# tychedelia/josefine

Hardware: AMD Instinct MI355X
Metric: Raft quorum decisions/sec over N partitions; achieved HBM GB/s vs roofline (higher is better)
Workload: dtype u64

## Files before the change

josefine_amd/csrc/jg_api_drains.h:

```cpp
#pragma once
namespace {
int node_keep_handover(jg_engine* e);
inline void seg_add(std::vector<JgSeg>& v, uint32_t seq, size_t n) {
  if (!n) return;
  if (!v.empty() && v.back().seq == seq) v.back().n += n;
  else v.push_back(JgSeg{seq, n});
}

int drain_scan(jg_engine* e, const std::vector<StepRec>& recs, hipStream_t st) {
  const size_t nrec = recs.size();
  if (!nrec) return JG_OK;
  if (e->scan_cap < 2 * nrec) {
    if (e->h_jobs) HIPCHK(hipHostFree(e->h_jobs));
    if (e->h_totals) HIPCHK(hipHostFree(e->h_totals));
    e->h_jobs = nullptr, e->h_totals = nullptr;
    e->scan_cap = std::max<size_t>(4 * nrec, 64);
    HIPCHK(hipHostMalloc((void**)&e->h_jobs, e->scan_cap * sizeof(JgScanJob), hipHostMallocDefault));
    HIPCHK(hipHostMalloc((void**)&e->h_totals, e->scan_cap * sizeof(uint64_t), hipHostMallocDefault));
  }
  for (size_t k = 0; k < nrec; k++) {
    const StepRec& r = recs[k];
    const uint32_t nb = (r.n + JG_SCAN_TILE - 1) / JG_SCAN_TILE;
    e->h_jobs[2 * k] = JgScanJob{r.d_bsum_m, r.d_bsum_m ? nb : 0u, 0};
    e->h_jobs[2 * k + 1] = JgScanJob{r.d_bsum_f, nb, 0};
// ... 460 lines not shown
    std::fill(count.begin(), count.end(), 0u);
    for (size_t i = 0; i < n; i++) count[(group[order[i]] >> shift) & (BUCKETS - 1)]++;
    uint32_t sum = 0;
    for (uint32_t b = 0; b < BUCKETS; b++) {
      uint32_t c = count[b];
      count[b] = sum;
      sum += c;
    }
    for (size_t i = 0; i < n; i++) tmp[count[(group[order[i]] >> shift) & (BUCKETS - 1)]++] = order[i];
    order.swap(tmp);
  }
}

int prepare_rows(jg_engine* e, uint32_t n, const uint32_t* group, const uint8_t* kind, const uint32_t* from,
                 const uint64_t* term, const uint64_t* id, const uint64_t* aux, const uint8_t* flag,
                 const uint64_t* blk_id, const uint64_t* blk_next, uint64_t n_blocks, uint64_t now_ms, JgRowsArgs* out,
                 uint32_t msg_per_row = 0) {
  StepRec rec;
  rec.n = n;
  rec.msg_per_row = msg_per_row ? msg_per_row : msg_bound(e->cfg.n_replicas);
  rec.fsm_per_row = fsm_bound();
  if ((uint64_t)n * rec.msg_per_row > 0xffffffffull) return fail(JG_EINVAL, "batch too large: split it");
  HIPCHK(e->arenas[e->cur_arena].alloc((size_t)n * 4, (void**)&rec.d_msg_cnt));
  HIPCHK(e->arenas[e->cur_arena].alloc((size_t)n * 4, (void**)&rec.d_fsm_cnt));
  HIPCHK(e->arenas[e->cur_arena].alloc((size_t)n * rec.msg_per_row * sizeof(jg_msg_row), (void**)&rec.d_msg));
  HIPCHK(e->arenas[e->cur_arena].alloc((size_t)n * rec.fsm_per_row * sizeof(jg_fsm_row), (void**)&rec.d_fsm));
  const uint32_t n_tiles = (n + JG_SCAN_TILE - 1) / JG_SCAN_TILE;
  HIPCHK(e->arenas[e->cur_arena].alloc((size_t)n_tiles * 8, (void**)&rec.d_bsum_m));
  HIPCHK(e->arenas[e->cur_arena].alloc((size_t)n_tiles * 8, (void**)&rec.d_bsum_f));
  JgRowsArgs a;
  a.n = n;
  a.group = group;
  a.kind = kind;
  a.from = from;
  a.term = term;
  a.id = id;
  a.aux = aux;
  a.flag = flag;
  a.blk_id = blk_id;
  a.blk_next = blk_next;
  a.n_blocks = n_blocks;
  a.msg_per_row = rec.msg_per_row;
  a.fsm_per_row = rec.fsm_per_row;
  a.msg_out = rec.d_msg;
  a.fsm_out = rec.d_fsm;
  a.msg_cnt = rec.d_msg_cnt;
  a.fsm_cnt = rec.d_fsm_cnt;
  a.bsum_m = rec.d_bsum_m;
  a.bsum_f = rec.d_bsum_f;
  a.err = e->d_err;
  a.now = now_ms;
  a.seq = e->seq;
  rec.seq = e->seq;
  e->n_launch += 1;
  e->recs.push_back(rec);
  e->n_cmds += n;
  e->maybe_irregular = true;
  e->flag_check_pending = true;
  e->irr_gen++;
  *out = a;
  return JG_OK;
}
int launch_rows(jg_engine* e, uint32_t n, const uint32_t* group, const uint8_t* kind, const uint32_t* from,
                const uint64_t* term, const uint64_t* id, const uint64_t* aux, const uint8_t* flag,
                const uint64_t* blk_id, const uint64_t* blk_next, uint64_t n_blocks, uint64_t now_ms) {
  JgRowsArgs a;
  const int rc = prepare_rows(e, n, group, kind, from, term, id, aux, flag, blk_id, blk_next, n_blocks, now_ms, &a);
  if (rc) return rc;
  static const char* runs_env = std::getenv("JG_APPLY_RUNS");
  static const bool runs = runs_env != nullptr, runs_small = runs_env && std::string(runs_env) == "small";
  if (runs_small)
    hipLaunchKernelGGL(k_apply_runs_small, dim3(std::min<uint32_t>((n + JG_RUN_TILE_SMALL - 1) / JG_RUN_TILE_SMALL, e->count_slots)), dim3(JG_BLOCK), 0,
                       e->stream, e->dev, a);
  else if (runs)
    hipLaunchKernelGGL(k_apply_runs, dim3(std::min<uint32_t>((n + JG_RUN_TILE - 1) / JG_RUN_TILE, e->count_slots)), dim3(JG_BLOCK), 0, e->stream,
                       e->dev, a);
  else
    hipLaunchKernelGGL(k_apply_rows, dim3(grid_for(n, e->count_slots)), dim3(JG_BLOCK), 0, e->stream, e->dev, a);
  HIPCHK(hipGetLastError());
  return JG_OK;
}

template <int R>
void launch_calib(jg_engine* e, const uint64_t* rot, const uint64_t* a8, uint64_t* b8, const uint32_t* c4) {
  hipLaunchKernelGGL(k_stream_calib<R>, dim3(e->dense_grid), dim3(JG_BLOCK), 0, e->stream, rot, a8, b8, c4,
                     e->cfg.n_groups);
}

}
```

josefine_amd/csrc/jg_api_misc.h:

```cpp
#pragma once
int jg_chain_compact(jg_engine* e, size_t n_trees, const uint64_t* off, const uint64_t* ids, const uint64_t* nexts,
                     const uint64_t* commits, uint8_t* removed) {
  if (!e || !off || !commits) return fail(JG_EINVAL, "null argument");
  if (!n_trees) return JG_OK;
  if (e->router) e = e->router->sh[0];
  HIPCHK(hipSetDevice(e->device));
  const size_t n = off[n_trees];
  if (n && (!ids || !nexts || !removed)) return fail(JG_EINVAL, "null argument");
  uint64_t *d_off = nullptr, *d_ids = nullptr, *d_next = nullptr, *d_commit = nullptr;
  uint8_t* d_rem = nullptr;
  HIPCHK(hipMalloc((void**)&d_off, (n_trees + 1) * 8));
  HIPCHK(hipMalloc((void**)&d_ids, std::max<size_t>(n * 8, 16)));
  HIPCHK(hipMalloc((void**)&d_next, std::max<size_t>(n * 8, 16)));
  HIPCHK(hipMalloc((void**)&d_commit, n_trees * 8));
  HIPCHK(hipMalloc((void**)&d_rem, std::max<size_t>(n, 16)));
  HIPCHK(hipMemcpyAsync(d_off, off, (n_trees + 1) * 8, hipMemcpyHostToDevice, e->stream));
  if (n) {
    HIPCHK(hipMemcpyAsync(d_ids, ids, n * 8, hipMemcpyHostToDevice, e->stream));
    HIPCHK(hipMemcpyAsync(d_next, nexts, n * 8, hipMemcpyHostToDevice, e->stream));
  }
  HIPCHK(hipMemcpyAsync(d_commit, commits, n_trees * 8, hipMemcpyHostToDevice, e->stream));
  HIPCHK(hipMemsetAsync(d_rem, 0, std::max<size_t>(n, 16), e->stream));
  hipLaunchKernelGGL(k_chain_compact, dim3(grid_for(n_trees, 2048)), dim3(JG_BLOCK), 0, e->stream, n_trees, d_off,
                     d_ids, d_next, d_commit, d_rem);
// ... 126 lines not shown
    if (!router_all_landed(e)) return JG_OK;
    return e->router->run([&](size_t d) { return drain_prefetch(e->router->sh[d], true); });
  }
  return drain_prefetch(e, false);
}

int jg_drain_wait(jg_engine* e) {
  if (!e) return fail(JG_EINVAL, "null argument");
  auto wait = [](jg_engine* s) {
    if (!s->inflight.phase) return (int)JG_OK;
    jg_engine::DrainThread& t = *s->drain_thread;
    std::unique_lock<std::mutex> lk(t.m);
    t.cv.wait(lk, [&] { return t.state == 2; });
    return (int)JG_OK;
  };
  if (e->router) {
    for (jg_engine* s : e->router->sh) wait(s);
    return JG_OK;
  }
  return wait(e);
}

int jg_drain_flush(jg_engine* e) {
  if (!e) return fail(JG_EINVAL, "null argument");
  auto flush = [](jg_engine* s) {
    int rc = drain_prefetch(s, true);
    if (rc) return rc;
    return inflight_finish(s);
  };
  if (e->router) {
    e->pipelined = true;
    for (jg_engine* s : e->router->sh) s->pipelined = true;
    return e->router->run([&](size_t d) { return flush(e->router->sh[d]); });
  }
  return flush(e);
}

int jg_drain_faults(jg_engine* e, jg_fault_row* out, size_t cap, size_t* n) {
  if (!e || !n) return fail(JG_EINVAL, "null argument");
  if (!e->router && e->pipelined && !inflight_landed(e)) {
    *n = 0;
    return JG_OK;
  }
  int rc = e->router ? router_collect(e, 0) : collect(e, 0);
  if (rc) return rc;
  std::vector<jg_fault_row>& q = e->router ? e->router->faults : e->q_faults;
  *n = q.size();
  if (!out) return JG_OK;
  if (cap < q.size()) return fail(JG_ECAPACITY, "output buffer too small");
  if (!q.empty()) std::memcpy(out, q.data(), q.size() * sizeof(jg_fault_row));
  q.clear();
  e->q_fault_seq.clear();
  return JG_OK;
}

int jg_read_state(jg_engine* e, int field, uint32_t replica, void* out, uint32_t g0, uint32_t n) {
  if (!e || (!out && n)) return fail(JG_EINVAL, "null argument");
  if (e->router) return router_read_state(e, field, replica, out, g0, n);
  if ((uint64_t)g0 + n > e->cfg.n_groups) return fail(JG_EINVAL, "group range out of bounds");
  if (field < 0 || field >= JG_FIELD__COUNT) return fail(JG_EINVAL, "unknown field");
  if (field == JG_FIELD_MATCH && replica >= e->cfg.n_replicas) return fail(JG_EINVAL, "replica out of range");
  if (!n) return JG_OK;
  int rc = sync_and_check(e);
  if (rc) return rc;
  const JgDev& d = e->dev;
  std::vector<uint32_t> fl(n);
  HIPCHK(hipMemcpy(fl.data(), d.flags + g0, (size_t)n * 4, hipMemcpyDeviceToHost));
  auto role = [&](uint32_t i) { return fl[i] & JGF_ROLE_MASK; };
  std::vector<uint64_t> t64;
  std::vector<uint32_t> t32;
  auto get64 = [&](const uint64_t* col) -> int {
    t64.resize(n);
    HIPCHK(hipMemcpy(t64.data(), col + g0, (size_t)n * 8, hipMemcpyDeviceToHost));
    return JG_OK;
  };
  auto cold_field = [&](const uint4* col, size_t offset, size_t width, void* dst) -> int {
    HIPCHK(hipMemcpy2D(dst, width, (const char*)(col + g0) + offset, sizeof(uint4), width, n, hipMemcpyDeviceToHost));
    return JG_OK;
  };
  auto cold32 = [&](size_t offset) -> int {
    t32.resize(n);
    return cold_field(d.cold.v, offset, 4, t32.data());
  };
  auto lag_base = [&](std::vector<uint64_t>& base) -> int {
    std::vector<uint64_t> top(n);
    HIPCHK(hipMemcpy(base.data(), d.head + g0, (size_t)n * 8, hipMemcpyDeviceToHost));
    HIPCHK(hipMemcpy(top.data(), d.run_hi + g0, (size_t)n * 8, hipMemcpyDeviceToHost));
    for (uint32_t i = 0; i < n; i++)
      if (jg_lag_base_is_run_hi(fl[i])) base[i] = top[i];
    return JG_OK;
  };
  auto copy64 = [&](const uint64_t* col) -> int {
    HIPCHK(hipMemcpy(out, col + g0, (size_t)n * 8, hipMemcpyDeviceToHost));
    return JG_OK;
  };
  uint64_t* o64 = (uint64_t*)out;
  uint32_t* o32 = (uint32_t*)out;
  uint8_t* o8 = (uint8_t*)out;
  switch (field) {
    case JG_FIELD_TERM: return copy64(d.term);
    case JG_FIELD_COMMIT: {
      std::vector<uint64_t> head(n), col(n);
      if ((rc = lag_base(head))) return rc;
      HIPCHK(hipMemcpy(col.data(), d.commit + g0, (size_t)n * 8, hipMemcpyDeviceToHost));
      if ((rc = get64(d.mlag))) return rc;
      for (uint32_t i = 0; i < n; i++) {
        const uint64_t f = jg_lag_field(t64[i], d.R, d.R);
        o64[i] = (role(i) != JG_ROLE_LEADER || jg_lag_wide(f, d.R)) ? col[i] : head[i] - f;
      }
      return JG_OK;
    }
    case JG_FIELD_HEAD: return copy64(d.head);
    case JG_FIELD_ELECTION_TIME: return cold_field(d.cold.t, JG_COLD_T_ELECTION_TIME, 8, out);
    case JG_FIELD_ELECTION_TIMEOUT: return cold_field(d.cold.t, JG_COLD_T_ELECTION_TIMEOUT, 4, out);
    case JG_FIELD_QUEUED_REQS: return cold_field(d.cold.v, JG_COLD_V_QUEUED, 4, out);
    case JG_FIELD_ID_GEN: {
      std::vector<uint64_t> head(n);
      HIPCHK(hipMemcpy(head.data(), d.head + g0, (size_t)n * 8, hipMemcpyDeviceToHost));
      if ((rc = get64(d.id_gen))) return rc;
      for (uint32_t i = 0; i < n; i++) o64[i] = (fl[i] & JGF_FAST) ? head[i] + 1 : t64[i];
      return JG_OK;
    }
    case JG_FIELD_MATCH: {
      std::vector<uint64_t> head(n), wide(n);
      if ((rc = lag_base(head))) return rc;
      HIPCHK(hipMemcpy(wide.data(), d.match_wide + (size_t)replica * d.G + g0, (size_t)n * 8, hipMemcpyDeviceToHost));
      if ((rc = get64(d.mlag))) return rc;
      for (uint32_t i = 0; i < n; i++) {
        const uint64_t f = jg_lag_field(t64[i], replica, d.R);
        o64[i] = role(i) != JG_ROLE_LEADER ? 0 : jg_lag_wide(f, d.R) ? wide[i] : head[i] - f;
      }
      return JG_OK;
    }
    case JG_FIELD_HEARTBEAT_TIME:
      if ((rc = get64(d.heartbeat_time))) return rc;
      for (uint32_t i = 0; i < n; i++) o64[i] = role(i) == JG_ROLE_LEADER ? t64[i] : 0;
      return JG_OK;
    case JG_FIELD_VOTED_FOR:
      if ((rc = cold32(JG_COLD_V_VOTED_FOR))) return rc;
      for (uint32_t i = 0; i < n; i++) o32[i] = (fl[i] & JGF_VOTED) ? t32[i] : 0;
      return JG_OK;
    case JG_FIELD_LEADER_ID:
      if ((rc = cold32(JG_COLD_V_LEADER_ID))) return rc;
      for (uint32_t i = 0; i < n; i++)
        o32[i] = (role(i) == JG_ROLE_FOLLOWER && (fl[i] & JGF_HAS_LEADER)) ? t32[i] : 0;
      return JG_OK;
    case JG_FIELD_VOTE_SEEN:
    case JG_FIELD_VOTE_GRANTED:
      if ((rc = cold32(JG_COLD_V_VOTES))) return rc;
      for (uint32_t i = 0; i < n; i++) {
        uint32_t v = field == JG_FIELD_VOTE_SEEN ? (t32[i] & 0xff) : ((t32[i] >> 8) & 0xff);
        o8[i] = role(i) == JG_ROLE_CANDIDATE ? (uint8_t)v : 0;
      }
      return JG_OK;
    case JG_FIELD_HAS_VOTED:
      for (uint32_t i = 0; i < n; i++) o8[i] = (fl[i] & JGF_VOTED) ? 1 : 0;
      return JG_OK;
    case JG_FIELD_ROLE:
      for (uint32_t i = 0; i < n; i++) o8[i] = (uint8_t)role(i);
      return JG_OK;
    case JG_FIELD_REPL_STATE:
      for (uint32_t i = 0; i < n; i++)
        o8[i] = role(i) == JG_ROLE_LEADER ? (uint8_t)((fl[i] & JGF_REPL_MASK) >> JGF_REPL_SHIFT) : 0;
      return JG_OK;
    case JG_FIELD_FAULT:
      for (uint32_t i = 0; i < n; i++) o8[i] = (uint8_t)((fl[i] & JGF_FAULT_MASK) >> JGF_FAULT_SHIFT);
      return JG_OK;
    case JG_FIELD_HAS_LEADER:
      for (uint32_t i = 0; i < n; i++) o8[i] = (role(i) == JG_ROLE_FOLLOWER && (fl[i] & JGF_HAS_LEADER)) ? 1 : 0;
      return JG_OK;
    case JG_FIELD_SELF_SLOT:
      for (uint32_t i = 0; i < n; i++) o8[i] = (uint8_t)((fl[i] & JGF_SELF_MASK) >> JGF_SELF_SHIFT);
      return JG_OK;
    default: return fail(JG_EINVAL, "unknown field");
  }
}

int jg_get_counters(jg_engine* e, uint64_t out[4]) {
  if (!e || !out) return fail(JG_EINVAL, "null argument");
  if (e->router) return router_get_counters(e, out);
  int rc = sync_and_check(e);
  if (rc) return rc;
  std::vector<uint64_t> slots(e->count_slots);
  HIPCHK(hipMemcpy(slots.data(), e->dev.blk_decisions, slots.size() * 8, hipMemcpyDeviceToHost));
  uint64_t dec = 0;
  for (uint64_t v : slots) dec += v;
  out[0] = e->n_cmds;
  out[1] = dec;
  out[2] = e->n_dense;
  out[3] = e->n_launch;
  return JG_OK;
}

int jg_device_alloc(jg_engine* e, size_t bytes, void** dev_ptr) {
  if (!e || !dev_ptr) return fail(JG_EINVAL, "null argument");
  if (e->router) return fail(JG_EINVAL, "device pointers are per shard: call this on a shard handle (jg_get_shard)");
  HIPCHK(hipSetDevice(e->device));
  HIPCHK(hipMalloc(dev_ptr, std::max<size_t>(bytes, 16)));
  HIPCHK(hipMemsetAsync(*dev_ptr, 0, std::max<size_t>(bytes, 16), e->stream));
  return JG_OK;
}
// ... 36 lines not shown
}
int jg_timer_stop(jg_engine* e, float* ms) {
  if (!e || !ms) return fail(JG_EINVAL, "null argument");
  if (e->router) {
    *ms = 0;
    for (jg_engine* s : e->router->sh) {
      float v = 0;
      const int rc = jg_timer_stop(s, &v);
      if (rc) return rc;
      *ms = std::max(*ms, v);
    }
    return JG_OK;
  }
  HIPCHK(hipSetDevice(e->device));
  HIPCHK(hipEventRecord(e->ev1, e->stream));
  {
    const auto t0 = std::chrono::steady_clock::now();
    hipError_t q;
    while ((q = hipEventQuery(e->ev1)) == hipErrorNotReady &&
           std::chrono::steady_clock::now() - t0 < std::chrono::milliseconds(20)) {
    }
    if (q != hipSuccess && q != hipErrorNotReady) return fail(JG_EDEVICE, std::string("hipEventQuery: ") + hipGetErrorString(q));
  }
  HIPCHK(hipEventSynchronize(e->ev1));
  HIPCHK(hipEventElapsedTime(ms, e->ev0, e->ev1));
  return JG_OK;
}

int jg_kernel_timing(jg_engine* e, int enable) {
  if (!e) return fail(JG_EINVAL, "null argument");
  if (e->router) {
    for (jg_engine* s : e->router->sh) {
      const int rc = jg_kernel_timing(s, enable);
      if (rc) return rc;
    }
    return JG_OK;
  }
  HIPCHK(hipSetDevice(e->device));
  if (enable && e->kt_ev.empty()) {
    e->kt_ev.resize(2 * jg_engine::KT_RING);
    for (hipEvent_t& ev : e->kt_ev) HIPCHK(hipEventCreate(&ev));
  }
  e->kt_on = enable != 0;
  e->kt_every = enable > 1 ? (uint32_t)enable : 1u;
  e->kt_n = 0, e->kt_seen = 0;
  return JG_OK;
}

int jg_kernel_timing_read(jg_engine* e, float* avg_us, uint32_t* n_launches) {
  if (!e || !avg_us || !n_launches) return fail(JG_EINVAL, "null argument");
  if (e->router) {
    *avg_us = 0, *n_launches = 0;
    for (jg_engine* s : e->router->sh) {
      float v = 0;
      uint32_t k = 0;
      const int rc = jg_kernel_timing_read(s, &v, &k);
      if (rc) return rc;
      if (v > *avg_us) *avg_us = v, *n_launches = k;
    }
    return JG_OK;
  }
  HIPCHK(hipSetDevice(e->device));
  HIPCHK(hipStreamSynchronize(e->stream));
  const uint64_t n = std::min<uint64_t>(e->kt_n, jg_engine::KT_RING);
  double sum = 0;
  for (uint64_t k = 0; k < n; k++) {
    float ms = 0;
    HIPCHK(hipEventElapsedTime(&ms, e->kt_ev[2 * k], e->kt_ev[2 * k + 1]));
    sum += ms;
  }
  *avg_us = n ? (float)(sum * 1e3 / (double)n) : 0.0f;
  *n_launches = (uint32_t)n;
  return JG_OK;
}

int jg_calibrate_stream(jg_engine* e, uint32_t iters, float* avg_us) {
  if (!e || !avg_us || !iters) return fail(JG_EINVAL, "null argument");
  if (e->router) e = e->router->sh[0];
  HIPCHK(hipSetDevice(e->device));
  const size_t G = e->cfg.n_groups, R = e->cfg.n_replicas;
  const size_t blk = std::max<size_t>(G * R * 8, 16);
  const size_t nbuf = std::min<size_t>(std::max<size_t>(((size_t)640 << 20) / blk + 1, 2), 64);
  char* rot = nullptr;
  uint64_t *a8 = nullptr, *b8 = nullptr;
  uint32_t* c4 = nullptr;
  HIPCHK(hipMalloc((void**)&rot, blk * nbuf));
  HIPCHK(hipMalloc((void**)&a8, std::max<size_t>(G * 8, 16)));
  HIPCHK(hipMalloc((void**)&b8, std::max<size_t>(G * 8, 16)));
  HIPCHK(hipMalloc((void**)&c4, std::max<size_t>(G * 4, 16)));
  HIPCHK(hipMemsetAsync(rot, 0, blk * nbuf, e->stream));
  HIPCHK(hipMemsetAsync(a8, 0, std::max<size_t>(G * 8, 16), e->stream));
  HIPCHK(hipMemsetAsync(b8, 0, std::max<size_t>(G * 8, 16), e->stream));
  HIPCHK(hipMemsetAsync(c4, 0, std::max<size_t>(G * 4, 16), e->stream));
  const uint32_t warm = 5;
  for (uint32_t i = 0; i < warm + iters; i++) {
    if (i == warm) HIPCHK(hipEventRecord(e->ev0, e->stream));
    const uint64_t* r = (const uint64_t*)(rot + (i % nbuf) * blk);
    switch (R) {
      case 1: launch_calib<1>(e, r, a8, b8, c4); break;
      case 2: launch_calib<2>(e, r, a8, b8, c4); break;
      case 3: launch_calib<3>(e, r, a8, b8, c4); break;
      case 4: launch_calib<4>(e, r, a8, b8, c4); break;
      case 5: launch_calib<5>(e, r, a8, b8, c4); break;
      case 6: launch_calib<6>(e, r, a8, b8, c4); break;
      case 7: launch_calib<7>(e, r, a8, b8, c4); break;
      default: launch_calib<8>(e, r, a8, b8, c4); break;
    }
  }
  HIPCHK(hipGetLastError());
  HIPCHK(hipEventRecord(e->ev1, e->stream));
  HIPCHK(hipEventSynchronize(e->ev1));
  float ms = 0;
  HIPCHK(hipEventElapsedTime(&ms, e->ev0, e->ev1));
  *avg_us = ms * 1000.0f / (float)iters;
  HIPCHK(hipFree(rot));
  HIPCHK(hipFree(a8));
  HIPCHK(hipFree(b8));
  HIPCHK(hipFree(c4));
  return JG_OK;
}

int jg_synth_fill_acks_device(jg_engine* e, uint32_t mode, uint64_t tick, uint64_t* sim_dev, uint64_t* acks_dev) {
  if (!e || !sim_dev || !acks_dev) return fail(JG_EINVAL, "null argument");
  if (e->router) return fail(JG_EINVAL, "device pointers are per shard: call this on a shard handle (jg_get_shard)");
  if (mode > 1) return fail(JG_EINVAL, "unknown synth mode");
  HIPCHK(hipSetDevice(e->device));
  hipLaunchKernelGGL(k_synth_acks, dim3(grid_for(e->cfg.n_groups, 4096)), dim3(JG_BLOCK), 0, e->stream, e->dev, mode,
                     tick, sim_dev, acks_dev);
  HIPCHK(hipGetLastError());
  return JG_OK;
}

}
```

josefine_amd/csrc/jg_await.h:

```cpp
#pragma once
#include "jg_device.h"
#include "jg_lookup.h"
#include "jg_read.h"
#include "jg_sparse.h"
#include "jg_compact.h"

#define JG_AWT_TILE JG_BLOCK
#define JG_AWT_PARTS 1024u
#define JG_AWT_WORDS 5u
static_assert(sizeof(jg_await_stats) == (JG_AWT_WORDS + 1) * 8, "jg_await_stats is the stat words in order, then left");
static_assert(sizeof(jg_await_row) == 48, "jg_await_row is three 16-byte pieces");
static_assert(sizeof(jg_done_row) == 48, "jg_done_row is three 16-byte pieces");

struct JgAwaitHead {
  uint32_t n, cur, pad[2];
};
static_assert(sizeof(JgAwaitHead) == 16, "the table's head is one 16-byte record");

struct JgAwaitArgs {
  uint32_t peek;
  uint32_t tiles;
  uint32_t parts;
  uint32_t n_keys;
  uint64_t now;
  uint64_t cap;
  uint64_t mask;
  uint4* buf[2];
  uint8_t* verdict;
  uint64_t* bsum;
  uint64_t* part;
  const uint64_t* total;
  uint4* out;
  const uint64_t* keys;
  uint64_t* mpart;
  uint32_t n;
  uint32_t cur;
  uint32_t add;
  uint64_t* sum;
  uint64_t* marked;
  uint32_t m;
  uint32_t room;
  uint32_t stats;
  JgAwaitHead* head;
  const uint32_t* gate;
  const uint4* rows;
  uint64_t* hdr;
};

__device__ __forceinline__ uint64_t jg_awt_u64(uint32_t lo, uint32_t hi) { return (uint64_t)lo | (uint64_t)hi << 32; }

__device__ __forceinline__ uint32_t jg_await_verdict(uint32_t wflags, uint32_t role, uint32_t fault, uint64_t term_now, uint64_t commit,
                                                     uint64_t block_id, uint64_t term, uint64_t deadline, uint64_t now) {
  if (wflags & JG_AWAIT_WITHDRAWN) return JG_DONE_CANCELLED;
  if (fault == JG_FAULT_VACANT) return JG_DONE_LOST | JG_DONE_VACANT;
  if (fault) return JG_DONE_LOST | JG_DONE_FAULTED;
  const bool leads = role == JG_ROLE_LEADER;
  if (term && (!leads || term_now != term)) return JG_DONE_LOST;
  if (leads ? block_id <= commit : block_id < commit) return JG_DONE_APPLIED;
  if (deadline && now >= deadline) return JG_DONE_EXPIRED;
  return 0u;
}

__device__ __forceinline__ void jg_await_count_tiles(const JgDev& d, const uint4* tab, uint32_t n, uint32_t tiles, uint32_t parts, uint64_t now,
                                                     uint8_t* verdict, uint64_t* bsum, uint64_t* part) {
  const uint32_t live = n / JG_AWT_TILE + (n % JG_AWT_TILE ? 1u : 0u);
  uint32_t bc[JG_AWT_WORDS] = {0u, 0u, 0u, 0u, 0u};
  for (uint32_t tile = blockIdx.x; tile < tiles; tile += parts) {
    uint32_t t = 0;
    if (tile < live) {
      const uint32_t i = tile * JG_AWT_TILE + threadIdx.x;
      const bool in = i < n;
      const size_t at = (size_t)(in ? i : 0u) * 3;
      const uint4 w0 = tab[at], w1 = tab[at + 1], w2 = tab[at + 2];
      const uint32_t g = w0.x < d.G ? w0.x : 0u;
      const uint32_t f = d.flags[g];
      const uint64_t term_now = d.term[g], head = d.head[g], pw = d.mlag[g], col = d.commit[g], run_hi = d.run_hi[g];
      const uint64_t commit = jg_read_commit(d, g, f);
      asm volatile("" ::"v"(f), "v"(term_now), "v"(head), "v"(pw), "v"(col), "v"(run_hi));
      const uint32_t role = f & JGF_ROLE_MASK, fault = (f & JGF_FAULT_MASK) >> JGF_FAULT_SHIFT;
      const uint32_t v = in ? jg_await_verdict(w0.y, role, fault, term_now, commit, jg_awt_u64(w1.x, w1.y), jg_awt_u64(w1.z, w1.w),
                                               jg_awt_u64(w2.x, w2.y), now)
                            : 0u;
      if (in) verdict[i] = (uint8_t)v;
      const uint64_t m = __ballot(in && v);
      bc[0] += __popcll(__ballot(in && !v));
      bc[1] += __popcll(m);
      bc[2] += __popcll(__ballot(in && (v & JG_DONE_APPLIED)));
      bc[3] += __popcll(__ballot(in && (v & JG_DONE_LOST)));
      bc[4] += __popcll(__ballot(in && (v & JG_DONE_EXPIRED)));
      t = jg_tile_count(__popcll(m));
    }
    if (threadIdx.x == 0) bsum[tile] = t;
    __syncthreads();
  }
  const uint64_t vals[JG_AWT_WORDS] = {bc[0], bc[1], bc[2], bc[3], bc[4]};
  jg_block_words<JG_AWT_WORDS>(vals, JgNeverMax(), part);
}

__device__ __forceinline__ void jg_await_write_tile(const JgDev& d, const uint4* tab, uint4* dst, uint32_t n, uint32_t add, uint32_t peek, uint64_t cap,
                                                    const uint64_t* total, const uint8_t* verdict, const uint64_t* bsum, uint4* out) {
  const uint64_t done = *total;
  if ((done < cap ? done : cap) == 0) return;
  if ((uint64_t)blockIdx.x * JG_AWT_TILE >= n) return;
  const uint64_t base = bsum[blockIdx.x];
  if (peek && base >= cap) return;
  const uint32_t i = blockIdx.x * JG_AWT_TILE + threadIdx.x;
  const bool in = i < n;
  const uint32_t v = in ? verdict[i] : 0u;
  const uint64_t rank = base + jg_rank_in_tile(__ballot(in && v));
  if (!in) return;
  const bool deliver = v && rank < cap;
  if (!deliver && peek) return;
  const size_t at = (size_t)i * 3;
  const uint4 w0 = tab[at], w1 = tab[at + 1], w2 = tab[at + 2];
  if (!deliver) {
    const size_t to = ((size_t)i - (size_t)(rank < cap ? rank : cap)) * 3;
    dst[to] = w0, dst[to + 1] = w1, dst[to + 2] = w2;
    return;
  }
  const uint32_t g = w0.x < d.G ? w0.x : 0u;
  const uint32_t f = d.flags[g];
  const uint64_t term_now = d.term[g], head = d.head[g];
  const uint64_t commit = jg_read_commit(d, g, f);
  const uint32_t role = f & JGF_ROLE_MASK, fault = (f & JGF_FAULT_MASK) >> JGF_FAULT_SHIFT, self = (f & JGF_SELF_MASK) >> JGF_SELF_SHIFT;
  auto lo = [](uint64_t x) { return (uint32_t)x; };
  auto hi = [](uint64_t x) { return (uint32_t)(x >> 32); };
  jg_u32x4* row = (jg_u32x4*)out + rank * 3;
  row[0] = jg_u32x4{add + g, v | role << 8 | fault << 16 | self << 24, w0.z, w0.w};
  row[1] = jg_u32x4{w1.x, w1.y, lo(term_now), hi(term_now)};
  row[2] = jg_u32x4{lo(commit), hi(commit), lo(head), hi(head)};
}

__global__ __launch_bounds__(JG_BLOCK) void k_await_count(JgDev d, JgAwaitArgs a) {
  jg_await_count_tiles(d, a.buf[a.cur & 1u], a.n, a.tiles, a.parts, a.now, a.verdict, a.bsum, a.part);
}

__global__ __launch_bounds__(JG_BLOCK) void k_await_stats_sum(JgAwaitArgs a) {
  jg_parts_reduce<JG_AWT_WORDS>(a.part, a.parts, a.sum, JgNeverMax());
}

__global__ __launch_bounds__(JG_BLOCK) void k_await_write(JgDev d, JgAwaitArgs a) {
  const uint32_t cur = a.cur & 1u;
  jg_await_write_tile(d, a.buf[cur], a.buf[cur ^ 1u], a.n, a.add, a.peek, a.cap, a.total, a.verdict, a.bsum, a.out);
}

#define JG_AWT_KEYS_LDS 2048u

__device__ __forceinline__ bool jg_awt_has_key(const uint64_t* keys, uint32_t n, uint64_t key) {
  uint32_t lo = 0, hi = n;
  while (lo < hi) {
    const uint32_t mid = (lo + hi) >> 1;
    if (keys[mid] < key) lo = mid + 1;
    else hi = mid;
  }
  return lo < n && keys[lo] == key;
}

__device__ __forceinline__ void jg_await_mark_tiles(uint4* tab, uint32_t n, uint32_t tiles, uint32_t parts, const uint64_t* keys, uint32_t n_keys,
                                                    uint64_t mask, uint64_t* part) {
  __shared__ uint64_t lds_keys[JG_AWT_KEYS_LDS];
  const bool staged = n_keys <= JG_AWT_KEYS_LDS;
  if (staged) {
    for (uint32_t k = threadIdx.x; k < n_keys; k += JG_BLOCK) lds_keys[k] = keys[k];
    __syncthreads();
  }
  uint32_t marked = 0;
  for (uint32_t tile = blockIdx.x; tile < tiles; tile += parts) {
    if ((uint64_t)tile * JG_AWT_TILE >= n) break;
    const uint32_t i = tile * JG_AWT_TILE + threadIdx.x;
    const bool in = i < n;
    const size_t at = (size_t)(in ? i : 0u) * 3;
    const uint4 w0 = tab[at];
    const uint64_t key = jg_awt_u64(w0.z, w0.w) & mask;
    const bool has = staged ? jg_awt_has_key(lds_keys, n_keys, key) : jg_awt_has_key(keys, n_keys, key);
    const bool hit = in && has && !(w0.y & JG_AWAIT_WITHDRAWN);
    if (hit) ((uint32_t*)(tab + at))[1] = w0.y | JG_AWAIT_WITHDRAWN;
    marked += __popcll(__ballot(hit));
  }
  const uint64_t vals[1] = {marked};
  jg_block_words<1>(vals, JgNeverMax(), part);
}

__global__ __launch_bounds__(JG_BLOCK) void k_await_mark(JgAwaitArgs a) {
  jg_await_mark_tiles(a.buf[a.cur & 1u], a.n, a.tiles, a.parts, a.keys, a.n_keys, a.mask, a.mpart);
}

__global__ __launch_bounds__(JG_BLOCK) void k_await_mark_sum(JgAwaitArgs a) {
  jg_parts_reduce<1>(a.mpart, a.parts, a.marked, JgNeverMax());
}


#define JG_AH_TOTAL 0u
#define JG_AH_GIVEN 1u
#define JG_AH_STATS 2u
#define JG_AH_LEFT (JG_AH_STATS + JG_AWT_WORDS)
#define JG_AH_N (JG_AH_LEFT + 1u)
#define JG_AH_CUR (JG_AH_N + 1u)
#define JG_AH_GATE (JG_AH_CUR + 1u)
#define JG_AH_MARKED (JG_AH_GATE + 1u)
#define JG_AH_WORDS (JG_AH_MARKED + 1u)

__device__ __forceinline__ bool jg_await_gated(const uint32_t* gate) { return gate && *gate; }
__device__ __forceinline__ uint32_t jg_await_n_eff(const JgAwaitArgs& a, uint32_t n) {
  const uint64_t e = (uint64_t)n + a.m;
  return e > a.room ? a.room : (uint32_t)e;
// ... 47 lines not shown
```

josefine_amd/csrc/jg_commits.h:

```cpp
#pragma once
#include "jg_device.h"
#include "jg_lookup.h"
#include "jg_read.h"
#include "jg_sparse.h"
#include "jg_watch.h"

#define JG_CMT_ROWS 4u
#define JG_CMT_TILE (JG_BLOCK * JG_CMT_ROWS)
#define JG_CMT_PARTS 1024u
#define JG_CMT_WORDS 6u
static_assert(sizeof(jg_commit_backlog) == JG_CMT_WORDS * 8, "jg_commit_backlog is the backlog words in order");
static_assert(sizeof(jg_commit_row) == 48, "jg_commit_row is three 16-byte pieces");

struct JgCommitArgs {
  uint32_t g0, n;
  uint32_t add;
  uint32_t peek;
  uint32_t commits_only;
  uint32_t backlog;
  uint32_t tiles;
  uint32_t parts;
  uint4* shadow;
  uint32_t* cnt;
  uint64_t* bsum;
  uint64_t* part;
  uint64_t* sum;
  uint4* out;
  uint64_t cap;
  const uint32_t* gate;
};

__device__ __forceinline__ uint64_t jg_cmt_u64(uint32_t lo, uint32_t hi) { return (uint64_t)lo | (uint64_t)hi << 32; }

__device__ __forceinline__ uint64_t jg_commit_view(const JgDev& d, uint32_t g, uint32_t f, uint64_t w, uint64_t head, uint64_t col) {
  const uint32_t R = d.R;
  const bool leader = (f & JGF_ROLE_MASK) == JG_ROLE_LEADER;
  const uint64_t fc = jg_lag_field(w, R, R);
  uint64_t c = leader ? head - fc : col;
  if (leader && (jg_lag_wide(fc, R) || jg_lag_base_is_run_hi(f))) c = jg_read_commit(d, g, f);
  return c;
}
__device__ __forceinline__ bool jg_commit_differs(const uint4& sh, uint64_t commit, uint64_t head, uint32_t commits_only) {
  return sh.x != (uint32_t)commit || sh.y != (uint32_t)(commit >> 32) ||
         (!commits_only && (sh.z != (uint32_t)head || sh.w != (uint32_t)(head >> 32)));
}
__device__ __forceinline__ void jg_commit_backlog_add(bool on, uint64_t m, const uint4& sh, uint64_t commit, uint64_t head, uint32_t* bc,
                                                      uint64_t& commits, uint64_t& appends) {
  const uint64_t cf = jg_cmt_u64(sh.x, sh.y), hf = jg_cmt_u64(sh.z, sh.w);
  const bool up_c = on && commit > cf, up_h = on && head > hf;
  bc[0] += __popcll(m);
  bc[1] += __popcll(__ballot(up_c));
  bc[2] += __popcll(__ballot(up_h));
  bc[3] += __popcll(__ballot(on && (commit < cf || head < hf)));
  commits += up_c ? commit - cf : 0ull;
  appends += up_h ? head - hf : 0ull;
}

__device__ __forceinline__ void jg_commit_ballots(const JgDev& d, const JgCommitArgs& a, uint32_t tile, uint32_t* f, uint64_t* commit,
                                                  uint64_t* head, uint4* sh, uint64_t* m) {
  const uint32_t t0 = tile * JG_CMT_TILE + threadIdx.x;
  uint64_t w[JG_CMT_ROWS], col[JG_CMT_ROWS];
#pragma unroll
  for (uint32_t k = 0; k < JG_CMT_ROWS; k++) {
    const uint32_t i = t0 + k * JG_BLOCK;
    const bool in = i < a.n;
    const uint32_t g = a.g0 + (in ? i : 0u);
    f[k] = in ? d.flags[g] : 0u;
    head[k] = in ? d.head[g] : 0ull;
    w[k] = in ? d.mlag[g] : 0ull;
    col[k] = in ? d.commit[g] : 0ull;
    sh[k] = in ? a.shadow[g] : make_uint4(0, 0, 0, 0);
  }
#pragma unroll
  for (uint32_t k = 0; k < JG_CMT_ROWS; k++) asm volatile("" ::"v"(f[k]), "v"(head[k]), "v"(w[k]), "v"(col[k]), "v"(sh[k].x), "v"(sh[k].z));
#pragma unroll
  for (uint32_t k = 0; k < JG_CMT_ROWS; k++) {
    const uint32_t i = t0 + k * JG_BLOCK;
    const bool in = i < a.n;
    commit[k] = jg_commit_view(d, a.g0 + (in ? i : 0u), f[k], w[k], head[k], col[k]);
    m[k] = __ballot(in && jg_commit_differs(sh[k], commit[k], head[k], a.commits_only));
  }
}

__global__ __launch_bounds__(JG_BLOCK) void k_commit_count(JgDev d, JgCommitArgs a) {
  const uint32_t lane = threadIdx.x & 63u;
  uint32_t bc[4] = {0u, 0u, 0u, 0u};
  uint64_t commits = 0, appends = 0;
  for (uint32_t tile = blockIdx.x; tile < a.tiles; tile += a.parts) {
    uint32_t f[JG_CMT_ROWS];
    uint64_t commit[JG_CMT_ROWS], head[JG_CMT_ROWS], m[JG_CMT_ROWS];
    uint4 sh[JG_CMT_ROWS];
    jg_commit_ballots(d, a, tile, f, commit, head, sh, m);
    uint32_t c = 0;
#pragma unroll
    for (uint32_t k = 0; k < JG_CMT_ROWS; k++) c += __popcll(m[k]);
    if (a.backlog) {
#pragma unroll
      for (uint32_t k = 0; k < JG_CMT_ROWS; k++)
        jg_commit_backlog_add((m[k] >> lane) & 1ull, m[k], sh[k], commit[k], head[k], bc, commits, appends);
    }
    const uint32_t t = jg_tile_count(c);
    if (threadIdx.x == 0) a.cnt[tile] = t, a.bsum[tile] = t;
    __syncthreads();
  }
  if (!a.backlog) return;
  const uint64_t vals[JG_CMT_WORDS] = {bc[0], bc[1], bc[2], bc[3], jg_wave_sum64(commits), jg_wave_sum64(appends)};
  jg_block_words<JG_CMT_WORDS>(vals, JgNeverMax(), a.part);
}

__global__ __launch_bounds__(JG_BLOCK) void k_commit_write(JgDev d, JgCommitArgs a) {
  const uint64_t base = a.bsum[blockIdx.x];
  if (a.cnt[blockIdx.x] == 0 || base >= a.cap) return;
  uint32_t f[JG_CMT_ROWS];
  uint64_t commit[JG_CMT_ROWS], head[JG_CMT_ROWS], m[JG_CMT_ROWS];
  uint4 sh[JG_CMT_ROWS];
  jg_commit_ballots(d, a, blockIdx.x, f, commit, head, sh, m);
  const uint32_t peek = jg_gated_peek(a.peek, a.gate);
  const uint32_t lane = threadIdx.x & 63u;
  const uint32_t t0 = blockIdx.x * JG_CMT_TILE + threadIdx.x;
  uint64_t term[JG_CMT_ROWS];
#pragma unroll
  for (uint32_t k = 0; k < JG_CMT_ROWS; k++)
    term[k] = ((m[k] >> lane) & 1ull) ? d.term[a.g0 + t0 + k * JG_BLOCK] : 0ull;
  jg_u32x4* out = (jg_u32x4*)a.out;
  auto lo = [](uint64_t x) { return (uint32_t)x; };
  auto hi = [](uint64_t x) { return (uint32_t)(x >> 32); };
  jg_ranked_rows<JG_CMT_ROWS>(m, base, a.cap, [&](uint32_t k, uint64_t pos) {
    const uint32_t g = a.g0 + t0 + k * JG_BLOCK;
    const uint32_t role = f[k] & JGF_ROLE_MASK, fault = (f[k] & JGF_FAULT_MASK) >> JGF_FAULT_SHIFT, self = (f[k] & JGF_SELF_MASK) >> JGF_SELF_SHIFT;
    const uint64_t cf = jg_cmt_u64(sh[k].x, sh[k].y), hf = jg_cmt_u64(sh[k].z, sh[k].w);
    const uint32_t state = (commit[k] > cf ? (uint32_t)JG_CMT_COMMITTED : 0u) | (head[k] > hf ? (uint32_t)JG_CMT_APPENDED : 0u) |
                           (commit[k] < cf || head[k] < hf ? (uint32_t)JG_CMT_REWOUND : 0u) |
                           (role == JG_ROLE_LEADER && fault == 0 ? (uint32_t)JG_CMT_LEADS : 0u) |
                           (fault == JG_FAULT_VACANT ? (uint32_t)JG_CMT_VACANT : fault ? (uint32_t)JG_CMT_FAULTED : 0u);
    out[pos * 3 + 0] = jg_u32x4{a.add + g, role | state << 8 | fault << 16 | self << 24, lo(term[k]), hi(term[k])};
    out[pos * 3 + 1] = jg_u32x4{sh[k].x, sh[k].y, lo(commit[k]), hi(commit[k])};
    out[pos * 3 + 2] = jg_u32x4{sh[k].z, sh[k].w, lo(head[k]), hi(head[k])};
    if (!peek) a.shadow[g] = make_uint4(lo(commit[k]), hi(commit[k]), lo(head[k]), hi(head[k]));
  });
}

__global__ __launch_bounds__(JG_BLOCK) void k_commit_backlog_sum(JgCommitArgs a) {
  jg_parts_reduce<JG_CMT_WORDS>(a.part, a.parts, a.sum, JgNeverMax());
}
```

josefine_amd/csrc/jg_dense.h:

```cpp
#pragma once
#include "jg_device.h"

#ifndef JG_BLOCK
#define JG_BLOCK 256
#endif

struct JgDenseHot {
  uint32_t* flags;
  uint64_t* mlag;
  uint64_t* head;
  uint64_t* blk_decisions;
  uint32_t G;
  uint32_t hb_timeout, cfg_flags;
  uint64_t* term;
  uint64_t* heartbeat_time;
  uint32_t g_begin, g_end;
};
__host__ __device__ __forceinline__ JgDenseHot jg_dense_hot_of(const JgDev& d) {
  return JgDenseHot{d.flags, d.mlag, d.head, d.blk_decisions, d.G, d.hb_timeout, d.cfg_flags, d.term, d.heartbeat_time, 0u, d.G};
}
__host__ __device__ __forceinline__ JgDenseHot jg_dense_hot_range(const JgDev& d, uint32_t begin, uint32_t end, uint32_t slot0) {
  JgDenseHot h = jg_dense_hot_of(d);
  h.blk_decisions += slot0, h.g_begin = begin, h.g_end = end;
  return h;
}


__device__ __forceinline__ void jg_block_count(uint64_t* slots, uint32_t v) {
  __shared__ uint32_t wave_sum[JG_BLOCK / 64];
#pragma unroll
  for (int off = 32; off > 0; off >>= 1) v += __shfl_down(v, off, 64);
  uint32_t lane = threadIdx.x & 63u, wave = threadIdx.x >> 6;
  if (lane == 0) wave_sum[wave] = v;
  __syncthreads();
  if (threadIdx.x == 0) {
    uint32_t s = 0;
#pragma unroll
    for (int w = 0; w < JG_BLOCK / 64; w++) s += wave_sum[w];
    if (s)
      (void)__hip_atomic_fetch_add(&slots[blockIdx.x], (uint64_t)s, __ATOMIC_RELAXED, __HIP_MEMORY_SCOPE_AGENT);
  }
}

struct JgDecCount {
  uint32_t lane = 0;
};
__device__ __forceinline__ void jg_count_add(uint64_t* slots, uint32_t total) {
  (void)__hip_atomic_fetch_add(&slots[blockIdx.x], (uint64_t)total, __ATOMIC_RELAXED, __HIP_MEMORY_SCOPE_AGENT);
}
__device__ __forceinline__ void jg_count_step(uint64_t* slots, JgDecCount& c, bool on, uint32_t n) {
  const uint64_t m = __ballot(on);
  if (!m) return;
  const int first = __ffsll((long long)m) - 1;
  const uint32_t n0 = __builtin_amdgcn_readlane(n, first);
  if (__ballot(on && n != n0) == 0) {
    if ((int)(threadIdx.x & 63u) == first && n0) jg_count_add(slots, n0 * (uint32_t)__popcll(m));
  } else {
    c.lane += on ? n : 0u;
  }
}
__device__ __forceinline__ void jg_wave_count(uint64_t* slots, const JgDecCount& c) {
  uint32_t v = c.lane;
  if (__ballot(v != 0) == 0) return;
#pragma unroll
  for (int off = 32; off > 0; off >>= 1) v += __shfl_down(v, off, 64);
  if ((threadIdx.x & 63u) == 0 && v) jg_count_add(slots, v);
}

template <int R>
__device__ __forceinline__ void jg_dense_load_acks(const uint64_t* __restrict__ acks, uint32_t G, uint32_t g,
                                                   uint64_t (&a)[R]) {
#pragma unroll
  for (int r = 0; r < R; r++) a[r] = __builtin_nontemporal_load(&acks[(size_t)r * G + g]);
}
template <int R, bool MAYBE_NO_ACKS = true>
__device__ __forceinline__ void jg_dense_load(const JgDenseHot& d, const uint64_t* __restrict__ acks, uint32_t g,
                                              uint64_t (&a)[R], uint64_t& mword, uint64_t& head) {
  if (!MAYBE_NO_ACKS || acks) {
    jg_dense_load_acks<R>(acks, d.G, g, a);
  } else {
#pragma unroll
    for (int r = 0; r < R; r++) a[r] = JG_NO_ACK;
  }
  mword = d.mlag[g];
  head = d.head[g];
}
template <int R>
struct JgLagTick {
  uint64_t w1, head1;
  uint32_t nf;
  uint32_t l[R + 1];
  uint32_t adv;
  bool cwide;
};

template <int R>
__device__ __forceinline__ uint32_t jg_kth_lag(const uint32_t (&v)[R + 1]) {
  constexpr int K = R / 2;
  if (R == 3) {
    const uint32_t lo = min(v[0], v[1]), hi = max(v[0], v[1]);
    return max(lo, min(hi, v[2]));
  } else if (R == 5) {
    const uint32_t x = max(min(v[0], v[1]), min(v[2], v[3]));
    const uint32_t y = min(max(v[0], v[1]), max(v[2], v[3]));
    const uint32_t lo = min(x, y), hi = max(x, y);
    return max(lo, min(hi, v[4]));
  } else {
    uint32_t q = 0;
#pragma unroll
    for (int j = 0; j < R; j++) {
      int cnt = 0;
#pragma unroll
      for (int i = 0; i < R; i++) cnt += (v[i] < v[j] || (v[i] == v[j] && i < j)) ? 1 : 0;
      q = (cnt == K) ? v[j] : q;
    }
    return q;
  }
}

template <int R>
__device__ __forceinline__ bool jg_lag_tick(uint32_t s, uint32_t f, uint64_t w0, uint64_t head0, uint64_t n_app,
                                            const uint64_t (&a)[R], JgLagTick<R>& o, uint32_t& dec) {
  constexpr uint32_t B = 64u / (R + 1u);
  if (B > 21) return false;
  constexpr uint32_t ESC = (uint32_t)((1ull << (B > 21 ? 21 : B)) - 1ull);
  constexpr uint32_t BEHIND = ESC - 1u, INF = 0xffffffffu;
  const uint32_t n = (uint32_t)n_app;
  bool bad = n_app >= JG_MAX_DENSE_APPENDS;
  const uint64_t head1 = head0 + n;
  uint32_t incm = 0, somem = 0;
#pragma unroll
  for (int r = 0; r < R; r++) {
    const uint32_t fr = (uint32_t)(w0 >> (r * B)) & ESC;
    const uint64_t ar = a[r];
    const uint64_t dk = head1 - ar;
    const bool self = (uint32_t)r == s;
    const bool some = !self && ar != JG_NO_ACK;
    const bool behind = fr == BEHIND;
    uint32_t dl = (uint32_t)(dk >> 32) ? 0xffffffffu : (uint32_t)dk;
    dl = some ? dl : 0xffffffffu;
    const uint32_t frn = fr + n;
    const bool inc = dl < frn;
    incm |= inc ? (1u << r) : 0u;
    somem |= some ? (1u << r) : 0u;
    uint32_t lo = (self && n) ? 0u : min(frn, dl);
    bad |= fr == ESC;
    bad |= behind ? some : lo >= BEHIND;
    bad |= some && ar > head1;
    lo = (behind && !(self && n)) ? INF : lo;
    o.l[r] = lo;
  }
  const uint32_t fc = (uint32_t)(w0 >> (R * B)) & ESC;
  const uint32_t lc = fc == BEHIND ? INF : fc + n;
  const uint32_t ql = jg_kth_lag<R>(o.l);
  const uint32_t nl = min(lc, ql);
  o.l[R] = nl;
  bad |= fc == ESC;
  bad |= nl >= BEHIND;
  if (bad) return false;
  uint32_t nf = (f & ~(somem << JGF_REPL_SHIFT)) | (incm << JGF_REPL_SHIFT);
  nf |= n ? (1u << (JGF_REPL_SHIFT + s)) : 0u;
  nf |= ql < lc ? JGF_COMMIT_KEY : 0u;
  uint64_t w = 0;
#pragma unroll
  for (int r = 0; r <= R; r++) w |= (uint64_t)min(o.l[r], BEHIND) << (r * B);
  o.w1 = w;
  o.head1 = head1;
  o.nf = nf;
  o.cwide = fc == BEHIND;
  o.adv = lc - nl;
  dec += n + (uint32_t)__popc(somem);
  return true;
}

template <int R>
__device__ __forceinline__ bool jg_lag_pre(uint32_t s, uint64_t w0, uint64_t head0, const uint64_t (&a)[R], uint32_t pre,
                                           uint32_t& adv_pre) {
  constexpr uint32_t B = 64u / (R + 1u);
  constexpr uint32_t ESC = (uint32_t)((1ull << (B > 21 ? 21 : B)) - 1ull);
  constexpr uint32_t BEHIND = ESC - 1u, INF = 0xffffffffu;
  bool bad = false;
  uint32_t l[R + 1];
#pragma unroll
  for (int r = 0; r < R; r++) {
    const uint32_t fr = (uint32_t)(w0 >> (r * B)) & ESC;
    const uint64_t ar = a[r];
    const bool some = (uint32_t)r != s && ((pre >> r) & 1u) && ar != JG_NO_ACK;
    const uint64_t dk = head0 - ar;
    uint32_t dl = (uint32_t)(dk >> 32) ? INF : (uint32_t)dk;
    dl = some ? dl : INF;
    bad |= some && ar > head0;
    l[r] = fr == BEHIND ? INF : min(fr, dl);
  }
  const uint32_t fc = (uint32_t)(w0 >> (R * B)) & ESC;
  const uint32_t lc = fc == BEHIND ? INF : fc;
  const uint32_t ql = jg_kth_lag<R>(l);
  adv_pre = lc - min(lc, ql);
  return !bad;
}

template <int R>
__device__ __forceinline__ bool jg_lag_tick_regs(uint32_t s, uint32_t& nf_io, uint32_t (&l)[R + 1], uint64_t& head_io,
                                                 uint64_t n_app, const uint64_t (&a)[R], uint32_t& dec) {
  const uint64_t head0 = head_io;
  constexpr uint32_t INF = 0xffffffffu;
  const uint32_t n = (uint32_t)n_app;
  bool bad = n_app >= JG_MAX_DENSE_APPENDS;
  const uint64_t head1 = head0 + n;
  uint32_t incm = 0, somem = 0;
  uint32_t nl[R + 1];
#pragma unroll
  for (int r = 0; r < R; r++) {
// ... 127 lines not shown
  if ((f & JGF_ROLE_MASK) != JG_ROLE_LEADER) {
    if (n_app) {
      d.flags[g] = f | (JG_FAULT_ENGINE_DENSE_NONLEADER << JGF_FAULT_SHIFT);
      jg_push_fault(d, g, JG_FAULT_ENGINE_DENSE_NONLEADER, seq);
    }
    return JG_DENSE_SKIP;
  }
  if (n_app >= JG_MAX_DENSE_APPENDS) {
    d.flags[g] = f | (JG_FAULT_ENGINE_DENSE_APPENDS << JGF_FAULT_SHIFT);
    jg_push_fault(d, g, JG_FAULT_ENGINE_DENSE_APPENDS, seq);
    return JG_DENSE_SKIP;
  }
  if (!(f & JGF_FAST)) return JG_DENSE_DEFER;
  return JG_DENSE_RUN;
}

template <int R, bool SKIP_OWN>
__device__ __forceinline__ void jg_dense_outbox_none(uint32_t G, const JgLeaderNode& nd, uint32_t g, uint32_t s) {
  nd.o_beat[g] = jg_leader_beat{0, JG_NO_ACK};
  if (nd.o_aec) {
    nd.o_aec[g] = JG_NO_ACK;
    return;
  }
#pragma unroll
  for (int r = 0; r < R; r++)
    if (!(SKIP_OWN && (uint32_t)r == s)) nd.o_ae[(size_t)r * G + g] = JG_NO_ACK;
}
template <int R, bool SKIP_OWN, class MoOf>
__device__ __forceinline__ uint32_t jg_dense_leader_tick(const JgDenseHot& h, const JgDev* dp, const JgLeaderNode& nd,
                                                         uint32_t g, uint32_t seq, uint32_t s, uint64_t term,
                                                         uint64_t hbt, uint64_t head, uint64_t commit, uint32_t nf,
                                                         MoOf mo_of) {
  const uint32_t G = h.G;
  if (head >= JG_MAILBOX_NONE) {
    jg_dense_outbox_none<R, SKIP_OWN>(G, nd, g, s);
    jg_push_fault(*dp, g, JG_FAULT_ENGINE_MAILBOX_RANGE, seq);
    return nf | (JG_FAULT_ENGINE_MAILBOX_RANGE << JGF_FAULT_SHIFT);
  }
  const bool due = (nd.now - hbt) > (uint64_t)h.hb_timeout;
  const uint64_t hb = due ? commit : JG_NO_ACK;
  const bool key_in_range = (nf & JGF_COMMIT_KEY) && !(h.cfg_flags & JG_CFG_SEPARATE_COMMIT_KEY);
  bool dead = false;
  uint64_t word[R];
#pragma unroll
  for (int r = 0; r < R; r++) {
    uint32_t n = JG_AE_NONE;
    uint64_t from = 0;
    if ((uint32_t)r != s && !dead) {
      const bool repl = (nf >> (JGF_REPL_SHIFT + r)) & 1u;
      const uint32_t want = repl ? JG_MAX_INFLIGHT + 1 : 2;
      from = mo_of(r);
      const uint64_t avail = from <= head ? head - from + 1 : 0;
      const uint32_t cnt = avail >= want ? want : (uint32_t)avail;
      if (cnt < want && key_in_range) {
        dead = true;
        from = 0;
        nf |= JG_FAULT_RANGE_HIT_COMMIT_KEY << JGF_FAULT_SHIFT;
      } else {
        n = cnt ? cnt - 1 : 0;
      }
    }
    word[r] = n == JG_AE_NONE ? JG_NO_ACK : JG_AE(from, n);
  }
  if (dead) jg_push_fault(*dp, g, JG_FAULT_RANGE_HIT_COMMIT_KEY, seq);
  if (due) h.heartbeat_time[g] = nd.now;
  nd.o_beat[g] = jg_leader_beat{term, hb};
  if (nd.o_aec) {
    const uint64_t first = s == 0 ? word[R > 1 ? 1 : 0] : word[0];
    bool same = true;
#pragma unroll
    for (int r = 0; r < R; r++) same = same && ((uint32_t)r == s || word[r] == first);
    nd.o_aec[g] = same ? first : JG_AEC_INDIVIDUAL;
    if (__builtin_expect(same, 1)) return nf;
  }
#pragma unroll
  for (int r = 0; r < R; r++)
    if (!(SKIP_OWN && (uint32_t)r == s)) nd.o_ae[(size_t)r * G + g] = word[r];
  return nf;
}

template <int R>
struct JgDenseIn {
  uint32_t f;
  uint64_t a[R], w, head;
  uint64_t term, hbt;
  uint32_t own;
};
template <int R, bool UNIFORM, bool NODE, bool ANY = false>
__device__ __forceinline__ void jg_dense_issue(const JgDenseHot& h, const JgDev* dp,
                                               const uint64_t* __restrict__ acks, uint32_t us,
                                               const JgLeaderNode& nd, bool emit, uint32_t g, JgDenseIn<R>& in) {
  in.f = h.flags[g];
  in.term = in.hbt = 0;
  if (!NODE) {
    jg_dense_load<R, false>(h, acks, g, in.a, in.w, in.head);
  } else {
#pragma unroll
    for (int r = 0; r < R; r++)
      in.a[r] = (ANY && (uint32_t)r == us) ? nd.offered[g] : __builtin_nontemporal_load(&acks[((size_t)r * h.G + g) * nd.ack_stride]);
    if (ANY) in.own = nd.owner[g];
    in.w = h.mlag[g];
    in.head = h.head[g];
    in.term = h.term[g];
    in.hbt = h.heartbeat_time[g];
  }
  asm volatile("" ::"v"(in.f));
  if (NODE) asm volatile("" ::"v"(in.term), "v"(in.hbt));
  __builtin_amdgcn_sched_barrier(0);
}

template <int R>
__device__ __forceinline__ uint64_t jg_lds_kth(const uint64_t (*sm)[JG_BLOCK]) {
  const uint32_t t = threadIdx.x;
  uint64_t q = 0;
#pragma clang loop unroll(disable)
  for (int j = 0; j < R; j++) {
    const uint64_t vj = sm[j][t];
    int cnt = 0;
#pragma clang loop unroll(disable)
    for (int i = 0; i < R; i++) {
      const uint64_t vi = sm[i][t];
      cnt += (vi > vj || (vi == vj && i < j)) ? 1 : 0;
    }
    q = (cnt == R / 2) ? vj : q;
  }
  return q;
}

template <int R, bool UNIFORM>
__device__ __forceinline__ void jg_dense_cold_lds(const JgDev& d, const uint64_t* __restrict__ acks, uint32_t seq,
                                               uint32_t s, uint32_t f, uint64_t n_app, uint32_t g,
                                               const uint64_t (&a_in)[R], uint64_t w0, uint64_t head0, JgDecCount& dec,
                                               uint64_t (*sm)[JG_BLOCK]) {
  const uint32_t G = d.G, t = threadIdx.x;
  const uint32_t B = jg_lag_bits(R);
  const uint64_t esc = jg_lag_esc(R);
  uint64_t(*sa)[JG_BLOCK] = sm + R;
#pragma unroll
  for (int r = 0; r < R; r++) sa[r][t] = ((uint32_t)r == s || !acks) ? JG_NO_ACK : a_in[r];
  uint64_t hi = 0;
#pragma clang loop unroll(disable)
  for (int r = 0; r < R; r++) {
    const uint64_t fl = (w0 >> (r * B)) & esc;
    const uint64_t v = jg_lag_wide(fl, R) ? d.match_wide[(size_t)r * G + g] : head0 - fl;
    sm[r][t] = v;
    hi = v > hi ? v : hi;
    const uint64_t a = sa[r][t];
    hi = (a != JG_NO_ACK && a > hi) ? a : hi;
  }
  const uint64_t fc = (w0 >> (R * B)) & esc;
  const uint64_t commit0 = jg_lag_wide(fc, R) ? d.commit[g] : head0 - fc;
  uint64_t commit = commit0, head = head0;
  uint32_t nf = f, fault = 0, dc = 0;
  const bool fused = hi <= head0;
  if (fused) {
    head = head0 + n_app;
    if (n_app) {
      const bool inc = sm[s][t] < head;
      if (inc) sm[s][t] = head;
      nf = inc ? (nf | (1u << (JGF_REPL_SHIFT + s))) : (nf & ~(1u << (JGF_REPL_SHIFT + s)));
      dc += (uint32_t)n_app;
    }
  } else {
    for (uint64_t i = 0; i < n_app && !fault; i++) {
      head += 1;
      const bool inc = sm[s][t] < head;
      if (inc) sm[s][t] = head;
      nf = inc ? (nf | (1u << (JGF_REPL_SHIFT + s))) : (nf & ~(1u << (JGF_REPL_SHIFT + s)));
      dc += 1;
      const uint64_t q = jg_lds_kth<R>(sm);
      if (q > commit) {
        if (q <= head) commit = q;
        else fault = JG_FAULT_COMMIT_MISSING_BLOCK;
      }
    }
  }
#pragma clang loop unroll(disable)
  for (int r = 0; r < R; r++) {
    if (fault) continue;
    const uint64_t a = sa[r][t];
    if (a == JG_NO_ACK) continue;
    const bool inc = sm[r][t] < a;
    if (inc) sm[r][t] = a;
    nf = inc ? (nf | (1u << (JGF_REPL_SHIFT + r))) : (nf & ~(1u << (JGF_REPL_SHIFT + r)));
    dc += 1;
    if (!fused) {
      const uint64_t q = jg_lds_kth<R>(sm);
      if (q > commit) {
        if (q <= head) commit = q;
        else fault = JG_FAULT_COMMIT_MISSING_BLOCK;
      }
    }
  }
  if (fused) {
    const uint64_t q = jg_lds_kth<R>(sm);
    commit = q > commit ? q : commit;
  }
  if (fault) {
    nf |= fault << JGF_FAULT_SHIFT;
    jg_push_fault(d, g, fault, seq);
  }
  if (commit != commit0) nf |= JGF_COMMIT_KEY;
  dec.lane += dc;
  uint64_t w = 0;
#pragma clang loop unroll(disable)
  for (int r = 0; r < R; r++) {
    const uint64_t v = sm[r][t];
    const uint64_t fl = jg_lag_encode(v, head, R);
    if (jg_lag_wide(fl, R)) d.match_wide[(size_t)r * G + g] = v;
    w |= fl << (r * B);
  }
  const uint64_t fl = jg_lag_encode(commit, head, R);
  if (jg_lag_wide(fl, R) && (commit != commit0 || !jg_lag_wide(fc, R))) d.commit[g] = commit;
  w |= fl << (R * B);
  if (w != w0) d.mlag[g] = w;
  if (head != head0) d.head[g] = head;
  if (nf != f) d.flags[g] = nf;
}

template <int R, bool UNIFORM, bool NODE, bool DEFER, bool FSM = false, bool ANY = false>
__device__ __forceinline__ void jg_dense_group(const JgDenseHot& h, const JgDev* dp,
                                               const uint64_t* __restrict__ acks, uint32_t seq, uint32_t us, const JgLeaderNode& nd, bool emit, uint32_t g,
                                               const JgDenseIn<R>& in, JgDecCount& dec, uint64_t (*sm)[JG_BLOCK]) {
  const uint32_t f = in.f;
  const uint32_t s = UNIFORM ? us : (f & JGF_SELF_MASK) >> JGF_SELF_SHIFT;
  const uint64_t mword0 = in.w, head0 = in.head, term = in.term, hbt = in.hbt;
  bool hbr_trigger = false;
  uint64_t a[R];
#pragma unroll
  for (int r = 0; r < R; r++) {
    a[r] = NODE ? jg_answer_ack(in.a[r]) : in.a[r];
    if (NODE) hbr_trigger |= (uint32_t)r != s && jg_answer_hb(in.a[r]) == 0;
  }
  uint64_t n_app = a[0];
#pragma unroll
  for (int r = 1; r < R; r++) n_app = (uint32_t)r == s ? a[r] : n_app;
  if (NODE && !nd.ack_stride) n_app = 0;
  const bool mine = !ANY || in.own == s;
  if (ANY && !mine) {
#pragma unroll
    for (int r = 0; r < R; r++) a[r] = JG_NO_ACK;
    n_app = 0;
    hbr_trigger = false;
  }
  uint32_t pre = 0;
  if (FSM) {
    pre = (uint32_t)(n_app >> JG_NODE_PRE_SHIFT) & 0xffu;
    n_app &= (1ull << JG_NODE_PRE_SHIFT) - 1ull;
  }
  JgLagTick<R> lt;
  lt.cwide = false, lt.adv = 0;
  uint32_t dl = 0;
  bool hot = (f & (JGF_FAULT_MASK | JGF_ROLE_MASK | JGF_FAST)) == (JG_ROLE_LEADER | JGF_FAST);
  uint64_t base0 = head0;
  if (NODE) {
    const bool runx = (f & (JGF_FAULT_MASK | JGF_ROLE_MASK | JGF_FAST | JGF_WIN_MASK | JGF_NO_GENESIS)) == JG_ROLE_LEADER && n_app == 0;
    if (__builtin_expect(runx, 0)) {
      if (!(f & JGF_RUN)) base0 = dp->run_hi[g];
      hot = true;
    }
  }
  if (NODE) hot = hot && !hbr_trigger;
  if (ANY) hot = hot && mine;
  hot = jg_lag_tick<R>(s, f, mword0, base0, n_app, a, lt, dl) && hot;
  if (FSM) hot = hot && n_app <= 1 && !lt.cwide;
  uint32_t adv_pre = 0;
  if (FSM && __builtin_expect(pre != 0, 0)) hot = jg_lag_pre<R>(s, mword0, base0, a, pre, adv_pre) && hot;
  if (!NODE) jg_count_step(h.blk_decisions, dec, hot, dl);
  if (__builtin_expect(hot, 1)) {
    if (emit)
      lt.nf = jg_dense_leader_tick<R, UNIFORM>(h, dp, nd, g, seq, s, term, hbt, lt.head1, lt.head1 - lt.l[R], lt.nf, [&](int r) {
        return lt.l[r] == 0xffffffffu ? dp->match_wide[(size_t)r * h.G + g] : lt.head1 - lt.l[r];
      });
    if (lt.w1 != mword0) h.mlag[g] = lt.w1;
    if (lt.head1 != base0) h.head[g] = lt.head1;
    if (lt.nf != f) h.flags[g] = lt.nf;
    if (FSM) {
      uint32_t w = (n_app ? JG_FSM_APPENDED_BIT : 0u) | lt.adv | (adv_pre << JG_FSM_PRE_SHIFT);
      if (__builtin_expect(lt.adv > JG_FSM_ADV_MASK, 0)) {
        const uint64_t commit0 = lt.head1 - lt.l[R] - lt.adv;
        nd.fsm_prev[g] = commit0;
        nd.fsm_mid[g] = commit0 + adv_pre;
        w = (n_app ? JG_FSM_APPENDED_BIT : 0u) | JG_FSM_WIDE_BIT;
      }
      if (w) nd.fsm_delta[g] = w;
    }
    if (NODE) jg_count_step(h.blk_decisions, dec, true, dl);
    return;
  }
  const JgDev& d = *dp;
  if (NODE && !ANY && nd.mask_offers && (f & JGF_ROLE_MASK) != JG_ROLE_LEADER) {
    if (emit) jg_dense_outbox_none<R, UNIFORM>(h.G, nd, g, s);
    return;
  }
  int cls = jg_dense_classify(d, g, f, n_app, seq);
  if ((NODE || DEFER) && cls == JG_DENSE_RUN) cls = JG_DENSE_DEFER;
  jg_defer_mark(d, g, cls == JG_DENSE_DEFER);
  if (NODE) {
    if (emit && mine) jg_dense_outbox_none<R, UNIFORM>(h.G, nd, g, s);
    return;
  }
  if (DEFER || cls != JG_DENSE_RUN) return;
  *d.cold_seen = 1;
  jg_dense_cold_lds<R, UNIFORM>(d, acks, seq, s, f, n_app, g, a, mword0, head0, dec, sm);
}

template <int R, bool UNIFORM, bool NODE, bool DEFER, bool FSM = false, bool ANY = false>
__device__ __forceinline__ JgDecCount jg_dense_tick_body(const JgDenseHot& h, const JgDev* dp,
                                                       const uint64_t* __restrict__ acks, uint32_t seq, uint32_t us,
                                                       const JgLeaderNode& nd, uint64_t (*sm)[JG_BLOCK]) {
  const uint32_t end = h.g_end, stride = gridDim.x * JG_BLOCK;
  const bool emit = NODE && nd.o_beat != nullptr;
  JgDecCount dec;
  uint32_t g = h.g_begin + blockIdx.x * JG_BLOCK + threadIdx.x;
  for (; g < end; g += stride) {
    if (FSM && nd.sparse_bits && jg_sparse_skip(nd.sparse_bits, nd.sparse_mode, g)) continue;
    if (ANY) {
      const uint32_t f0 = h.flags[g];
      if (__ballot((f0 & (JGF_ROLE_MASK | JGF_FAULT_MASK)) == JG_ROLE_LEADER) == 0) continue;
    }
    JgDenseIn<R> in;
    jg_dense_issue<R, UNIFORM, NODE, ANY>(h, dp, acks, us, nd, emit, g, in);
    jg_dense_group<R, UNIFORM, NODE, DEFER, FSM, ANY>(h, dp, acks, seq, us, nd, emit, g, in, dec, sm);
  }
  return dec;
}

template <int R, bool DEFER>
__global__ __launch_bounds__(JG_BLOCK) void k_leader_tick_dense(JgDenseHot h, const JgDev* __restrict__ dp,
                                                                               const uint64_t* __restrict__ acks,
                                                                               uint32_t seq, int us) {
  __shared__ uint64_t sm[DEFER ? 1 : 2 * R][JG_BLOCK];
  JgDecCount dec;
  JgLeaderNode nd{};
  if (us >= 0) dec = jg_dense_tick_body<R, true, false, DEFER>(h, dp, acks, seq, (uint32_t)us, nd, sm);
  else dec = jg_dense_tick_body<R, false, false, DEFER>(h, dp, acks, seq, 0, nd, sm);
  jg_wave_count(h.blk_decisions, dec);
}

#ifdef JG_LEADER_WAVES
#define JG_LEADER_OCC __attribute__((amdgpu_waves_per_eu(JG_LEADER_WAVES, JG_LEADER_WAVES)))
#else
#define JG_LEADER_OCC
#endif
#ifdef JG_FOLLOWER_WAVES
#define JG_FOLLOWER_OCC __attribute__((amdgpu_waves_per_eu(JG_FOLLOWER_WAVES, JG_FOLLOWER_WAVES)))
#else
#define JG_FOLLOWER_OCC
#endif
template <int R, bool FSM>
__global__ __launch_bounds__(JG_BLOCK) JG_LEADER_OCC void k_leader_node_tick(JgDenseHot h, const JgDev* __restrict__ dp,
                                                                const uint64_t* __restrict__ acks, uint32_t seq, int us,
                                                                JgLeaderNode nd) {
  if (nd.clock) {
    const uint32_t a = nd.clock->idx_lead & 1u;
    nd.now = nd.clock->v[a].now, seq = nd.clock->v[a].seq[nd.clock_slot];
    if (blockIdx.x == 0 && threadIdx.x == 0) nd.clock->idx_rest = a;
  }
  JgDecCount dec;
  if (us >= 0) dec = jg_dense_tick_body<R, true, true, true, FSM>(h, dp, acks, seq, (uint32_t)us, nd, nullptr);
  else dec = jg_dense_tick_body<R, false, true, true, FSM>(h, dp, acks, seq, 0, nd, nullptr);
  jg_wave_count(h.blk_decisions, dec);
}

struct JgLeaderJob {
  JgDenseHot h;
  const JgDev* dp;
  const uint64_t* acks;
  uint32_t seq;
  int us;
  JgLeaderNode nd;
};
template <int R>
__global__ __launch_bounds__(JG_BLOCK) void k_leader_node_tick_any(const JgLeaderJob* __restrict__ jobs) {
  const JgLeaderJob& j = jobs[blockIdx.y];
  JgLeaderNode nd = j.nd;
  uint32_t seq = j.seq;
  if (nd.clock) {
    const uint32_t a = nd.clock->idx_lead & 1u;
    nd.now = nd.clock->v[a].now, seq = nd.clock->v[a].seq[nd.clock_slot];
    if (blockIdx.x == 0 && blockIdx.y == 0 && threadIdx.x == 0) nd.clock->idx_rest = a;
  }
  const JgDecCount dec = jg_dense_tick_body<R, true, true, true, false, true>(j.h, j.dp, j.acks, seq, (uint32_t)j.us, nd, nullptr);
  jg_wave_count(j.h.blk_decisions, dec);
}

struct JgClaimArgs {
  const uint32_t* flags[JG_MAX_REPLICAS];
  uint32_t R, G;
  uint8_t* owner;
  uint64_t* answers;
};
__global__ __launch_bounds__(JG_BLOCK) void k_cluster_claim(JgClaimArgs a) {
  const uint32_t n4 = (a.G + 3u) / 4u;
  constexpr uint32_t M = JGF_ROLE_MASK | JGF_FAULT_MASK;
  for (uint32_t q = blockIdx.x * JG_BLOCK + threadIdx.x; q < n4; q += gridDim.x * JG_BLOCK) {
    uint32_t o[4] = {JG_OWNER_NONE, JG_OWNER_NONE, JG_OWNER_NONE, JG_OWNER_NONE};
    if (q * 4u + 3u < a.G) {
      for (uint32_t r = a.R; r-- > 0;) {
        const uint4 f = ((const uint4*)a.flags[r])[q];
        o[0] = (f.x & M) == JG_ROLE_LEADER ? r : o[0];
        o[1] = (f.y & M) == JG_ROLE_LEADER ? r : o[1];
        o[2] = (f.z & M) == JG_ROLE_LEADER ? r : o[2];
        o[3] = (f.w & M) == JG_ROLE_LEADER ? r : o[3];
      }
    } else {
      for (uint32_t k = 0; k < 4; k++)
        for (uint32_t r = a.R; q * 4u + k < a.G && r-- > 0;) o[k] = (a.flags[r][q * 4u + k] & M) == JG_ROLE_LEADER ? r : o[k];
    }
    const uint32_t now = o[0] | o[1] << 8 | o[2] << 16 | o[3] << 24, was = ((const uint32_t*)a.owner)[q];
    if (now == was) continue;
    for (uint32_t k = 0; k < 4; k++) {
      const uint32_t p = (was >> (8 * k)) & 0xffu;
      if (p != JG_OWNER_NONE && p != o[k] && o[k] != JG_OWNER_NONE && q * 4u + k < a.G) a.answers[(size_t)p * a.G + q * 4u + k] = JG_NO_ACK;
    }
    ((uint32_t*)a.owner)[q] = now;
  }
}

template <int R, bool UNIFORM>
__device__ __forceinline__ uint32_t jg_dense_ticks_body(const JgDev& d, const uint64_t* __restrict__ acks,
                                                        uint32_t n_ticks, size_t tick_stride, uint32_t seq0,
                                                        uint32_t us) {
  const uint32_t G = d.G;
  uint32_t dec = 0;
  for (uint32_t g = blockIdx.x * JG_BLOCK + threadIdx.x; g < G; g += gridDim.x * JG_BLOCK) {
    const uint32_t f = d.flags[g];
    const uint32_t s = UNIFORM ? us : (f & JGF_SELF_MASK) >> JGF_SELF_SHIFT;
    uint64_t a[R], mword0, head0;
    jg_dense_load<R, false>(jg_dense_hot_of(d), acks, g, a, mword0, head0);
    asm volatile("" ::"v"(f));
    __builtin_amdgcn_sched_barrier(0);
    const bool leader = (f & JGF_ROLE_MASK) == JG_ROLE_LEADER;
    const bool dead = (f & JGF_FAULT_MASK) != 0;
    const bool defer = !dead && leader && !(f & JGF_FAST);
    jg_defer_mark(d, g, defer);
    if (dead || defer) continue;
    constexpr uint32_t B = 64u / (R + 1u);
    constexpr uint32_t ESC = (uint32_t)((1ull << (B > 31 ? 31 : B)) - 1ull);
    uint64_t head = head0;
    uint32_t nf = f, gdec = 0;
    uint32_t l[R + 1];
    bool fits = B <= 21;
#pragma unroll
    for (int r = 0; r <= R; r++) {
      l[r] = (uint32_t)(mword0 >> (r * B)) & ESC;
      fits = fits && l[r] != ESC;
      l[r] = l[r] == ESC - 1u ? 0xffffffffu : l[r];
    }
    fits = fits || !leader;
    uint64_t a1[R];
    if (n_ticks > 1) {
      jg_dense_load_acks<R>(acks + tick_stride, G, g, a1);
    } else {
#pragma unroll
      for (int r = 0; r < R; r++) a1[r] = JG_NO_ACK;
    }
    for (uint32_t t = 0; fits && t < n_ticks; t++) {
      uint64_t a2[R];
      if (t + 2 < n_ticks) {
        jg_dense_load_acks<R>(acks + (size_t)(t + 2) * tick_stride, G, g, a2);
      } else {
#pragma unroll
        for (int r = 0; r < R; r++) a2[r] = JG_NO_ACK;
      }
      uint64_t n_app = a[0];
#pragma unroll
      for (int r = 1; r < R; r++) n_app = (uint32_t)r == s ? a[r] : n_app;
      if (!leader) {
        if (n_app) {
          nf = f | (JG_FAULT_ENGINE_DENSE_NONLEADER << JGF_FAULT_SHIFT);
          jg_push_fault(d, g, JG_FAULT_ENGINE_DENSE_NONLEADER, seq0 + t);
          break;
        }
      } else if (!jg_lag_tick_regs<R>(s, nf, l, head, n_app, a, gdec)) {
        fits = false;
      }
#pragma unroll
      for (int r = 0; r < R; r++) a[r] = a1[r], a1[r] = a2[r];
    }
    uint64_t w = mword0;
    if (leader && fits) {
      w = 0;
#pragma unroll
      for (int r = 0; r <= R; r++) {
        fits = fits && (l[r] < ESC - 1u || l[r] == 0xffffffffu);
        w |= (uint64_t)min(l[r], ESC - 1u) << (r * B);
      }
    }
    jg_defer_mark(d, g, !fits);
    if (!fits) continue;
    dec += gdec;
    if (w != mword0) d.mlag[g] = w;
    if (head != head0) d.head[g] = head;
    if (nf != f) d.flags[g] = nf;
  }
  return dec;
}

template <int R>
__global__ __launch_bounds__(JG_BLOCK) void k_leader_tick_dense_n(JgDev d, const uint64_t* __restrict__ acks,
                                                                   uint32_t n_ticks, size_t tick_stride,
                                                                   uint32_t seq0, int us) {
  uint32_t dec;
  if (us >= 0) dec = jg_dense_ticks_body<R, true>(d, acks, n_ticks, tick_stride, seq0, (uint32_t)us);
  else dec = jg_dense_ticks_body<R, false>(d, acks, n_ticks, tick_stride, seq0, 0);
  jg_block_count(d.blk_decisions, dec);
}
```

josefine_amd/csrc/jg_device.h:

```cpp
#pragma once
#include <hip/hip_runtime.h>
#include <stdint.h>

#include "../../include/josefine_gpu.h"

#define JGF_ROLE_MASK 0x3u
#define JGF_VOTED (1u << 2)
#define JGF_HAS_LEADER (1u << 3)
#define JGF_FAST (1u << 4)
#define JGF_COMMIT_KEY (1u << 5)
#ifdef JG_GSM_WAVES
#define JG_GSM_OCC __attribute__((amdgpu_waves_per_eu(JG_GSM_WAVES)))
#else
#define JG_GSM_OCC
#endif
#define JGF_NO_GENESIS (1u << 6)
#define JGF_RUN (1u << 7)
#define JGF_REPL_SHIFT 8
#define JGF_REPL_MASK (0xffu << JGF_REPL_SHIFT)
#define JGF_FAULT_SHIFT 16
#define JGF_FAULT_MASK (0xffu << JGF_FAULT_SHIFT)
#define JGF_SELF_SHIFT 24
#define JGF_SELF_MASK (0x7u << JGF_SELF_SHIFT)
#define JGF_WIN_SHIFT 28
#define JGF_WIN_MASK (0xfu << JGF_WIN_SHIFT)

struct JgXqRec {
  jg_msg_row row;
  uint32_t seq;
  uint32_t k;
};

struct JgFaultRec {
  uint32_t group;
  uint32_t code;
  uint32_t seq;
  uint32_t pad;
};

struct JgCold {
  uint64_t election_time;
  uint32_t election_timeout;
  uint32_t rng_draws;
  uint32_t voted_for;
  uint32_t leader_id;
  uint32_t queued;
  uint32_t votes;
};
struct JgColdCols {
  uint4* t;
  uint4* v;
};
#define JG_COLD_T_ELECTION_TIME 0
#define JG_COLD_T_ELECTION_TIMEOUT 8
#define JG_COLD_V_VOTED_FOR 0
#define JG_COLD_V_LEADER_ID 4
#define JG_COLD_V_QUEUED 8
#define JG_COLD_V_VOTES 12
__device__ __forceinline__ JgCold jg_cold_load(const JgColdCols& p, uint32_t g) {
  const uint4 a = p.t[g], b = p.v[g];
  JgCold c;
  c.election_time = (uint64_t)a.x | (uint64_t)a.y << 32;
  c.election_timeout = a.z, c.rng_draws = a.w, c.voted_for = b.x, c.leader_id = b.y, c.queued = b.z, c.votes = b.w;
  return c;
}
__device__ __forceinline__ void jg_cold_store_timer(const JgColdCols& p, uint32_t g, const JgCold& c) {
  p.t[g] = make_uint4((uint32_t)c.election_time, (uint32_t)(c.election_time >> 32), c.election_timeout, c.rng_draws);
}
__device__ __forceinline__ void jg_cold_store_rest(const JgColdCols& p, uint32_t g, const JgCold& c) {
  p.v[g] = make_uint4(c.voted_for, c.leader_id, c.queued, c.votes);
}
__device__ __forceinline__ void jg_cold_store(const JgColdCols& p, uint32_t g, const JgCold& c) {
  jg_cold_store_timer(p, g, c);
  jg_cold_store_rest(p, g, c);
}
__device__ __forceinline__ JgCold jg_cold_of(uint64_t election_time, uint32_t voted_for, uint32_t leader_id, uint32_t election_timeout,
                                             uint32_t rng_draws, uint32_t queued, uint32_t votes) {
  JgCold c;
  c.election_time = election_time, c.election_timeout = election_timeout, c.rng_draws = rng_draws;
  c.voted_for = voted_for, c.leader_id = leader_id, c.queued = queued, c.votes = votes;
  return c;
}

struct JgDev {
  uint32_t G, R;
  uint32_t node_ids[JG_MAX_REPLICAS];
  uint32_t hb_timeout, el_min, el_max, cfg_flags;
  uint64_t seed, group_base;
  uint64_t* term;
  uint64_t* commit;
  uint64_t* head;
  uint64_t* id_gen;
  uint64_t* run_hi;
  uint64_t* mlag;
  uint64_t* match_wide;
  uint64_t* heartbeat_time;
  uint64_t* win_lo;
  uint64_t* win_hi;
  uint64_t* win_next;
  uint32_t* flags;
  JgColdCols cold;
  uint32_t* fvote_id;
  uint64_t* blk_decisions;
  JgFaultRec* fault_q;
  uint32_t* fault_q_n;
  uint32_t fault_q_cap;
// ... 6 lines not shown
  uint32_t* cold_seen;
  JgXqRec* xq;
  uint32_t* xq_n;
  uint32_t xq_cap;
  uint32_t slow_cap;
  uint32_t* err;
};

__device__ __forceinline__ uint64_t jg_mix64(uint64_t z) {
  z += 0x9e3779b97f4a7c15ull;
  z = (z ^ (z >> 30)) * 0xbf58476d1ce4e5b9ull;
  z = (z ^ (z >> 27)) * 0x94d049bb133111ebull;
  return z ^ (z >> 31);
}

__host__ __device__ __forceinline__ uint32_t jg_lag_bits(uint32_t R) { return 64u / (R + 1u); }
__host__ __device__ __forceinline__ uint64_t jg_lag_esc(uint32_t R) { return (1ull << jg_lag_bits(R)) - 1ull; }
__host__ __device__ __forceinline__ uint64_t jg_lag_field(uint64_t w, uint32_t r, uint32_t R) {
  return (w >> (r * jg_lag_bits(R))) & jg_lag_esc(R);
}
__host__ __device__ __forceinline__ uint64_t jg_lag_with(uint64_t w, uint32_t r, uint32_t R, uint64_t field) {
  const uint32_t sh = r * jg_lag_bits(R);
  return (w & ~(jg_lag_esc(R) << sh)) | (field << sh);
}
__host__ __device__ __forceinline__ uint64_t jg_lag_behind(uint32_t R) { return jg_lag_esc(R) - 1ull; }
__host__ __device__ __forceinline__ bool jg_lag_wide(uint64_t field, uint32_t R) { return field >= jg_lag_behind(R); }
__host__ __device__ __forceinline__ uint64_t jg_lag_encode(uint64_t v, uint64_t base, uint32_t R) {
  if (v > base) return jg_lag_esc(R);
  return base - v < jg_lag_behind(R) ? base - v : jg_lag_behind(R);
}

struct JgLane {
  uint32_t g;
  uint64_t term, commit, head, id_gen, run_hi, election_time, heartbeat_time;
  uint64_t mword, mbase;
  uint32_t flags, voted_for, leader_id, election_timeout, rng_draws, queued, votes;
  uint64_t now;
  uint32_t seq;
  uint32_t decisions;
  jg_msg_row* mp;
  jg_msg_row* mend;
  jg_fsm_row* fp;
  jg_fsm_row* fend;
  uint32_t overflow;
  uint32_t xq_on;
  uint32_t xq_k;
  uint64_t cap_ack, cap_hbc;
  uint32_t cap_has;
  uint64_t* cap_ae;
};

__device__ __forceinline__ uint32_t jg_role(const JgLane& L) { return L.flags & JGF_ROLE_MASK; }
__device__ __forceinline__ void jg_set_role(JgLane& L, uint32_t r) { L.flags = (L.flags & ~JGF_ROLE_MASK) | r; }
__device__ __forceinline__ uint32_t jg_fault(const JgLane& L) { return (L.flags & JGF_FAULT_MASK) >> JGF_FAULT_SHIFT; }
__device__ __forceinline__ uint32_t jg_self(const JgLane& L) { return (L.flags & JGF_SELF_MASK) >> JGF_SELF_SHIFT; }
__device__ __forceinline__ uint32_t jg_wcnt(const JgLane& L) { return (L.flags & JGF_WIN_MASK) >> JGF_WIN_SHIFT; }
__device__ __forceinline__ uint32_t jg_self_id(const JgDev& d, const JgLane& L) { return d.node_ids[jg_self(L)]; }

__device__ inline void jg_push_fault(const JgDev& d, uint32_t g, uint32_t code, uint32_t seq) {
  uint32_t i = atomicAdd(d.fault_q_n, 1u);
  if (i < d.fault_q_cap) {
    JgFaultRec r;
    r.group = g;
    r.code = code;
    r.seq = seq;
    r.pad = 0;
    d.fault_q[i] = r;
  }
}
__device__ inline void jg_raise(const JgDev& d, JgLane& L, uint32_t code) {
  if (jg_fault(L)) return;
  L.flags |= code << JGF_FAULT_SHIFT;
  jg_push_fault(d, L.g, code, L.seq);
}

__device__ inline void jg_chain_normalize(const JgDev& d, JgLane& L);

__host__ __device__ __forceinline__ bool jg_lag_base_is_run_hi(uint32_t flags) {
  return (flags & (JGF_WIN_MASK | JGF_NO_GENESIS | JGF_RUN)) == 0;
}
__device__ __forceinline__ uint64_t jg_lane_base(const JgLane& L) {
  return (L.flags & (JGF_WIN_MASK | JGF_NO_GENESIS)) == 0 ? L.run_hi : L.head;
}
__device__ inline uint64_t jg_match_get(const JgDev& d, const JgLane& L, uint32_t r) {
  const uint64_t f = jg_lag_field(L.mword, r, d.R);
  return jg_lag_wide(f, d.R) ? d.match_wide[(size_t)r * d.G + L.g] : L.mbase - f;
}
__device__ inline void jg_match_set(const JgDev& d, JgLane& L, uint32_t r, uint64_t v) {
  const uint64_t f = jg_lag_encode(v, L.mbase, d.R);
  if (jg_lag_wide(f, d.R)) d.match_wide[(size_t)r * d.G + L.g] = v;
  L.mword = jg_lag_with(L.mword, r, d.R, f);
}
__device__ inline void jg_match_rebase(const JgDev& d, JgLane& L, uint64_t base) {
  uint64_t w = 0;
  for (uint32_t r = 0; r < d.R; r++) {
    const uint64_t v = jg_match_get(d, L, r);
    const uint64_t f = jg_lag_encode(v, base, d.R);
    if (jg_lag_wide(f, d.R)) d.match_wide[(size_t)r * d.G + L.g] = v;
    w = jg_lag_with(w, r, d.R, f);
  }
  L.mword = w;
  L.mbase = base;
}

__device__ inline void jg_load(const JgDev& d, JgLane& L, uint32_t g) {
  L.g = g;
  L.flags = d.flags[g];
  L.term = d.term[g];
  L.head = d.head[g];
  L.id_gen = (L.flags & JGF_FAST) ? L.head + 1 : d.id_gen[g];
  L.run_hi = (L.flags & JGF_RUN) ? L.head : d.run_hi[g];
  L.heartbeat_time = d.heartbeat_time[g];
  {
    const JgCold c = jg_cold_load(d.cold, g);
    L.election_time = c.election_time, L.voted_for = c.voted_for, L.leader_id = c.leader_id;
    L.election_timeout = c.election_timeout, L.rng_draws = c.rng_draws, L.queued = c.queued, L.votes = c.votes;
  }
  L.mword = 0;
  L.mbase = jg_lane_base(L);
  if ((L.flags & JGF_ROLE_MASK) == JG_ROLE_LEADER) {
    L.mword = d.mlag[g];
    const uint64_t fc = jg_lag_field(L.mword, d.R, d.R);
    L.commit = jg_lag_wide(fc, d.R) ? d.commit[g] : L.mbase - fc;
  } else {
    L.commit = d.commit[g];
  }
  L.decisions = 0;
  L.overflow = 0;
  L.xq_on = 0;
  L.xq_k = 0;
}
template <bool CHAIN = true>
__device__ inline void jg_store(const JgDev& d, JgLane& L) {
  uint32_t g = L.g;
  if (CHAIN && jg_wcnt(L)) jg_chain_normalize(d, L);
  const bool run = (L.run_hi == L.head) && (jg_wcnt(L) == 0) && !(L.flags & JGF_NO_GENESIS);
  const bool fast = run && (L.id_gen == L.head + 1);
  L.flags = run ? (L.flags | JGF_RUN) : (L.flags & ~JGF_RUN);
  L.flags = fast ? (L.flags | JGF_FAST) : (L.flags & ~JGF_FAST);
  if (!fast && jg_role(L) == JG_ROLE_LEADER && !jg_fault(L)) *d.irregular_seen = 1;
  if (jg_role(L) == JG_ROLE_LEADER) {
    const uint64_t base = jg_lane_base(L);
    if (L.mbase != base) jg_match_rebase(d, L, base);
    const uint64_t fc = jg_lag_encode(L.commit, base, d.R);
    if (jg_lag_wide(fc, d.R)) d.commit[g] = L.commit;
    d.mlag[g] = jg_lag_with(L.mword, d.R, d.R, fc);
  } else {
    d.commit[g] = L.commit;
  }
  d.flags[g] = L.flags;
  d.term[g] = L.term;
  d.head[g] = L.head;
  d.id_gen[g] = L.id_gen;
  d.run_hi[g] = L.run_hi;
  d.heartbeat_time[g] = L.heartbeat_time;
  jg_cold_store(d.cold, g, jg_cold_of(L.election_time, L.voted_for, L.leader_id, L.election_timeout, L.rng_draws, L.queued, L.votes));
}

__device__ inline int jg_slot_of(const JgDev& d, uint32_t node_id);

template <bool CHAIN = true>
__device__ inline void jg_store_dirty(const JgDev& d, JgLane& L, const JgLane& O) {
  if (jg_role(L) != jg_role(O)) {
    jg_store<CHAIN>(d, L);
    return;
  }
  const uint32_t g = L.g;
  if (CHAIN && jg_wcnt(L)) jg_chain_normalize(d, L);
  const bool run = (L.run_hi == L.head) && (jg_wcnt(L) == 0) && !(L.flags & JGF_NO_GENESIS);
  const bool fast = run && (L.id_gen == L.head + 1);
  L.flags = run ? (L.flags | JGF_RUN) : (L.flags & ~JGF_RUN);
  L.flags = fast ? (L.flags | JGF_FAST) : (L.flags & ~JGF_FAST);
  if (!fast && jg_role(L) == JG_ROLE_LEADER && !jg_fault(L)) *d.irregular_seen = 1;
  if (jg_role(L) == JG_ROLE_LEADER) {
    const uint64_t base = jg_lane_base(L);
    if (L.mbase != base) jg_match_rebase(d, L, base);
    const uint64_t fc = jg_lag_encode(L.commit, base, d.R);
    if (jg_lag_wide(fc, d.R)) d.commit[g] = L.commit;
    const uint64_t w = jg_lag_with(L.mword, d.R, d.R, fc);
    if (w != O.mword) d.mlag[g] = w;
  } else if (L.commit != O.commit) {
    d.commit[g] = L.commit;
  }
  if (L.flags != O.flags) d.flags[g] = L.flags;
  if (L.term != O.term) d.term[g] = L.term;
  if (L.head != O.head) d.head[g] = L.head;
  if (!fast && (L.id_gen != O.id_gen || (O.flags & JGF_FAST))) d.id_gen[g] = L.id_gen;
  if (!run && (L.run_hi != O.run_hi || (O.flags & JGF_RUN))) d.run_hi[g] = L.run_hi;
  if (L.heartbeat_time != O.heartbeat_time) d.heartbeat_time[g] = L.heartbeat_time;
  if (L.election_time != O.election_time || L.voted_for != O.voted_for || L.leader_id != O.leader_id ||
      L.election_timeout != O.election_timeout || L.rng_draws != O.rng_draws || L.queued != O.queued || L.votes != O.votes)
    jg_cold_store(d.cold, g, jg_cold_of(L.election_time, L.voted_for, L.leader_id, L.election_timeout, L.rng_draws, L.queued, L.votes));
}

__device__ inline void jg_emit_msg(const JgDev& d, JgLane& L, uint8_t kind, uint8_t to_kind, uint32_t to_id,
                                   uint8_t flag, uint64_t term, uint64_t id, uint64_t aux) {
  if (!L.xq_on && L.mp >= L.mend) {
    L.overflow = 1;
    return;
  }
  if (L.xq_on == 2) {
    if (kind == JG_CMD_APPEND_RESPONSE) {
      L.cap_ack = id;
      return;
    }
    if (kind == JG_CMD_HEARTBEAT_RESPONSE) {
      L.cap_hbc = id;
      L.cap_has = flag;
      return;
    }
  }
  if (L.xq_on == 3) {
    if (kind == JG_CMD_HEARTBEAT) {
      L.cap_hbc = id;
      return;
    }
    if (kind == JG_CMD_APPEND_ENTRIES) {
      const int r = jg_slot_of(d, to_id);
      if (r >= 0) L.cap_ae[(size_t)r * d.G + L.g] = JG_AE(id, aux);
      return;
    }
  }
  if (L.xq_on == 4 && kind == JG_CMD_VOTE_RESPONSE && to_kind == JG_TO_PEER && id == 0 && aux == 0 && L.xq_k < 256u) {
    const int to = jg_slot_of(d, to_id);
    const uint32_t n = (uint32_t)L.cap_hbc & 0xffu;
    if (to >= 0 && !n) {
      L.cap_ack = term;
      L.cap_hbc = 1u | L.xq_k << 8 | (uint32_t)(flag & 1u) << 19 | (uint32_t)to << 21;
      L.xq_k++;
      return;
    }
    if (to >= 0 && (uint32_t)to == (((uint32_t)L.cap_hbc >> 21) & 7u) && term == L.cap_ack && L.xq_k == (((uint32_t)L.cap_hbc >> 8) & 0xffu) + n && n < 255u &&
        (n == 1u || (uint32_t)(flag & 1u) == (((uint32_t)L.cap_hbc >> 20) & 1u))) {
      L.cap_hbc = (((uint32_t)L.cap_hbc & ~(1u << 20)) | (uint32_t)(flag & 1u) << 20) + 1u;
      L.xq_k++;
      return;
    }
  }
  jg_msg_row r;
  r.group = L.g;
  r.kind = kind;
  r.to_kind = to_kind;
  r.flag = flag;
  r.pad = 0;
  r.to_id = to_id;
  r.from = jg_self_id(d, L);
  r.term = term;
  r.id = id;
  r.aux = aux;
  if (L.xq_on) {
    const uint32_t i = atomicAdd(d.xq_n, 1u);
    if (i < d.xq_cap) {
      JgXqRec q;
      q.row = r;
      q.seq = L.seq;
      q.k = L.xq_k++;
      d.xq[i] = q;
    }
    return;
  }
  *L.mp++ = r;
}
__device__ inline void jg_emit_fsm(JgLane& L, uint8_t kind, uint64_t a, uint64_t b) {
  if (L.fp >= L.fend) {
    L.overflow = 1;
    return;
  }
  jg_fsm_row r;
  r.group = L.g;
// ... 535 lines not shown
```

josefine_amd/csrc/jg_follower.h:

```cpp
#pragma once
#include "jg_dense.h"

struct JgFollowerArgs {
  const uint32_t* leader;
  uint32_t leader_id;
  const jg_leader_beat* beat;
  const uint64_t* ae;
  const uint64_t* aec;
  uint64_t* o_answer;
  uint64_t* o_hbc;
  uint64_t now;
  uint32_t seq;
  uint32_t tick;
  const JgClock* clock;
  uint32_t clock_slot, pad_;
  uint32_t* fsm_delta;
  uint64_t* fsm_prev;
  const uint8_t* owner;
  uint32_t self_slot;
  uint32_t seq_off;
  const uint64_t* sparse_bits;
  uint32_t sparse_mode, pad3_;
};
__device__ __forceinline__ uint32_t jg_member_id(const JgDev& d, uint32_t slot) {
  uint32_t id = 0;
#pragma unroll
  for (uint32_t r = 0; r < JG_MAX_REPLICAS; r++) id = r == slot ? d.node_ids[r] : id;
  return id;
}
__device__ __forceinline__ void jg_follower_fsm_note(const JgFollowerArgs& a, uint32_t g, uint64_t commit0, uint64_t commit1) {
  if (!a.fsm_delta || commit1 == commit0) return;
  const uint64_t adv = commit1 - commit0;
  if (adv <= JG_FSM_ADV_MASK) {
    a.fsm_delta[g] = JG_FSM_FOLLOWER_BIT | (uint32_t)adv;
  } else {
    a.fsm_prev[g] = commit0;
    a.fsm_delta[g] = JG_FSM_FOLLOWER_BIT | JG_FSM_WIDE_BIT;
  }
}

template <bool ANY = false>
__device__ __forceinline__ void jg_follower_fast_body(const JgDev& d, JgFollowerArgs a) {
  if (a.clock) jg_clock_read(a.clock, a.clock_slot, a.now, a.seq), a.seq += a.seq_off;
  const uint32_t G = d.G;
  for (uint32_t g = blockIdx.x * JG_BLOCK + threadIdx.x; g < G; g += gridDim.x * JG_BLOCK) {
    if (a.sparse_bits && jg_sparse_skip(a.sparse_bits, a.sparse_mode, g)) continue;
    const uint32_t f = d.flags[g];
    uint32_t own = 0;
    if (ANY) {
      own = a.owner[g];
      if (__ballot(!((f & JGF_ROLE_MASK) == JG_ROLE_LEADER && own == a.self_slot)) == 0) continue;
    }
    const bool mail = !ANY || (own != JG_OWNER_NONE && own != a.self_slot);
    jg_leader_beat beat = a.beat[g];
    uint64_t in_ae = jg_ae_word_for(a.aec, a.ae, g);
    if (ANY && !mail) beat = jg_leader_beat{0, JG_NO_ACK}, in_ae = JG_NO_ACK;
    const uint64_t in_term = beat.term, in_hbc = beat.hb_commit;
    const uint64_t in_from = in_ae >> 8;
    const uint32_t in_n = (uint32_t)in_ae & 0xffu;
    const uint32_t lead = ANY ? jg_member_id(d, own) : (a.leader ? a.leader[g] : a.leader_id);
    uint64_t term = d.term[g], head = d.head[g], commit = d.commit[g];
    const JgCold cold0 = jg_cold_load(d.cold, g);
    uint32_t voted_for = cold0.voted_for, leader_id = cold0.leader_id;
    const uint32_t queued = cold0.queued;
    uint32_t draws = cold0.rng_draws;
    uint64_t et = cold0.election_time;
    uint32_t eto = cold0.election_timeout;
    const bool has_hb = in_hbc != JG_NO_ACK, has_ae = in_n != JG_AE_NONE;

    const uint32_t role = f & JGF_ROLE_MASK;
    const bool dead = (f & JGF_FAULT_MASK) != 0;
    const bool idle_leader = role == JG_ROLE_LEADER && !has_ae;
    const bool fired = (a.now - et) > (uint64_t)eto;
    const bool quiet = !has_hb && !has_ae &&
                       ((role == JG_ROLE_FOLLOWER && (!fired || (f & JGF_VOTED))) || (role == JG_ROLE_CANDIDATE && !fired));
    const bool nothing = (!has_hb && !has_ae && !a.tick) || quiet;
    const bool fast = role == JG_ROLE_FOLLOWER && (f & JGF_RUN) && queued == 0;
    const bool defer = !dead && !idle_leader && !nothing && !fast;
    jg_defer_mark_in(d.fdefer_bits, d, g, defer);
    if (dead || idle_leader || nothing || defer) {
      if (!(ANY && idle_leader && own == a.self_slot)) a.o_answer[g] = JG_NO_ACK;
      continue;
    }
    uint64_t o_ack = JG_MAILBOX_NONE;
    uint32_t o_has = JG_HB_NONE;

    uint32_t nf = f;
    const uint64_t term0 = term, head0 = head, commit0 = commit;
    const uint32_t vf0 = voted_for, lid0 = leader_id;
    bool timer_dirty = false;
    uint32_t fault = 0;

    if (has_hb) {
      const uint32_t span = d.el_max - d.el_min;
      const uint64_t r = jg_mix64(d.seed ^ jg_mix64((d.group_base + g) * 0xd1342543de82ef95ull + draws));
      eto = d.el_min + (span ? (uint32_t)(r % span) : 0u);
      et = a.now;
      draws += 1;
      timer_dirty = true;
      term = in_term;
      nf |= JGF_HAS_LEADER | JGF_VOTED;
      leader_id = lead;
      voted_for = lead;
      const bool has = in_hbc <= head;
      if (has && in_hbc > commit) {
        commit = in_hbc;
        nf |= JGF_COMMIT_KEY;
      }
      a.o_hbc[g] = commit;
      o_has = has ? 1 : 0;
    }
    if (has_ae) {
      if (!(nf & JGF_VOTED) && in_term >= term) {
        term = in_term;
        et = a.now;
        timer_dirty = true;
        nf |= JGF_HAS_LEADER | JGF_VOTED;
        leader_id = lead;
        voted_for = lead;
      }
      if ((nf & JGF_VOTED) && voted_for != lead && in_term < term) {
        fault = JG_FAULT_FOLLOWER_STALE_LEADER;
      } else if (in_n) {
        if (in_from > head) {
          fault = JG_FAULT_EXTEND_MISSING_PARENT;
        } else {
          const uint64_t new_head = in_from + in_n;
          const uint64_t run_hi = new_head > head ? new_head : head;
          if (nf & JGF_FAST) {
            d.id_gen[g] = head + 1;
            nf &= ~JGF_FAST;
          }
          head = new_head;
          if (head != run_hi) {
            d.run_hi[g] = run_hi;
            nf &= ~JGF_RUN;
          }
          if (head >= JG_MAILBOX_NONE) fault = JG_FAULT_ENGINE_MAILBOX_RANGE;
          else o_ack = head;
        }
      }
    }
    bool tick_defer = false;
    if (a.tick && !fault) {
      tick_defer = (a.now - et) > (uint64_t)eto && !(nf & JGF_VOTED);
    }
    if (fault) {
      nf |= fault << JGF_FAULT_SHIFT;
      jg_push_fault(d, g, fault, a.seq);
    }
    a.o_answer[g] = JG_ANSWER(o_ack, o_has);
    if (term != term0) d.term[g] = term;
    if (head != head0) d.head[g] = head;
    if (commit != commit0) d.commit[g] = commit;
    jg_follower_fsm_note(a, g, commit0, commit);
    {
      const JgCold c = jg_cold_of(et, voted_for, leader_id, eto, draws, queued, cold0.votes);
      if (timer_dirty) jg_cold_store_timer(d.cold, g, c);
      if (voted_for != vf0 || leader_id != lid0) jg_cold_store_rest(d.cold, g, c);
    }
    if (nf != f) d.flags[g] = nf;
    jg_defer_mark_in(d.fdefer_bits + (G + 63u) / 64u, d, g, tick_defer);
  }
}

__global__ __launch_bounds__(JG_BLOCK) void k_follower_tick_dense(JgDev d, JgFollowerArgs a) { jg_follower_fast_body<false>(d, a); }

struct JgFollowerJob {
  JgDev d;
  JgFollowerArgs a;
};
__global__ __launch_bounds__(JG_BLOCK) JG_FOLLOWER_OCC void k_follower_tick_dense_multi(const JgFollowerJob* __restrict__ jobs) {
  const JgFollowerJob& j = jobs[blockIdx.y];
  jg_follower_fast_body<false>(j.d, j.a);
}
__global__ __launch_bounds__(JG_BLOCK) void k_follower_tick_dense_any(const JgFollowerJob* __restrict__ jobs) {
  const JgFollowerJob& j = jobs[blockIdx.y];
  jg_follower_fast_body<true>(j.d, j.a);
}

__device__ __forceinline__ void jg_follower_slow_body(const JgDev& d, JgFollowerArgs a) {
  if (a.clock) jg_clock_read(a.clock, a.clock_slot, a.now, a.seq), a.seq += a.seq_off;
  uint32_t dec = 0;
  __shared__ uint32_t s_n;
  if (threadIdx.x == 0) s_n = 0;
  __syncthreads();
  uint32_t* list = d.slow_list + (size_t)blockIdx.x * d.slow_cap;
  {
    const uint32_t n_words = (d.G + 63u) / 64u;
    const uint32_t wpb = (n_words + gridDim.x - 1) / gridDim.x;
    const uint32_t w0 = blockIdx.x * wpb, w1 = w0 + wpb < n_words ? w0 + wpb : n_words;
    for (uint32_t w = w0 + threadIdx.x; w < w1; w += JG_BLOCK) {
      uint64_t m = d.fdefer_bits[w], mt = d.fdefer_bits[n_words + w];
      if (!(m | mt)) continue;
      if (m) d.fdefer_bits[w] = 0;
      if (mt) d.fdefer_bits[n_words + w] = 0;
      uint32_t at = atomicAdd(&s_n, (uint32_t)(__popcll(m) + __popcll(mt)));
      for (int pass = 0; pass < 2; pass++) {
        uint64_t b = pass ? mt : m;
        for (; b; b &= b - 1, at++) {
          const uint32_t g = w * 64u + (uint32_t)__ffsll((long long)b) - 1u;
          if (at < d.slow_cap) list[at] = g | (pass ? JG_DEFER_TICK_ONLY : 0u);
          else *d.err = 4;
        }
      }
    }
  }
  __syncthreads();
  const uint32_t n = s_n < d.slow_cap ? s_n : d.slow_cap;
  for (uint32_t i = threadIdx.x; i < n; i += JG_BLOCK) {
    const uint32_t entry = list[i];
    const uint32_t g = entry & ~JG_DEFER_TICK_ONLY;
    const bool tick_only = (entry & JG_DEFER_TICK_ONLY) != 0;
    JgLane L;
    jg_load(d, L, g);
    const uint64_t fsm_commit0 = L.commit;
    const bool was_leader = jg_role(L) == JG_ROLE_LEADER;
    L.now = a.now;
    L.seq = a.seq;
    L.mp = L.mend = nullptr;
    jg_fsm_row sink[2];
    L.xq_on = 2;
    L.cap_ack = JG_NO_ACK;
    L.cap_hbc = 0;
    L.cap_has = JG_HB_NONE;
    const uint32_t own = a.owner ? a.owner[g] : 0u;
    const bool mail = !a.owner || (own != JG_OWNER_NONE && own != a.self_slot);
    const uint32_t lead = a.owner ? jg_member_id(d, own) : (a.leader ? a.leader[g] : a.leader_id);
    JgCmd c;
    c.from = lead;
    c.flag = 0;
    c.term = a.beat[g].term;
    c.aux = 0;
    if (!tick_only) {
      const uint64_t hbc = mail ? a.beat[g].hb_commit : JG_NO_ACK;
      const uint64_t ae = mail ? jg_ae_word_for(a.aec, a.ae, g) : JG_NO_ACK;
// ... 48 lines not shown
```

josefine_amd/csrc/jg_isr.h:

```cpp
#pragma once
#include "jg_device.h"
#include "jg_read.h"
#include "jg_sparse.h"
#include "jg_watch.h"

#define JG_ISR_ROWS 4u
#define JG_ISR_TILE (JG_BLOCK * JG_ISR_ROWS)
#define JG_ISR_SHADOW_LEADS 0x100u
#define JG_REPL_CENSUS_ROWS 4u
#define JG_REPL_CENSUS_TILE (JG_BLOCK * JG_REPL_CENSUS_ROWS)
#define JG_REPL_CENSUS_PARTS 1024u

#define JG_RC_OUT_OF_SYNC 4u
#define JG_RC_MAX_LAG (JG_RC_OUT_OF_SYNC + JG_MAX_REPLICAS)
#define JG_RC_SUM_LAG (JG_RC_MAX_LAG + JG_MAX_REPLICAS)
#define JG_RC_MAX_UNCOMMITTED (JG_RC_SUM_LAG + JG_MAX_REPLICAS)
#define JG_RC_WORDS (JG_RC_MAX_UNCOMMITTED + 1u)
static_assert(sizeof(jg_repl_census) == JG_RC_WORDS * 8, "jg_repl_census is the census words in order");
static_assert(sizeof(jg_isr_row) == 24, "jg_isr_row is three 8-byte pieces");
__host__ __device__ __forceinline__ bool jg_rc_is_max(uint32_t x) {
  return (x >= JG_RC_MAX_LAG && x < JG_RC_SUM_LAG) || x == JG_RC_MAX_UNCOMMITTED;
}

__device__ __forceinline__ bool jg_isr_leads(uint32_t f) { return (f & (JGF_ROLE_MASK | JGF_FAULT_MASK)) == JG_ROLE_LEADER; }

__device__ __forceinline__ uint64_t jg_isr_lag_exact(const JgDev& d, uint32_t g, uint64_t field, uint32_t r, uint64_t base, uint64_t head) {
  const uint64_t match = jg_lag_wide(field, d.R) ? d.match_wide[(size_t)r * d.G + g] : base - field;
  return head > match ? head - match : 0ull;
}

__device__ __forceinline__ uint32_t jg_isr_word(const JgDev& d, uint64_t leave, uint64_t join, uint32_t leave32, uint32_t join32, uint32_t g,
                                                uint32_t f, uint64_t w, uint32_t sh) {
  if (!jg_isr_leads(f)) return 0u;
  const uint32_t R = d.R, self = (f & JGF_SELF_MASK) >> JGF_SELF_SHIFT;
  const uint32_t was = (sh & JG_ISR_SHADOW_LEADS) ? (sh & 0xffu) : 0u;
  const uint32_t behind = (uint32_t)jg_lag_behind(R);
  const bool run = jg_lag_base_is_run_hi(f);
  uint32_t isr = 1u << self, rare = 0;
#pragma unroll
  for (uint32_t r = 0; r < JG_MAX_REPLICAS; r++) {
    if (r < R && r != self) {
      const uint32_t field = (uint32_t)jg_lag_field(w, r, R);
      const bool stays = (was >> r) & 1u;
      const uint32_t thr = stays ? leave32 : join32;
      if (!run && field < behind)
        isr |= (field <= thr ? 1u : 0u) << r;
      else if (!run && field == behind && (stays ? leave : join) < (uint64_t)behind)
        ;
      else
        rare |= 1u << r;
    }
  }
  if (rare) {
    const uint64_t head = d.head[g], base = run ? d.run_hi[g] : head;
#pragma unroll
    for (uint32_t r = 0; r < JG_MAX_REPLICAS; r++) {
      if ((rare >> r) & 1u) {
        const uint64_t lag = jg_isr_lag_exact(d, g, jg_lag_field(w, r, R), r, base, head);
        isr |= (lag <= (((was >> r) & 1u) ? leave : join) ? 1u : 0u) << r;
      }
    }
  }
  return isr | JG_ISR_SHADOW_LEADS;
}

__device__ __forceinline__ uint64_t jg_isr_worst_lag(const JgDev& d, uint32_t g, uint32_t f, uint64_t w, uint64_t head) {
  const uint32_t R = d.R, self = (f & JGF_SELF_MASK) >> JGF_SELF_SHIFT;
  const bool run = jg_lag_base_is_run_hi(f);
  const uint64_t base = run ? d.run_hi[g] : head;
  uint64_t worst = 0;
#pragma unroll
  for (uint32_t r = 0; r < JG_MAX_REPLICAS; r++) {
    if (r < R && r != self) {
      const uint64_t field = jg_lag_field(w, r, R);
      const uint64_t lag = (!run && !jg_lag_wide(field, R)) ? field : jg_isr_lag_exact(d, g, field, r, base, head);
      worst = lag > worst ? lag : worst;
    }
  }
  return worst;
}

struct JgIsrArgs {
  uint32_t g0, n;
  uint32_t add;
  uint32_t peek;
  uint64_t leave_lag, join_lag;
  uint32_t* shadow;
  uint32_t* cnt;
  uint64_t* bsum;
  jg_isr_row* out;
  uint64_t cap;
  const uint32_t* gate;
};

__device__ __forceinline__ void jg_isr_ballots(const JgDev& d, const JgIsrArgs& a, uint32_t* v, uint32_t* f, uint64_t* w, uint64_t* m) {
  const uint32_t t0 = blockIdx.x * JG_ISR_TILE + threadIdx.x;
  const uint32_t leave32 = jg_clamp32(a.leave_lag), join32 = jg_clamp32(a.join_lag);
  uint32_t sh[JG_ISR_ROWS];
#pragma unroll
  for (uint32_t k = 0; k < JG_ISR_ROWS; k++) {
    const uint32_t i = t0 + k * JG_BLOCK;
    const bool in = i < a.n;
    const uint32_t g = a.g0 + (in ? i : 0u);
    f[k] = in ? d.flags[g] : 0u;
    w[k] = in ? d.mlag[g] : 0ull;
    sh[k] = in ? a.shadow[g] : 0u;
  }
#pragma unroll
  for (uint32_t k = 0; k < JG_ISR_ROWS; k++) {
    const uint32_t i = t0 + k * JG_BLOCK;
    const bool in = i < a.n;
    v[k] = in ? jg_isr_word(d, a.leave_lag, a.join_lag, leave32, join32, a.g0 + i, f[k], w[k], sh[k]) : 0u;
    m[k] = __ballot(in && v[k] != sh[k]);
  }
}

__global__ __launch_bounds__(JG_BLOCK) void k_isr_count(JgDev d, JgIsrArgs a) {
  uint32_t v[JG_ISR_ROWS], f[JG_ISR_ROWS];
  uint64_t w[JG_ISR_ROWS], m[JG_ISR_ROWS];
  jg_isr_ballots(d, a, v, f, w, m);
  uint32_t c = 0;
#pragma unroll
  for (uint32_t k = 0; k < JG_ISR_ROWS; k++) c += __popcll(m[k]);
  const uint32_t t = jg_tile_count(c);
  if (threadIdx.x == 0) a.cnt[blockIdx.x] = t, a.bsum[blockIdx.x] = t;
}

template <class A>
__device__ __forceinline__ void jg_isr_write_rows(const JgDev& d, const A& a, uint64_t base, const uint32_t* v, const uint32_t* f, const uint64_t* w,
                                                  const uint64_t* m) {
  const uint32_t peek = jg_gated_peek(a.peek, a.gate);
  const uint32_t lane = threadIdx.x & 63u;
  const uint32_t t0 = blockIdx.x * JG_ISR_TILE + threadIdx.x;
  uint64_t head[JG_ISR_ROWS];
#pragma unroll
  for (uint32_t k = 0; k < JG_ISR_ROWS; k++)
    head[k] = (((m[k] >> lane) & 1ull) && v[k]) ? d.head[a.g0 + t0 + k * JG_BLOCK] : 0ull;
  const uint32_t R = d.R;
  uint64_t* out64 = (uint64_t*)a.out;
  jg_ranked_rows<JG_ISR_ROWS>(m, base, a.cap, [&](uint32_t k, uint64_t pos) {
    const uint32_t g = a.g0 + t0 + k * JG_BLOCK;
    const uint32_t self = (f[k] & JGF_SELF_MASK) >> JGF_SELF_SHIFT;
    uint32_t isr = 0, replicate = 0, state = 0;
    uint64_t worst = 0;
    if (v[k]) {
      isr = v[k] & 0xffu;
      const uint32_t in_sync = (uint32_t)__popcll((uint64_t)isr);
      replicate = (f[k] & JGF_REPL_MASK) >> JGF_REPL_SHIFT;
      state = JG_ISR_LEADS | (in_sync < R ? (uint32_t)JG_ISR_UNDER : 0u) | (in_sync < R / 2u + 1u ? (uint32_t)JG_ISR_BELOW_QUORUM : 0u);
      worst = jg_isr_worst_lag(d, g, f[k], w[k], head[k]);
    }
    out64[pos * 3 + 0] = (uint64_t)(a.add + g) | (uint64_t)(isr | replicate << 8 | state << 16 | self << 24) << 32;
    out64[pos * 3 + 1] = head[k];
    out64[pos * 3 + 2] = worst;
    if (!peek) a.shadow[g] = v[k];
  });
}

__global__ __launch_bounds__(JG_BLOCK) void k_isr_write(JgDev d, JgIsrArgs a) {
  const uint64_t base = a.bsum[blockIdx.x];
  if (a.cnt[blockIdx.x] == 0 || base >= a.cap) return;
  uint32_t v[JG_ISR_ROWS], f[JG_ISR_ROWS];
  uint64_t w[JG_ISR_ROWS], m[JG_ISR_ROWS];
  jg_isr_ballots(d, a, v, f, w, m);
  jg_isr_write_rows(d, a, base, v, f, w, m);
}

struct JgReplCensusArgs {
  uint32_t g0, n;
  uint32_t tiles;
  uint32_t parts;
  uint64_t lag_limit;
  uint64_t* part;
  uint64_t* out;
};

__global__ __launch_bounds__(JG_BLOCK) void k_repl_census(JgDev d, JgReplCensusArgs a) {
  const uint32_t R = d.R;
  uint32_t c[JG_RC_MAX_LAG];
#pragma unroll
  for (uint32_t x = 0; x < JG_RC_MAX_LAG; x++) c[x] = 0;
  uint64_t max_lag[JG_MAX_REPLICAS], sum_lag[JG_MAX_REPLICAS], max_unc = 0;
#pragma unroll
  for (uint32_t r = 0; r < JG_MAX_REPLICAS; r++) max_lag[r] = 0, sum_lag[r] = 0;
  for (uint32_t tile = blockIdx.x; tile < a.tiles; tile += a.parts) {
    const uint32_t t0 = tile * JG_REPL_CENSUS_TILE + threadIdx.x;
    uint32_t f[JG_REPL_CENSUS_ROWS];
    uint64_t w[JG_REPL_CENSUS_ROWS];
#pragma unroll
    for (uint32_t k = 0; k < JG_REPL_CENSUS_ROWS; k++) {
      const uint32_t i = t0 + k * JG_BLOCK;
      const bool in = i < a.n;
      const uint32_t g = a.g0 + (in ? i : 0u);
      f[k] = in ? d.flags[g] : 0u;
      w[k] = in ? d.mlag[g] : 0ull;
    }
#pragma unroll
    for (uint32_t k = 0; k < JG_REPL_CENSUS_ROWS; k++) {
      const uint32_t i = t0 + k * JG_BLOCK;
      const uint32_t g = a.g0 + (i < a.n ? i : 0u);
      const bool led = i < a.n && jg_isr_leads(f[k]);
      const uint32_t self = (f[k] & JGF_SELF_MASK) >> JGF_SELF_SHIFT;
      uint64_t lag[JG_MAX_REPLICAS], unc = 0;
#pragma unroll
      for (uint32_t r = 0; r < JG_MAX_REPLICAS; r++) lag[r] = 0;
      if (led) {
        const bool run = jg_lag_base_is_run_hi(f[k]);
        const uint64_t fc = jg_lag_field(w[k], R, R);
        bool rare = run || jg_lag_wide(fc, R);
#pragma unroll
        for (uint32_t r = 0; r < JG_MAX_REPLICAS; r++) {
          if (r < R && r != self) {
            lag[r] = jg_lag_field(w[k], r, R);
            rare = rare || jg_lag_wide(lag[r], R);
          }
        }
        unc = fc;
        if (rare) {
          const uint64_t head = d.head[g], base = run ? d.run_hi[g] : head;
#pragma unroll
          for (uint32_t r = 0; r < JG_MAX_REPLICAS; r++)
            if (r < R && r != self) lag[r] = jg_isr_lag_exact(d, g, lag[r], r, base, head);
          unc = head - jg_read_commit(d, g, f[k]);
        }
      }
      uint32_t in_sync = 1;
#pragma unroll
      for (uint32_t r = 0; r < JG_MAX_REPLICAS; r++) {
        if (r < R) {
          const bool member = led && r != self;
          const bool out = member && lag[r] > a.lag_limit;
          in_sync += member && !out ? 1u : 0u;
          c[JG_RC_OUT_OF_SYNC + r] += __popcll(__ballot(out));
          max_lag[r] = lag[r] > max_lag[r] ? lag[r] : max_lag[r];
          sum_lag[r] += lag[r];
        }
      }
      c[0] += __popcll(__ballot(led));
      c[1] += __popcll(__ballot(led && in_sync == R));
      c[2] += __popcll(__ballot(led && in_sync < R));
      c[3] += __popcll(__ballot(led && in_sync < R / 2u + 1u));
      max_unc = unc > max_unc ? unc : max_unc;
    }
  }
  uint64_t vals[JG_RC_WORDS];
#pragma unroll
  for (uint32_t x = 0; x < JG_RC_MAX_LAG; x++) vals[x] = c[x];
#pragma unroll
  for (uint32_t r = 0; r < JG_MAX_REPLICAS; r++) {
    vals[JG_RC_MAX_LAG + r] = jg_wave_max64(max_lag[r]);
    vals[JG_RC_SUM_LAG + r] = jg_wave_sum64(sum_lag[r]);
  }
  vals[JG_RC_MAX_UNCOMMITTED] = jg_wave_max64(max_unc);
  jg_block_words<JG_RC_WORDS>(vals, [](uint32_t x) { return jg_rc_is_max(x); }, a.part);
}

__global__ __launch_bounds__(JG_BLOCK) void k_repl_census_sum(JgReplCensusArgs a) {
  jg_parts_reduce<JG_RC_WORDS>(a.part, a.parts, a.out, [](uint32_t x) { return jg_rc_is_max(x); });
}
```

josefine_amd/csrc/jg_kernels.h:

```cpp
#pragma once
#include "jg_device.h"

#include "jg_dense.h"

template <bool NODE>
__device__ __forceinline__ void jg_dense_slow_body(const JgDev& d, const uint64_t* __restrict__ acks, uint32_t n_ticks,
                                                   size_t tick_stride, uint32_t seq0, JgLeaderNode nd, bool advance_clock) {
  if (nd.clock) jg_clock_read(nd.clock, nd.clock_slot, nd.now, seq0);
  uint32_t dec = 0;
  __shared__ uint32_t s_n;
  if (threadIdx.x == 0) s_n = 0;
  __syncthreads();
  uint32_t* list = d.slow_list + (size_t)blockIdx.x * d.slow_cap;
  {
    const uint32_t n_words = (d.G + 63u) / 64u;
    const uint32_t wpb = (n_words + gridDim.x - 1) / gridDim.x;
    const uint32_t w0 = blockIdx.x * wpb, w1 = w0 + wpb < n_words ? w0 + wpb : n_words;
    for (uint32_t w = w0 + threadIdx.x; w < w1; w += JG_BLOCK) {
      uint64_t m = d.defer_bits[w];
      if (!m) continue;
      d.defer_bits[w] = 0;
      uint32_t at = atomicAdd(&s_n, (uint32_t)__popcll(m));
      while (m) {
        const uint32_t b = (uint32_t)__ffsll((long long)m) - 1u;
// ... 279 lines not shown
        const uint32_t lane = t & 63u;
        const int first = __ffsll((long long)m) - 1;
        uint32_t base = 0;
        if ((int)lane == first) base = atomicAdd(out_n, (uint32_t)__popcll(m));
        base = __shfl(base, first, 64);
        if (remove) {
          const uint32_t at = base + (uint32_t)__popcll(m & ((1ull << lane) - 1ull));
          if (at < out_cap) out[at] = JgCompactRow{g, i, top};
          changed = true;
          const uint32_t ix = s_ix[i][t];
          if (ix == 0) {
            if (top == 0) L.flags |= JGF_NO_GENESIS;
            else L.run_hi = top - 1;
          } else if (hi == lo) {
            drop_mask |= 1u << (ix - 1);
          } else {
            d.win_hi[(size_t)(ix - 1) * d.G + g] = hi - 1;
          }
        }
      }
      if (visit) {
        have_next = true;
        next_id = s_nx[i][t];
      }
    }
    if (!changed) continue;
    if (drop_mask) {
      uint32_t k = 0;
      for (uint32_t w = 0; w < nw; w++) {
        if ((drop_mask >> w) & 1u) continue;
        if (k != w) {
          JG_SEG(win_lo, k) = JG_SEG(win_lo, w);
          JG_SEG(win_hi, k) = JG_SEG(win_hi, w);
          JG_SEG(win_next, k) = JG_SEG(win_next, w);
        }
        k++;
      }
      L.flags = (L.flags & ~JGF_WIN_MASK) | (k << JGF_WIN_SHIFT);
    }
    jg_store(d, L);
  }
}

__device__ __forceinline__ uint64_t jg_synth_hash(uint64_t seed, uint64_t tick, uint64_t gg, uint32_t r) {
  return jg_mix64(jg_mix64(seed + tick * 0x9e3779b97f4a7c15ull) ^ (gg * 8 + r));
}
__global__ void k_synth_acks(JgDev d, uint32_t mode, uint64_t tick, uint64_t* __restrict__ sim,
                             uint64_t* __restrict__ acks) {
  const uint32_t G = d.G, R = d.R;
  for (uint32_t g = blockIdx.x * blockDim.x + threadIdx.x; g < G; g += gridDim.x * blockDim.x) {
    const uint32_t s = (d.flags[g] & JGF_SELF_MASK) >> JGF_SELF_SHIFT;
    const uint64_t gg = d.group_base + g;
    const uint64_t lead = sim[(size_t)s * G + g];
    const uint64_t n_app = mode == 0 ? 1 : jg_synth_hash(d.seed, tick, gg, s) % 3;
    acks[(size_t)s * G + g] = n_app;
    sim[(size_t)s * G + g] = lead + n_app;
    for (uint32_t r = 0; r < R; r++) {
      if (r == s) continue;
      const size_t k = (size_t)r * G + g;
      if (mode == 0) {
        acks[k] = lead;
        sim[k] = lead;
      } else {
        const uint64_t u = jg_synth_hash(d.seed, tick, gg, r);
        const uint32_t p = (uint32_t)(u % 100);
        if (p < 5) {
          acks[k] = JG_NO_ACK;
        } else if (p < 10) {
          acks[k] = sim[k];
        } else {
          const uint64_t adv = (u >> 32) % (JG_MAX_INFLIGHT + 1);
          uint64_t v = sim[k] + adv;
          v = v < lead ? v : lead;
          acks[k] = v;
          sim[k] = v;
        }
      }
    }
  }
}

template <int R>
__global__ __launch_bounds__(JG_BLOCK) void k_stream_calib(const uint64_t* __restrict__ rot,
                                                            const uint64_t* __restrict__ a8, uint64_t* b8,
                                                            const uint32_t* __restrict__ c4, uint32_t G) {
  for (uint32_t g = blockIdx.x * JG_BLOCK + threadIdx.x; g < G; g += gridDim.x * JG_BLOCK) {
    uint64_t v[R];
#pragma unroll
    for (int r = 0; r < R; r++) v[r] = __builtin_nontemporal_load(&rot[(size_t)r * G + g]);
    uint64_t s = a8[g] ^ b8[g] ^ c4[g];
#pragma unroll
    for (int r = 0; r < R; r++) s += v[r];
    b8[g] = s;
  }
}

__global__ void k_init_groups(JgDev d, const uint8_t* __restrict__ self_slots) {
  for (uint32_t g = blockIdx.x * blockDim.x + threadIdx.x; g < d.G; g += gridDim.x * blockDim.x) {
    JgLane L;
    L.g = g;
    L.now = 0;
    L.seq = 0;
    L.mp = L.mend = nullptr;
    L.fp = L.fend = nullptr;
    L.overflow = 0;
    L.xq_on = 0;
    L.xq_k = 0;
    L.decisions = 0;
    L.term = 0;
    L.mword = 0;
    L.mbase = 0;
    L.commit = L.head = 0;
    L.id_gen = 1;
    L.run_hi = 0;
    L.heartbeat_time = 0;
    L.voted_for = L.leader_id = L.queued = L.votes = 0;
    L.rng_draws = 0;
    uint32_t s = self_slots ? self_slots[g] : 0;
    L.flags = JG_ROLE_FOLLOWER | (s << JGF_SELF_SHIFT);
    if (d.cfg_flags & JG_CFG_START_VACANT) {
      L.flags |= JG_FAULT_VACANT << JGF_FAULT_SHIFT;
      L.election_time = 0;
      L.election_timeout = 0;
    } else {
      jg_set_election_timeout(d, L);
    }
    d.mlag[g] = 0;
    jg_store(d, L);
  }
}
```

josefine_amd/csrc/jg_lookup.h:

```cpp
#pragma once
#include "jg_device.h"
#include "jg_read.h"
#include "jg_watch.h"

static_assert(sizeof(jg_group_state) == 80, "jg_group_state is five 16-byte pieces");

typedef uint32_t jg_u32x4 __attribute__((ext_vector_type(4)));

struct JgLookupArgs {
  uint32_t g0, n;
  const uint32_t* list;
  uint32_t add;
  uint32_t pad;
  uint4* out;
  uint64_t* match;
  uint32_t* err;
};

template <int R>
__global__ __launch_bounds__(JG_BLOCK) void k_lookup(JgDev d, JgLookupArgs a) {
  const uint32_t i = blockIdx.x * JG_BLOCK + threadIdx.x;
  if (i >= a.n) return;
  const uint32_t g = a.list ? a.list[i] : a.g0 + i;
  if (g >= d.G) {
    *a.err = 1u;
    return;
  }
  const uint32_t f = d.flags[g];
  const uint64_t term = d.term[g], head = d.head[g], commit = d.commit[g], w = d.mlag[g], run_hi = d.run_hi[g], id_gen = d.id_gen[g],
                 hbt = d.heartbeat_time[g];
  const uint4 ct = d.cold.t[g], cv = d.cold.v[g];
  const uint32_t role = f & JGF_ROLE_MASK, fault = (f & JGF_FAULT_MASK) >> JGF_FAULT_SHIFT, self = (f & JGF_SELF_MASK) >> JGF_SELF_SHIFT;
  const bool leader = role == JG_ROLE_LEADER, knows = role == JG_ROLE_FOLLOWER && (f & JGF_HAS_LEADER);
  const JgLeadView v = jg_lead_view(d, f, term, cv.y);
  const uint64_t commit_now = jg_read_commit(d, g, f);
  asm volatile("" ::"v"(f), "v"(term), "v"(head), "v"(commit), "v"(w), "v"(run_hi), "v"(id_gen), "v"(hbt));
  asm volatile("" ::"v"(ct.x), "v"(ct.y), "v"(ct.z), "v"(cv.x), "v"(cv.y), "v"(cv.z), "v"(cv.w));
  const uint64_t idg = (f & JGF_FAST) ? head + 1 : id_gen;
  const uint64_t hb = leader ? hbt : 0ull;
  const uint32_t voted_for = (f & JGF_VOTED) ? cv.x : 0u, leader_id = knows ? cv.y : 0u;
  const uint32_t votes = role == JG_ROLE_CANDIDATE ? cv.w : 0u;
  const uint32_t repl = leader ? (f & JGF_REPL_MASK) >> JGF_REPL_SHIFT : 0u;
  const uint32_t has = ((f & JGF_VOTED) ? 1u : 0u) | (knows ? 2u : 0u);
  const uint32_t b0 = role | ((v.meta >> 8) & 0xffu) << 8 | fault << 16 | self << 24;
  const uint32_t b1 = repl | (votes & 0xffu) << 8 | ((votes >> 8) & 0xffu) << 16 | has << 24;
  auto lo = [](uint64_t x) { return (uint32_t)x; };
  auto hi = [](uint64_t x) { return (uint32_t)(x >> 32); };
  jg_u32x4* o = (jg_u32x4*)(a.out + (size_t)i * 5);
  o[0] = jg_u32x4{a.add + g, v.leader_id, lo(term), hi(term)};
  o[1] = jg_u32x4{lo(head), hi(head), lo(commit_now), hi(commit_now)};
  o[2] = jg_u32x4{lo(idg), hi(idg), ct.x, ct.y};
  o[3] = jg_u32x4{lo(hb), hi(hb), voted_for, leader_id};
  o[4] = jg_u32x4{ct.z, cv.z, b0, b1};
  if (a.match) {
    const uint64_t base = jg_lag_base_is_run_hi(f) ? run_hi : head;
    uint64_t* m = a.match + (size_t)i * R;
#pragma unroll
    for (uint32_t r = 0; r < (uint32_t)R; r++) {
      const uint64_t field = jg_lag_field(w, r, R);
      m[r] = !leader ? 0ull : jg_lag_wide(field, R) ? d.match_wide[(size_t)r * d.G + g] : base - field;
    }
  }
}

__global__ __launch_bounds__(JG_BLOCK) void k_lookup_check(uint32_t G, const uint32_t* list, uint64_t n, uint32_t* err) {
  for (uint64_t i = (uint64_t)blockIdx.x * JG_BLOCK + threadIdx.x; i < n; i += (uint64_t)gridDim.x * JG_BLOCK)
    if (list[i] >= G) *err = 1u;
}
```

josefine_amd/csrc/jg_move.h:

```cpp
#pragma once
#include "jg_device.h"

#define JG_MOVE_TILE 64u
#define JG_MOVE_W_TERM 1u
#define JG_MOVE_W_FLAGS 8u
#define JG_MOVE_W_COLD 9u
#define JG_MOVE_W_FVOTE 13u
#define JG_MOVE_W_WIN (JG_MOVE_W_FVOTE + JG_FOREIGN_VOTERS / 2u)
#define JG_MOVE_W_MATCH (JG_MOVE_W_WIN + 3u * JG_CHAIN_WINDOW)
#define JG_MOVE_ROWS_FIXED (JG_MOVE_W_MATCH + 1u)
#define JG_MOVE_KEY 0x6a6f73656d6f7665ull
static_assert(JG_BLOCK == 4 * JG_MOVE_TILE, "jg_move_check: four lanes per record of a tile");
static_assert(JG_FOREIGN_VOTERS == 8, "the record holds fvote_id[8] in words 13-16");
static_assert(JG_CHAIN_WINDOW == 8 && JG_MAX_REPLICAS == 8, "the record layout of DESIGN.md \"Handing groups over\"");

__host__ __device__ __forceinline__ uint32_t jg_move_words(uint32_t R) { return (JG_MOVE_W_MATCH + R + 7u) & ~7u; }

__device__ __forceinline__ uint64_t jg_move_term(uint64_t w, uint32_t k) { return jg_mix64(w ^ (uint64_t)k * 0x9e3779b97f4a7c15ull); }

struct JgMoveArgs {
  uint32_t g0, n;
  uint64_t shift;
  uint4* out;
  const uint4* in;
  uint32_t* err;
};

template <uint32_t NW>
struct JgMoveTileLds {
  static constexpr uint32_t P = 2 * NW + 1;
  uint32_t s[JG_MOVE_TILE * P];
};

template <uint32_t NW, bool EXPORT>
__device__ __forceinline__ void jg_move_row(const JgDev& d, uint32_t* s, uint32_t row, uint32_t i, uint32_t g, uint64_t shift) {
  uint32_t* w = s + i * JgMoveTileLds<NW>::P;
  const size_t G = d.G;
  uint64_t* col = nullptr;
  uint32_t k = 0;
  if (row < 7u) {
    col = row == 0 ? d.term : row == 1 ? d.commit : row == 2 ? d.head : row == 3 ? d.id_gen : row == 4 ? d.run_hi : row == 5 ? d.mlag : d.heartbeat_time;
    col += g, k = JG_MOVE_W_TERM + row;
  } else if (row == 7u) {
    if (EXPORT) w[2 * JG_MOVE_W_FLAGS] = d.flags[g], w[2 * JG_MOVE_W_FLAGS + 1] = 0u;
    else d.flags[g] = w[2 * JG_MOVE_W_FLAGS];
    return;
  } else if (row < 10u) {
    uint4* c = (row == 8u ? d.cold.t : d.cold.v) + g;
    uint32_t* q = w + 2 * (JG_MOVE_W_COLD + 2u * (row - 8u));
    if (EXPORT) {
      const uint4 v = *c;
      q[0] = v.x, q[1] = v.y, q[2] = v.z, q[3] = v.w;
    } else {
      uint64_t t = (uint64_t)q[0] | (uint64_t)q[1] << 32;
      if (row == 8u) t += shift;
      *c = make_uint4((uint32_t)t, (uint32_t)(t >> 32), q[2], q[3]);
    }
    return;
  } else if (row < 10u + JG_FOREIGN_VOTERS) {
    uint32_t* c = d.fvote_id + (size_t)(row - 10u) * G + g;
    uint32_t* q = w + 2 * JG_MOVE_W_FVOTE + (row - 10u);
    if (EXPORT) *q = *c;
    else *c = *q;
    return;
  } else if (row < 10u + JG_FOREIGN_VOTERS + 3u * JG_CHAIN_WINDOW) {
    const uint32_t r = row - 10u - JG_FOREIGN_VOTERS, a = r / JG_CHAIN_WINDOW, x = r % JG_CHAIN_WINDOW;
    col = (a == 0 ? d.win_lo : a == 1 ? d.win_hi : d.win_next) + (size_t)x * G + g, k = JG_MOVE_W_WIN + r;
  } else {
    const uint32_t r = row - JG_MOVE_ROWS_FIXED;
    col = d.match_wide + (size_t)r * G + g, k = JG_MOVE_W_MATCH + r;
  }
  if (EXPORT) {
    const uint64_t v = *col;
    w[2 * k] = (uint32_t)v, w[2 * k + 1] = (uint32_t)(v >> 32);
  } else {
    uint64_t v = (uint64_t)w[2 * k] | (uint64_t)w[2 * k + 1] << 32;
    if (k == JG_MOVE_W_TERM + 6u) v += shift;
    *col = v;
  }
}

template <uint32_t NW>
__device__ __forceinline__ uint64_t jg_move_check(const uint32_t* s) {
  const uint32_t i = threadIdx.x >> 2, part = threadIdx.x & 3u;
  const uint32_t* w = s + i * JgMoveTileLds<NW>::P;
  uint64_t c = part == 0 ? jg_mix64(JG_MOVE_KEY ^ NW) : 0ull;
  for (uint32_t k = 1 + part; k < NW; k += 4) c ^= jg_move_term((uint64_t)w[2 * k] | (uint64_t)w[2 * k + 1] << 32, k);
  uint32_t lo = (uint32_t)c, hi = (uint32_t)(c >> 32);
  lo ^= __shfl_xor(lo, 1, 64), hi ^= __shfl_xor(hi, 1, 64);
  lo ^= __shfl_xor(lo, 2, 64), hi ^= __shfl_xor(hi, 2, 64);
  return (uint64_t)lo | (uint64_t)hi << 32;
}

template <uint32_t NW>
__device__ __forceinline__ void jg_move_tile_in(uint32_t* s, const uint4* in, uint32_t nt) {
  constexpr uint32_t C = NW / 2, P = JgMoveTileLds<NW>::P;
  for (uint32_t c = threadIdx.x; c < nt * C; c += JG_BLOCK) {
    const uint4 v = in[c];
    uint32_t* q = s + (c / C) * P + (c % C) * 4;
    q[0] = v.x, q[1] = v.y, q[2] = v.z, q[3] = v.w;
  }
}

template <uint32_t NW>
__global__ __launch_bounds__(JG_BLOCK) void k_export_groups(JgDev d, JgMoveArgs a) {
  __shared__ JgMoveTileLds<NW> t;
  constexpr uint32_t P = JgMoveTileLds<NW>::P, C = NW / 2;
  const uint32_t t0 = blockIdx.x * JG_MOVE_TILE, nt = min(JG_MOVE_TILE, a.n - t0);
  const uint32_t rows = JG_MOVE_ROWS_FIXED + d.R;
  for (uint32_t k = threadIdx.x; k < rows * JG_MOVE_TILE; k += JG_BLOCK) {
    const uint32_t row = k / JG_MOVE_TILE, i = k % JG_MOVE_TILE;
    if (i < nt) jg_move_row<NW, true>(d, t.s, row, i, a.g0 + t0 + i, 0);
  }
  for (uint32_t k = threadIdx.x; k < (NW - JG_MOVE_W_MATCH - d.R) * JG_MOVE_TILE; k += JG_BLOCK) {
    const uint32_t i = k % JG_MOVE_TILE, q = 2 * (JG_MOVE_W_MATCH + d.R + k / JG_MOVE_TILE);
    t.s[i * P + q] = 0u, t.s[i * P + q + 1] = 0u;
  }
  __syncthreads();
  const uint64_t c = jg_move_check<NW>(t.s);
  if ((threadIdx.x & 3u) == 0) {
    uint32_t* w = t.s + (threadIdx.x >> 2) * P;
    w[0] = (uint32_t)c, w[1] = (uint32_t)(c >> 32);
  }
  __syncthreads();
  uint4* out = a.out + (size_t)t0 * C;
  for (uint32_t k = threadIdx.x; k < nt * C; k += JG_BLOCK) {
    const uint32_t* q = t.s + (k / C) * P + (k % C) * 4;
    out[k] = make_uint4(q[0], q[1], q[2], q[3]);
// ... 59 lines not shown
```

josefine_amd/csrc/jg_node.h:

```cpp
#pragma once
#include "jg_device.h"
#include "jg_sparse.h"

#define JGN_ACK_SHIFT 0
#define JGN_HBR_SHIFT 8
#define JGN_HB (1u << 16)
#define JGN_AE (1u << 17)
#define JGN_CR (1u << 18)
#define JGN_SPARSE (1u << 31)
#define JGN_PRE_SHIFT (8 + JG_NODE_PRE_SHIFT)

#define JGN_FSM_APPENDED JG_FSM_APPENDED_BIT
#define JGN_FSM_WIDE JG_FSM_WIDE_BIT
#define JGN_FSM_FOLLOWER JG_FSM_FOLLOWER_BIT
#define JGN_FSM_ADV_MASK JG_FSM_ADV_MASK

struct JgNodeCols {
  uint64_t* answers;
  uint64_t* hbr_commit;
  uint64_t* token;
  jg_leader_beat* f_beat;
  uint64_t* f_ae;
  uint32_t* f_leader;
  uint32_t* cls;
// ... 523 lines not shown
        atomicAnd((unsigned long long*)&T.answers[s][q], (unsigned long long)(~0xffull | has));
        if (!has) c.hbr_commit[(size_t)s * G + g0 + q] = row.id;
        break;
      }
      case JG_CMD_CLIENT_REQUEST:
        atomicOr((unsigned long long*)&T.answers[selfq][q], 1ull << 8);
        T.token[q] = row.id;
        break;
      case JG_CMD_HEARTBEAT:
        if (FOLLOWER) F[0].f_beat[q] = jg_leader_beat{row.term, row.id}, F[0].f_leader[q] = row.from;
        break;
      default: {
        uint64_t from = 0;
        (void)jg_node_ae_run(a, row.id, row.aux, &from);
        if (FOLLOWER) {
          F[0].f_ae[q] = JG_AE(from, row.aux);
          if (!(w & JGN_HB)) {
            F[0].f_beat[q].term = row.term;
            F[0].f_leader[q] = row.from;
          }
        }
      }
    }
  }
  __syncthreads();
  if (live) {
    c.fsm_delta[g] = 0;
    if (leader_half) {
#pragma unroll
      for (int r = 0; r < R; r++)
        if ((uint32_t)r == self || !((col_mask >> r) & 1u)) c.answers[(size_t)r * G + g] = T.answers[r][p];
#pragma unroll
      for (int r = 0; r < 2 * R; r++) c.arr[(size_t)r * G + g] = T.arr[r][p];
      c.token[g] = T.token[p];
    }
    if (follower_half) c.f_beat[g] = F[0].f_beat[p], c.f_ae[g] = F[0].f_ae[p], c.f_leader[g] = F[0].f_leader[p];
  }
  if (p < JGN_TILE / 64 && g0 + p * 64u < G) c.sparse_bits[(g0 >> 6) + p] = T.sparse[p];
}
#endif

struct JgNodeSorted {
  uint32_t* group;
  uint8_t* kind;
  uint32_t* from;
  uint64_t* term;
  uint64_t* id;
  uint64_t* aux;
  uint8_t* flag;
};
__global__ __launch_bounds__(JG_BLOCK) void k_node_gather_rows(uint32_t n, const uint32_t* __restrict__ order, JgNodeRows a,
                                                               JgNodeSorted o) {
  const uint32_t p = blockIdx.x * JG_BLOCK + threadIdx.x;
  if (p >= n) return;
  const uint32_t i = order[p];
  o.group[p] = a.group[i];
  o.kind[p] = (uint8_t)a.kind_of(i);
  o.from[p] = a.from_of(i);
  o.term[p] = a.term_of(i);
  o.id[p] = a.id_of(i);
  o.aux[p] = a.aux_of(i);
  o.flag[p] = a.flag_of(i);
}

#define JGN_FSM_ROWS 3
__device__ __forceinline__ uint64_t jg_node_commit_of(const JgDev& d, uint32_t g, uint32_t f, uint64_t head) {
  if ((f & JGF_ROLE_MASK) != JG_ROLE_LEADER) return d.commit[g];
  const uint64_t fc = jg_lag_field(d.mlag[g], d.R, d.R);
  if (jg_lag_wide(fc, d.R)) return d.commit[g];
  return (jg_lag_base_is_run_hi(f) ? d.run_hi[g] : head) - fc;
}
__device__ __forceinline__ void jg_node_fsm_row(jg_fsm_row& r, uint32_t g, uint32_t kind, uint64_t a, uint64_t b) {
  r.group = g, r.kind = (uint8_t)kind, r.pad[0] = r.pad[1] = r.pad[2] = 0;
  r.a = a, r.b = b;
}
__global__ __launch_bounds__(JG_BLOCK) void k_node_fsm_build(JgDev d, JgNodeCols c, jg_fsm_row* __restrict__ out,
                                                             uint32_t* __restrict__ cnt, uint64_t* __restrict__ bsum, uint32_t fused) {
  const uint32_t g = blockIdx.x * JG_BLOCK + threadIdx.x;
  uint32_t n = 0;
  if (g < d.G) {
    const uint32_t w = c.fsm_delta[g];
    if (w) {
      const uint32_t f = d.flags[g];
      const uint64_t head = d.head[g];
      const uint64_t commit1 = jg_node_commit_of(d, g, f, head);
      const bool fol = (w & JGN_FSM_FOLLOWER) != 0;
      uint64_t commit0, mid;
      if (w & JGN_FSM_WIDE) {
        commit0 = c.fsm_prev[g];
        mid = fol ? commit0 : c.fsm_mid[g];
      } else {
        commit0 = commit1 - (w & JGN_FSM_ADV_MASK);
        mid = commit0 + ((w >> JG_FSM_PRE_SHIFT) & JGN_FSM_ADV_MASK);
      }
      jg_fsm_row* r = out + (size_t)g * JGN_FSM_ROWS;
      if (fol) {
        if (commit1 != commit0) jg_node_fsm_row(r[n++], g, JG_FSM_APPLY_FOLLOWER, commit0, commit1);
      } else if (fused && (w & JGN_FSM_APPENDED) && head >= commit1 && head - commit0 <= 255u && commit0 <= mid && mid <= commit1) {
        jg_fsm_row& o = r[n++];
        o.group = g, o.kind = (uint8_t)JG_FSM_LEADER_STEP;
        o.pad[0] = (uint8_t)(head - commit0), o.pad[1] = (uint8_t)(head - mid), o.pad[2] = (uint8_t)(head - commit1);
        o.a = head, o.b = c.token[g];
      } else {
        if (mid != commit0) jg_node_fsm_row(r[n++], g, JG_FSM_APPLY_LEADER, commit0, mid);
        if (w & JGN_FSM_APPENDED) jg_node_fsm_row(r[n++], g, JG_FSM_NOTIFY, head, c.token[g]);
        if (commit1 != mid) jg_node_fsm_row(r[n++], g, JG_FSM_APPLY_LEADER, mid, commit1);
      }
    }
    cnt[g] = n;
  }
  uint32_t tot;
  (void)jg_block_exclusive_scan(n, &tot);
  if (threadIdx.x == 0) bsum[blockIdx.x] = tot;
}

__global__ __launch_bounds__(JG_BLOCK) void k_node_count_individual(const uint64_t* __restrict__ aec, uint32_t G, uint32_t* __restrict__ count) {
  uint32_t n = 0;
  for (uint32_t g = blockIdx.x * JG_BLOCK + threadIdx.x; g < G; g += gridDim.x * JG_BLOCK) n += aec[g] == JG_AEC_INDIVIDUAL;
  uint32_t tot;
  (void)jg_block_exclusive_scan(n, &tot);
  if (threadIdx.x == 0 && tot) atomicAdd(count, tot);
}
```

josefine_amd/csrc/jg_poll.h:

```cpp
#pragma once
#include "jg_commits.h"
#include "jg_isr.h"
#include "jg_isr_clock.h"
#include "jg_watch.h"

static_assert(JG_WATCH_TILE == JG_ISR_TILE && JG_ISR_TILE == JG_CMT_TILE, "the three write passes index one tiling");
#define JG_POLL_ROWS JG_CMT_ROWS
#define JG_POLL_TILE JG_CMT_TILE
static_assert(JG_ISR_TILE == JG_POLL_TILE, "k_isrc_write (jg_isr_clock.h) indexes the tiling of the timed pass");
#define JG_POLL_FLIGHT 4u
static_assert(JG_POLL_ROWS % JG_POLL_FLIGHT == 0, "a tile is whole passes");

struct JgPollArgs {
  uint32_t tiles;
  uint32_t parts;
  JgWatchArgs lw;
  JgIsrArgs ir;
  JgCommitArgs cm;
  JgIsrClockArgs ic;
};

template <bool L, bool I, bool C, bool T>
__device__ __forceinline__ void jg_poll_rows(const JgDev& d, const JgPollArgs& a, uint32_t g0, uint32_t n, uint32_t tile, uint32_t k0,
                                             uint32_t leave32, uint32_t join32, uint32_t lane, bool advance, uint32_t* c, uint32_t* bc,
                                             uint64_t& commits, uint64_t& appends) {
  static_assert(I || !T, "the time rule is the replicas part's");
  const uint32_t t0 = tile * JG_POLL_TILE + k0 * JG_BLOCK + threadIdx.x;
  uint32_t f[JG_POLL_FLIGHT], ish[JG_POLL_FLIGHT], mk[JG_POLL_FLIGHT];
  uint64_t term[JG_POLL_FLIGHT], w[JG_POLL_FLIGHT], head[JG_POLL_FLIGHT], col[JG_POLL_FLIGHT];
  uint4 cold[JG_POLL_FLIGHT], lsh[JG_POLL_FLIGHT], csh[JG_POLL_FLIGHT];
#pragma unroll
  for (uint32_t k = 0; k < JG_POLL_FLIGHT; k++) {
    const uint32_t i = t0 + k * JG_BLOCK;
    const bool in = i < n;
    const uint32_t g = g0 + (in ? i : 0u);
    f[k] = in ? d.flags[g] : 0u;
    if (L) {
      term[k] = in ? d.term[g] : 0ull;
      cold[k] = in ? d.cold.v[g] : make_uint4(0, 0, 0, 0);
      lsh[k] = in ? a.lw.shadow[g] : make_uint4(0, 0, 0, 0);
    }
    if (I || C) w[k] = in ? d.mlag[g] : 0ull;
    if (I) ish[k] = in ? (T ? a.ic.shadow : a.ir.shadow)[g] : 0u;
    if (T) mk[k] = in ? (uint32_t)a.ic.mask[g] & ((1u << d.R) - 1u) : 0u;
    if (C) {
      head[k] = in ? d.head[g] : 0ull;
      col[k] = in ? d.commit[g] : 0ull;
      csh[k] = in ? a.cm.shadow[g] : make_uint4(0, 0, 0, 0);
    }
  }
#pragma unroll
  for (uint32_t k = 0; k < JG_POLL_FLIGHT; k++) {
    asm volatile("" ::"v"(f[k]));
    if (L) asm volatile("" ::"v"(term[k]), "v"(cold[k].y), "v"(lsh[k].x), "v"(lsh[k].z));
    if (I || C) asm volatile("" ::"v"(w[k]));
    if (I) asm volatile("" ::"v"(ish[k]));
    if (T) asm volatile("" ::"v"(mk[k]));
    if (C) asm volatile("" ::"v"(head[k]), "v"(col[k]), "v"(csh[k].x), "v"(csh[k].z));
  }
#pragma unroll
  for (uint32_t k = 0; k < JG_POLL_FLIGHT; k++) {
    const uint32_t i = t0 + k * JG_BLOCK;
    const bool in = i < n;
    if (L)
      c[0] += __popcll(__ballot(in && jg_lead_differs(lsh[k], jg_lead_view(d, f[k], term[k], cold[k].y))));
    if (I && !T) {
      const uint32_t v = in ? jg_isr_word(d, a.ir.leave_lag, a.ir.join_lag, leave32, join32, g0 + i, f[k], w[k], ish[k]) : 0u;
      c[1] += __popcll(__ballot(in && v != ish[k]));
    }
    if (T) {
      const uint32_t v = in ? jg_isrc_word(d, a.ic, leave32, join32, g0 + i, f[k], w[k], ish[k], mk[k], advance) : 0u;
      c[1] += __popcll(__ballot(in && v != ish[k]));
    }
    if (C) {
      const uint64_t cm = jg_commit_view(d, g0 + (in ? i : 0u), f[k], w[k], head[k], col[k]);
      const uint64_t m = __ballot(in && jg_commit_differs(csh[k], cm, head[k], a.cm.commits_only));
      c[2] += __popcll(m);
      if (a.cm.backlog) jg_commit_backlog_add((m >> lane) & 1ull, m, csh[k], cm, head[k], bc, commits, appends);
    }
  }
}

template <bool L, bool I, bool C, bool T>
__device__ __forceinline__ void jg_poll_count_body(const JgDev& d, const JgPollArgs& a) {
  const uint32_t lane = threadIdx.x & 63u;
  const uint32_t g0 = T ? a.ic.g0 : L ? a.lw.g0 : a.ir.g0, n = T ? a.ic.n : L ? a.lw.n : a.ir.n;
  const uint32_t leave32 = jg_clamp32(T ? a.ic.caught_lag : a.ir.leave_lag), join32 = jg_clamp32(T ? a.ic.join_lag : a.ir.join_lag);
  const bool advance = T && !jg_gated_peek(a.ic.peek, a.ic.gate);
  uint32_t bc[4] = {0u, 0u, 0u, 0u};
  uint64_t commits = 0, appends = 0;
  for (uint32_t tile = blockIdx.x; tile < a.tiles; tile += a.parts) {
    uint32_t c[3] = {0u, 0u, 0u};
#pragma unroll
    for (uint32_t k0 = 0; k0 < JG_POLL_ROWS; k0 += JG_POLL_FLIGHT)
      jg_poll_rows<L, I, C, T>(d, a, g0, n, tile, k0, leave32, join32, lane, advance, c, bc, commits, appends);
    const uint32_t t = jg_tile_counts<3>(c);
    if (threadIdx.x < 3) {
      const uint32_t x = threadIdx.x;
      if (L && x == 0) a.lw.cnt[tile] = t, a.lw.bsum[tile] = t;
      if (I && x == 1) (T ? a.ic.cnt : a.ir.cnt)[tile] = t, (T ? a.ic.bsum : a.ir.bsum)[tile] = t;
      if (C && x == 2) a.cm.cnt[tile] = t, a.cm.bsum[tile] = t;
    }
    __syncthreads();
  }
  if (!C || !a.cm.backlog) return;
  const uint64_t vals[JG_CMT_WORDS] = {bc[0], bc[1], bc[2], bc[3], jg_wave_sum64(commits), jg_wave_sum64(appends)};
  jg_block_words<JG_CMT_WORDS>(vals, JgNeverMax(), a.cm.part);
}

template <bool L, bool I, bool C>
__global__ __launch_bounds__(JG_BLOCK) void k_poll_count(JgDev d, JgPollArgs a) {
  jg_poll_count_body<L, I, C, false>(d, a);
}

template <bool L, bool C>
__global__ __launch_bounds__(JG_BLOCK) void k_poll_count_timed(JgDev d, JgPollArgs a) {
  static_assert(L || C, "a timed replicas part wanted alone is k_isrc_count's");
  jg_poll_count_body<L, true, C, true>(d, a);
}

#define JG_PH_TOTAL 0u
#define JG_PH_GIVEN 3u
#define JG_PH_BACKLOG 6u
#define JG_PH_CENSUS (JG_PH_BACKLOG + JG_CMT_WORDS)
#define JG_PH_REPL (JG_PH_CENSUS + JG_CENSUS_WORDS)
#define JG_PH_GATE (JG_PH_REPL + JG_RC_WORDS)
#define JG_PH_WORDS (JG_PH_GATE + 1u)
static_assert(JG_PH_WORDS <= JG_BLOCK, "one thread a word");

// ... 32 lines not shown
```

josefine_amd/csrc/jg_read.h:

```cpp
#pragma once
#include "jg_device.h"
#include "jg_sparse.h"

#define JG_READ_ITEMS 8u
#define JG_READ_TILE (JG_BLOCK * JG_READ_ITEMS)
#define JG_READ_PIECE (1ull << 24)
#define JG_READ_SEGS (1u + JG_CHAIN_WINDOW)

struct JgReadArgs {
  uint32_t n;
  uint32_t g0;
  uint64_t row_base;
  const uint64_t* from;
  uint64_t* commit;
  uint8_t* has_commit;
  uint8_t* fault;
  uint64_t* bsum_r;
  uint64_t* bsum_s;
  uint64_t* total;
  uint64_t* off;
  uint64_t* seg_lo;
  uint64_t* seg_nx;
  uint64_t* seg_row;
  uint32_t* err;
};

struct JgReadSegs {
  uint64_t lo[JG_READ_SEGS], hi[JG_READ_SEGS], nx[JG_READ_SEGS];
  bool ok[JG_READ_SEGS];
  uint32_t n;
  uint64_t rows;
};

__device__ __forceinline__ void jg_read_cx(JgReadSegs& s, uint32_t a, uint32_t b) {
  const bool swap = s.ok[b] && (!s.ok[a] || s.lo[b] < s.lo[a]);
  if (swap) {
    const uint64_t l = s.lo[a], h = s.hi[a], x = s.nx[a];
    const bool o = s.ok[a];
    s.lo[a] = s.lo[b], s.hi[a] = s.hi[b], s.nx[a] = s.nx[b], s.ok[a] = s.ok[b];
    s.lo[b] = l, s.hi[b] = h, s.nx[b] = x, s.ok[b] = o;
  }
}

__device__ inline uint32_t jg_read_decode(const JgDev& d, uint32_t g, uint64_t from, JgReadSegs& s) {
  const uint32_t flags = d.flags[g];
  const uint32_t fault = (flags & JGF_FAULT_MASK) >> JGF_FAULT_SHIFT;
  const uint32_t wn = fault >= 128u ? 0u : (flags & JGF_WIN_MASK) >> JGF_WIN_SHIFT;
  const uint64_t run_hi = (flags & JGF_RUN) ? d.head[g] : d.run_hi[g];
  s.lo[0] = 0, s.hi[0] = run_hi, s.nx[0] = 0;
  s.ok[0] = fault < 128u && !(flags & JGF_NO_GENESIS);
#pragma unroll
  for (uint32_t w = 0; w < JG_CHAIN_WINDOW; w++) {
    const bool ok = w < wn;
    const size_t at = (size_t)w * d.G + g;
    s.lo[1 + w] = ok ? d.win_lo[at] : 0;
    s.hi[1 + w] = ok ? d.win_hi[at] : 0;
    s.nx[1 + w] = ok ? d.win_next[at] : 0;
    s.ok[1 + w] = ok;
  }
#pragma unroll
  for (uint32_t k = 0; k < JG_READ_SEGS; k++) {
    if (s.hi[k] < from) s.ok[k] = false;
    if (s.lo[k] < from) s.lo[k] = from, s.nx[k] = from - 1;
  }
#pragma unroll
  for (uint32_t r = 0; r < JG_CHAIN_WINDOW; r++) {
#pragma unroll
    for (uint32_t a = 1 + (r & 1u); a + 1 < JG_READ_SEGS; a += 2) jg_read_cx(s, a, a + 1);
  }
  s.n = 0;
  s.rows = 0;
#pragma unroll
  for (uint32_t k = 0; k < JG_READ_SEGS; k++)
    if (s.ok[k]) s.n++, s.rows += s.hi[k] - s.lo[k] + 1;
  return flags;
}

__device__ __forceinline__ uint64_t jg_read_commit(const JgDev& d, uint32_t g, uint32_t flags) {
  if ((flags & JGF_ROLE_MASK) != JG_ROLE_LEADER) return d.commit[g];
  const uint64_t fc = jg_lag_field(d.mlag[g], d.R, d.R);
  if (jg_lag_wide(fc, d.R)) return d.commit[g];
  return (jg_lag_base_is_run_hi(flags) ? d.run_hi[g] : d.head[g]) - fc;
}

__device__ __forceinline__ uint64_t jg_block_exclusive_scan64(uint64_t v, uint64_t* total) {
  __shared__ uint64_t wave_tot64[JG_BLOCK / 64];
  const uint32_t lane = threadIdx.x & 63u, wave = threadIdx.x >> 6;
  uint64_t inc = v;
#pragma unroll
  for (int off = 1; off < 64; off <<= 1) {
    const uint64_t up = __shfl_up(inc, off, 64);
    if (lane >= (uint32_t)off) inc += up;
  }
  if (lane == 63) wave_tot64[wave] = inc;
  __syncthreads();
  uint64_t base = 0, tot = 0;
#pragma unroll
  for (uint32_t w = 0; w < JG_BLOCK / 64; w++) {
    base += w < wave ? wave_tot64[w] : 0ull;
    tot += wave_tot64[w];
  }
  __syncthreads();
  *total = tot;
  return base + inc - v;
}

__global__ __launch_bounds__(JG_BLOCK) void k_read_groups(JgDev d, JgReadArgs a) {
  const uint32_t i = blockIdx.x * JG_BLOCK + threadIdx.x;
  uint64_t rows = 0;
  uint32_t nseg = 0;
  if (i < a.n) {
    const uint32_t g = a.g0 + i;
    JgReadSegs s;
    const uint32_t flags = jg_read_decode(d, g, a.from ? a.from[i] : 0, s);
    const uint32_t fault = (flags & JGF_FAULT_MASK) >> JGF_FAULT_SHIFT;
    const bool has = fault < 128u && (flags & JGF_COMMIT_KEY);
    a.commit[i] = has ? jg_read_commit(d, g, flags) : 0;
    a.has_commit[i] = has ? 1 : 0;
    a.fault[i] = (uint8_t)fault;
    rows = s.rows;
    nseg = s.n;
  }
  uint64_t tot_r;
  uint32_t tot_s;
  (void)jg_block_exclusive_scan64(rows, &tot_r);
  (void)jg_block_exclusive_scan(nseg, &tot_s);
  if (threadIdx.x == 0) {
    a.bsum_r[blockIdx.x] = tot_r;
    a.bsum_s[blockIdx.x] = tot_s;
    if (tot_r >> 32) atomicOr(a.err, 1u);
  }
}

__global__ __launch_bounds__(JG_BLOCK) void k_read_segs(JgDev d, JgReadArgs a) {
  const uint32_t i = blockIdx.x * JG_BLOCK + threadIdx.x;
  JgReadSegs s;
  s.n = 0;
  s.rows = 0;
  if (i < a.n) (void)jg_read_decode(d, a.g0 + i, a.from ? a.from[i] : 0, s);
  uint64_t tot_r;
  uint32_t tot_s;
  uint64_t row = a.bsum_r[blockIdx.x] + jg_block_exclusive_scan64(s.rows, &tot_r);
  const uint64_t sb = a.bsum_s[blockIdx.x] + jg_block_exclusive_scan(s.n, &tot_s);
  if (i >= a.n) return;
  a.off[i] = a.row_base + row;
  uint64_t at = sb;
#pragma unroll
  for (uint32_t k = 0; k < JG_READ_SEGS; k++)
    if (s.ok[k]) {
      a.seg_lo[at] = s.lo[k];
      a.seg_nx[at] = s.nx[k];
      a.seg_row[at] = row;
      at++;
      row += s.hi[k] - s.lo[k] + 1;
    }
}

__global__ __launch_bounds__(JG_BLOCK) void k_read_rows(const uint64_t* __restrict__ seg_lo, const uint64_t* __restrict__ seg_nx,
                                                        const uint64_t* __restrict__ seg_row, uint64_t nseg, uint64_t r0,
                                                        uint64_t nr, uint64_t* __restrict__ out_id, uint64_t* __restrict__ out_nx) {
  __shared__ uint64_t l_id[JG_BLOCK * (JG_READ_ITEMS + 1)], l_nx[JG_BLOCK * (JG_READ_ITEMS + 1)];
  const uint64_t tile = (uint64_t)blockIdx.x * JG_READ_TILE;
  const uint64_t first = tile + (uint64_t)threadIdx.x * JG_READ_ITEMS;
  if (first < nr) {
    const uint64_t r = r0 + first;
// ... 37 lines not shown
```

josefine_amd/csrc/jg_watch.h:

```cpp
#pragma once
#include "jg_compact.h"
#include "jg_device.h"
#include "jg_hosting.h"
#include "jg_read.h"
#include "jg_sparse.h"

#define JG_WATCH_ROWS 4u
#define JG_WATCH_TILE (JG_BLOCK * JG_WATCH_ROWS)
#define JG_CENSUS_ROWS 16u
#define JG_CENSUS_TILE (JG_BLOCK * JG_CENSUS_ROWS)
#define JG_WATCH_VACANT_META (((uint32_t)JG_LEAD_VACANT << 8) | ((uint32_t)JG_FAULT_VACANT << 16))

#define JG_CENSUS_LED_BY 8u
#define JG_CENSUS_MAX_TERM (JG_CENSUS_LED_BY + JG_MAX_REPLICAS + 1u)
#define JG_CENSUS_UNCOMMITTED (JG_CENSUS_MAX_TERM + 1u)
#define JG_CENSUS_WORDS (JG_CENSUS_UNCOMMITTED + 1u)
static_assert(sizeof(jg_census) == JG_CENSUS_WORDS * 8, "jg_census is the census words in order");
static_assert(sizeof(jg_leader_row) == 24, "jg_leader_row is three 8-byte pieces");

struct JgLeadView {
  uint64_t term;
  uint32_t leader_id;
  uint32_t meta;
};
// ... 66 lines not shown
  uint32_t f[JG_WATCH_ROWS];
  uint64_t m[JG_WATCH_ROWS];
  jg_watch_ballots(d, a, v, f, m);
  uint32_t c = 0;
#pragma unroll
  for (uint32_t k = 0; k < JG_WATCH_ROWS; k++) c += __popcll(m[k]);
  const uint32_t t = jg_tile_count(c);
  if (threadIdx.x == 0) a.cnt[blockIdx.x] = t, a.bsum[blockIdx.x] = t;
}

__global__ __launch_bounds__(JG_BLOCK) void k_watch_write(JgDev d, JgWatchArgs a) {
  const uint64_t base = a.bsum[blockIdx.x];
  if (a.cnt[blockIdx.x] == 0 || base >= a.cap) return;
  JgLeadView v[JG_WATCH_ROWS];
  uint32_t f[JG_WATCH_ROWS];
  uint64_t m[JG_WATCH_ROWS];
  jg_watch_ballots(d, a, v, f, m);
  const uint32_t peek = jg_gated_peek(a.peek, a.gate);
  const uint32_t t0 = blockIdx.x * JG_WATCH_TILE + threadIdx.x;
  uint64_t* out64 = (uint64_t*)a.out;
  jg_ranked_rows<JG_WATCH_ROWS>(m, base, a.cap, [&](uint32_t k, uint64_t pos) {
    const uint32_t g = a.g0 + t0 + k * JG_BLOCK;
    const uint32_t self = (f[k] & JGF_SELF_MASK) >> JGF_SELF_SHIFT;
    out64[pos * 3 + 0] = (uint64_t)(a.add + g) | (uint64_t)v[k].leader_id << 32;
    out64[pos * 3 + 1] = v[k].term;
    out64[pos * 3 + 2] = (uint64_t)(v[k].meta | self << 24);
    if (!peek) a.shadow[g] = jg_lead_shadow(v[k]);
  });
}

struct JgCensusArgs {
  uint32_t g0, n;
  uint32_t tiles;
  uint32_t pad;
  uint64_t* part;
  uint64_t* out;
};

__global__ __launch_bounds__(JG_BLOCK) void k_census(JgDev d, JgCensusArgs a) {
  const uint32_t t0 = blockIdx.x * JG_CENSUS_TILE + threadIdx.x;
  uint32_t c[JG_CENSUS_MAX_TERM];
#pragma unroll
  for (uint32_t x = 0; x < JG_CENSUS_MAX_TERM; x++) c[x] = 0;
  uint64_t max_term = 0, uncommitted = 0;
  for (uint32_t k0 = 0; k0 < JG_CENSUS_ROWS; k0 += 4) {
    uint32_t f[4];
    uint64_t term[4];
    uint4 cold[4];
#pragma unroll
    for (uint32_t k = 0; k < 4; k++) {
      const uint32_t i = t0 + (k0 + k) * JG_BLOCK;
      const bool in = i < a.n;
      const uint32_t g = a.g0 + (in ? i : 0u);
      f[k] = in ? d.flags[g] : (uint32_t)JG_FAULT_VACANT << JGF_FAULT_SHIFT;
      term[k] = in ? d.term[g] : 0ull;
      cold[k] = in ? d.cold.v[g] : make_uint4(0, 0, 0, 0);
    }
#pragma unroll
    for (uint32_t k = 0; k < 4; k++) {
      const uint32_t i = t0 + (k0 + k) * JG_BLOCK;
      const bool in = i < a.n;
      const uint32_t g = a.g0 + (in ? i : 0u);
      const JgLeadView v = jg_lead_view(d, f[k], term[k], cold[k].y);
      const uint32_t fault = (v.meta >> 16) & 0xffu, role = v.meta & 0xffu, state = (v.meta >> 8) & 0xffu;
      const bool hosted = in && fault != JG_FAULT_VACANT, healthy = hosted && fault == 0;
      const bool known = healthy && (state & JG_LEAD_KNOWN);
      c[0] += __popcll(__ballot(hosted));
      c[1] += __popcll(__ballot(in && !hosted));
      c[2] += __popcll(__ballot(hosted && fault >= 1u && fault < 128u));
      c[3] += __popcll(__ballot(hosted && fault >= 128u));
      c[4] += __popcll(__ballot(healthy && role == JG_ROLE_FOLLOWER));
      c[5] += __popcll(__ballot(healthy && role == JG_ROLE_CANDIDATE));
      c[6] += __popcll(__ballot(healthy && role == JG_ROLE_LEADER));
      c[7] += __popcll(__ballot(healthy && !known));
      bool member = false;
#pragma unroll
      for (uint32_t r = 0; r < JG_MAX_REPLICAS; r++) {
        const bool is = known && !member && r < d.R && v.leader_id == d.node_ids[r];
        c[JG_CENSUS_LED_BY + r] += __popcll(__ballot(is));
        member = member || is;
      }
      c[JG_CENSUS_LED_BY + JG_MAX_REPLICAS] += __popcll(__ballot(known && !member));
      if (hosted && v.term > max_term) max_term = v.term;
      if (healthy && role == JG_ROLE_LEADER) uncommitted += d.head[g] - jg_read_commit(d, g, f[k]);
    }
  }
  uint64_t vals[JG_CENSUS_WORDS];
#pragma unroll
  for (uint32_t x = 0; x < JG_CENSUS_MAX_TERM; x++) vals[x] = c[x];
  vals[JG_CENSUS_MAX_TERM] = jg_wave_max64(max_term);
  vals[JG_CENSUS_UNCOMMITTED] = jg_wave_sum64(uncommitted);
  jg_block_words<JG_CENSUS_WORDS>(vals, [](uint32_t x) { return x == JG_CENSUS_MAX_TERM; }, a.part);
}

__global__ __launch_bounds__(JG_BLOCK) void k_census_sum(JgCensusArgs a) {
  jg_parts_reduce<JG_CENSUS_WORDS>(a.part, a.tiles, a.out, [](uint32_t x) { return x == JG_CENSUS_MAX_TERM; });
}
```

Baseline: 490.5 billion.

## Split head column into lo/hi u32 planes and read only lo in hot paths

Stores the per-group head index as two 32-bit planes (low and high words) instead of one u64 array, and adds a JGF_HEAD_WIDE flag marking groups whose head exceeds 32 bits. The dense leader and follower fast paths then load and store only the low 4-byte plane, cutting head traffic on the bandwidth-bound path; wide heads fall back to the slow path. The calibration kernel is also narrowed to a 4-byte b column to match the new roofline traffic. The change adds overflow checks and touches every head accessor, which risks correctness near the 2^32 boundary and removes the follower mailbox range fault check.

```diff
diff --git a/josefine_amd/csrc/jg_api_drains.h b/josefine_amd/csrc/jg_api_drains.h
--- a/josefine_amd/csrc/jg_api_drains.h
+++ b/josefine_amd/csrc/jg_api_drains.h
@@ -566,8 +566,8 @@
 }
 
 template <int R>
-void launch_calib(jg_engine* e, const uint64_t* rot, const uint64_t* a8, uint64_t* b8, const uint32_t* c4) {
-  hipLaunchKernelGGL(k_stream_calib<R>, dim3(e->dense_grid), dim3(JG_BLOCK), 0, e->stream, rot, a8, b8, c4,
+void launch_calib(jg_engine* e, const uint64_t* rot, const uint64_t* a8, uint32_t* b4, const uint32_t* c4) {
+  hipLaunchKernelGGL(k_stream_calib<R>, dim3(e->dense_grid), dim3(JG_BLOCK), 0, e->stream, rot, a8, b4, c4,
                      e->cfg.n_groups);
 }
 
diff --git a/josefine_amd/csrc/jg_api_misc.h b/josefine_amd/csrc/jg_api_misc.h
--- a/josefine_amd/csrc/jg_api_misc.h
+++ b/josefine_amd/csrc/jg_api_misc.h
@@ -232,9 +232,16 @@
     t32.resize(n);
     return cold_field(d.cold.v, offset, 4, t32.data());
   };
+  auto heads = [&](uint64_t* dst) -> int {
+    std::vector<uint32_t> lo(n), hi(n);
+    HIPCHK(hipMemcpy(lo.data(), jg_head_lo_plane(d.head) + g0, (size_t)n * 4, hipMemcpyDeviceToHost));
+    HIPCHK(hipMemcpy(hi.data(), jg_head_hi_plane(d.head, d.G) + g0, (size_t)n * 4, hipMemcpyDeviceToHost));
+    for (uint32_t i = 0; i < n; i++) dst[i] = (uint64_t)hi[i] << 32 | lo[i];
+    return JG_OK;
+  };
   auto lag_base = [&](std::vector<uint64_t>& base) -> int {
     std::vector<uint64_t> top(n);
-    HIPCHK(hipMemcpy(base.data(), d.head + g0, (size_t)n * 8, hipMemcpyDeviceToHost));
+    if ((rc = heads(base.data()))) return rc;
     HIPCHK(hipMemcpy(top.data(), d.run_hi + g0, (size_t)n * 8, hipMemcpyDeviceToHost));
     for (uint32_t i = 0; i < n; i++)
       if (jg_lag_base_is_run_hi(fl[i])) base[i] = top[i];
@@ -260,13 +267,13 @@
       }
       return JG_OK;
     }
-    case JG_FIELD_HEAD: return copy64(d.head);
+    case JG_FIELD_HEAD: return heads(o64);
     case JG_FIELD_ELECTION_TIME: return cold_field(d.cold.t, JG_COLD_T_ELECTION_TIME, 8, out);
     case JG_FIELD_ELECTION_TIMEOUT: return cold_field(d.cold.t, JG_COLD_T_ELECTION_TIMEOUT, 4, out);
     case JG_FIELD_QUEUED_REQS: return cold_field(d.cold.v, JG_COLD_V_QUEUED, 4, out);
     case JG_FIELD_ID_GEN: {
       std::vector<uint64_t> head(n);
-      HIPCHK(hipMemcpy(head.data(), d.head + g0, (size_t)n * 8, hipMemcpyDeviceToHost));
+      if ((rc = heads(head.data()))) return rc;
       if ((rc = get64(d.id_gen))) return rc;
       for (uint32_t i = 0; i < n; i++) o64[i] = (fl[i] & JGF_FAST) ? head[i] + 1 : t64[i];
       return JG_OK;
@@ -469,29 +476,29 @@
   const size_t blk = std::max<size_t>(G * R * 8, 16);
   const size_t nbuf = std::min<size_t>(std::max<size_t>(((size_t)640 << 20) / blk + 1, 2), 64);
   char* rot = nullptr;
-  uint64_t *a8 = nullptr, *b8 = nullptr;
-  uint32_t* c4 = nullptr;
+  uint64_t* a8 = nullptr;
+  uint32_t *b4 = nullptr, *c4 = nullptr;
   HIPCHK(hipMalloc((void**)&rot, blk * nbuf));
   HIPCHK(hipMalloc((void**)&a8, std::max<size_t>(G * 8, 16)));
-  HIPCHK(hipMalloc((void**)&b8, std::max<size_t>(G * 8, 16)));
+  HIPCHK(hipMalloc((void**)&b4, std::max<size_t>(G * 4, 16)));
   HIPCHK(hipMalloc((void**)&c4, std::max<size_t>(G * 4, 16)));
   HIPCHK(hipMemsetAsync(rot, 0, blk * nbuf, e->stream));
   HIPCHK(hipMemsetAsync(a8, 0, std::max<size_t>(G * 8, 16), e->stream));
-  HIPCHK(hipMemsetAsync(b8, 0, std::max<size_t>(G * 8, 16), e->stream));
+  HIPCHK(hipMemsetAsync(b4, 0, std::max<size_t>(G * 4, 16), e->stream));
   HIPCHK(hipMemsetAsync(c4, 0, std::max<size_t>(G * 4, 16), e->stream));
   const uint32_t warm = 5;
   for (uint32_t i = 0; i < warm + iters; i++) {
     if (i == warm) HIPCHK(hipEventRecord(e->ev0, e->stream));
     const uint64_t* r = (const uint64_t*)(rot + (i % nbuf) * blk);
     switch (R) {
-      case 1: launch_calib<1>(e, r, a8, b8, c4); break;
-      case 2: launch_calib<2>(e, r, a8, b8, c4); break;
-      case 3: launch_calib<3>(e, r, a8, b8, c4); break;
-      case 4: launch_calib<4>(e, r, a8, b8, c4); break;
-      case 5: launch_calib<5>(e, r, a8, b8, c4); break;
-      case 6: launch_calib<6>(e, r, a8, b8, c4); break;
-      case 7: launch_calib<7>(e, r, a8, b8, c4); break;
-      default: launch_calib<8>(e, r, a8, b8, c4); break;
+      case 1: launch_calib<1>(e, r, a8, b4, c4); break;
+      case 2: launch_calib<2>(e, r, a8, b4, c4); break;
+      case 3: launch_calib<3>(e, r, a8, b4, c4); break;
+      case 4: launch_calib<4>(e, r, a8, b4, c4); break;
+      case 5: launch_calib<5>(e, r, a8, b4, c4); break;
+      case 6: launch_calib<6>(e, r, a8, b4, c4); break;
+      case 7: launch_calib<7>(e, r, a8, b4, c4); break;
+      default: launch_calib<8>(e, r, a8, b4, c4); break;
     }
   }
   HIPCHK(hipGetLastError());
@@ -502,7 +509,7 @@
   *avg_us = ms * 1000.0f / (float)iters;
   HIPCHK(hipFree(rot));
   HIPCHK(hipFree(a8));
-  HIPCHK(hipFree(b8));
+  HIPCHK(hipFree(b4));
   HIPCHK(hipFree(c4));
   return JG_OK;
 }
diff --git a/josefine_amd/csrc/jg_await.h b/josefine_amd/csrc/jg_await.h
--- a/josefine_amd/csrc/jg_await.h
+++ b/josefine_amd/csrc/jg_await.h
@@ -74,7 +74,7 @@
       const uint4 w0 = tab[at], w1 = tab[at + 1], w2 = tab[at + 2];
       const uint32_t g = w0.x < d.G ? w0.x : 0u;
       const uint32_t f = d.flags[g];
-      const uint64_t term_now = d.term[g], head = d.head[g], pw = d.mlag[g], col = d.commit[g], run_hi = d.run_hi[g];
+      const uint64_t term_now = d.term[g], head = jg_head_get(d, g), pw = d.mlag[g], col = d.commit[g], run_hi = d.run_hi[g];
       const uint64_t commit = jg_read_commit(d, g, f);
       asm volatile("" ::"v"(f), "v"(term_now), "v"(head), "v"(pw), "v"(col), "v"(run_hi));
       const uint32_t role = f & JGF_ROLE_MASK, fault = (f & JGF_FAULT_MASK) >> JGF_FAULT_SHIFT;
@@ -120,7 +120,7 @@
   }
   const uint32_t g = w0.x < d.G ? w0.x : 0u;
   const uint32_t f = d.flags[g];
-  const uint64_t term_now = d.term[g], head = d.head[g];
+  const uint64_t term_now = d.term[g], head = jg_head_get(d, g);
   const uint64_t commit = jg_read_commit(d, g, f);
   const uint32_t role = f & JGF_ROLE_MASK, fault = (f & JGF_FAULT_MASK) >> JGF_FAULT_SHIFT, self = (f & JGF_SELF_MASK) >> JGF_SELF_SHIFT;
   auto lo = [](uint64_t x) { return (uint32_t)x; };
diff --git a/josefine_amd/csrc/jg_commits.h b/josefine_amd/csrc/jg_commits.h
--- a/josefine_amd/csrc/jg_commits.h
+++ b/josefine_amd/csrc/jg_commits.h
@@ -66,7 +66,7 @@
     const bool in = i < a.n;
     const uint32_t g = a.g0 + (in ? i : 0u);
     f[k] = in ? d.flags[g] : 0u;
-    head[k] = in ? d.head[g] : 0ull;
+    head[k] = in ? jg_head_get(d, g) : 0ull;
     w[k] = in ? d.mlag[g] : 0ull;
     col[k] = in ? d.commit[g] : 0ull;
     sh[k] = in ? a.shadow[g] : make_uint4(0, 0, 0, 0);
diff --git a/josefine_amd/csrc/jg_dense.h b/josefine_amd/csrc/jg_dense.h
--- a/josefine_amd/csrc/jg_dense.h
+++ b/josefine_amd/csrc/jg_dense.h
@@ -8,7 +8,7 @@
 struct JgDenseHot {
   uint32_t* flags;
   uint64_t* mlag;
-  uint64_t* head;
+  uint32_t* head_lo;
   uint64_t* blk_decisions;
   uint32_t G;
   uint32_t hb_timeout, cfg_flags;
@@ -17,7 +17,7 @@
   uint32_t g_begin, g_end;
 };
 __host__ __device__ __forceinline__ JgDenseHot jg_dense_hot_of(const JgDev& d) {
-  return JgDenseHot{d.flags, d.mlag, d.head, d.blk_decisions, d.G, d.hb_timeout, d.cfg_flags, d.term, d.heartbeat_time, 0u, d.G};
+  return JgDenseHot{d.flags, d.mlag, jg_head_lo_plane(d.head), d.blk_decisions, d.G, d.hb_timeout, d.cfg_flags, d.term, d.heartbeat_time, 0u, d.G};
 }
 __host__ __device__ __forceinline__ JgDenseHot jg_dense_hot_range(const JgDev& d, uint32_t begin, uint32_t end, uint32_t slot0) {
   JgDenseHot h = jg_dense_hot_of(d);
@@ -75,7 +75,7 @@
 }
 template <int R, bool MAYBE_NO_ACKS = true>
 __device__ __forceinline__ void jg_dense_load(const JgDenseHot& d, const uint64_t* __restrict__ acks, uint32_t g,
-                                              uint64_t (&a)[R], uint64_t& mword, uint64_t& head) {
+                                              uint64_t (&a)[R], uint64_t& mword, uint32_t& head) {
   if (!MAYBE_NO_ACKS || acks) {
     jg_dense_load_acks<R>(acks, d.G, g, a);
   } else {
@@ -83,7 +83,7 @@
     for (int r = 0; r < R; r++) a[r] = JG_NO_ACK;
   }
   mword = d.mlag[g];
-  head = d.head[g];
+  head = d.head_lo[g];
 }
 template <int R>
 struct JgLagTick {
@@ -128,6 +128,7 @@
   const uint32_t n = (uint32_t)n_app;
   bool bad = n_app >= JG_MAX_DENSE_APPENDS;
   const uint64_t head1 = head0 + n;
+  bad |= (head1 >> 32) != 0;
   uint32_t incm = 0, somem = 0;
 #pragma unroll
   for (int r = 0; r < R; r++) {
@@ -421,7 +422,8 @@
 template <int R>
 struct JgDenseIn {
   uint32_t f;
-  uint64_t a[R], w, head;
+  uint64_t a[R], w;
+  uint32_t head;
   uint64_t term, hbt;
   uint32_t own;
 };
@@ -439,7 +441,7 @@
       in.a[r] = (ANY && (uint32_t)r == us) ? nd.offered[g] : __builtin_nontemporal_load(&acks[((size_t)r * h.G + g) * nd.ack_stride]);
     if (ANY) in.own = nd.owner[g];
     in.w = h.mlag[g];
-    in.head = h.head[g];
+    in.head = h.head_lo[g];
     in.term = h.term[g];
     in.hbt = h.heartbeat_time[g];
   }
@@ -553,7 +555,7 @@
   if (jg_lag_wide(fl, R) && (commit != commit0 || !jg_lag_wide(fc, R))) d.commit[g] = commit;
   w |= fl << (R * B);
   if (w != w0) d.mlag[g] = w;
-  if (head != head0) d.head[g] = head;
+  if (head != head0) jg_head_set(d, g, head), nf = jg_head_flag(nf, head);
   if (nf != f) d.flags[g] = nf;
 }
 
@@ -590,10 +592,10 @@
   JgLagTick<R> lt;
   lt.cwide = false, lt.adv = 0;
   uint32_t dl = 0;
-  bool hot = (f & (JGF_FAULT_MASK | JGF_ROLE_MASK | JGF_FAST)) == (JG_ROLE_LEADER | JGF_FAST);
+  bool hot = (f & (JGF_FAULT_MASK | JGF_ROLE_MASK | JGF_FAST | JGF_HEAD_WIDE)) == (JG_ROLE_LEADER | JGF_FAST);
   uint64_t base0 = head0;
   if (NODE) {
-    const bool runx = (f & (JGF_FAULT_MASK | JGF_ROLE_MASK | JGF_FAST | JGF_WIN_MASK | JGF_NO_GENESIS)) == JG_ROLE_LEADER && n_app == 0;
+    const bool runx = (f & (JGF_FAULT_MASK | JGF_ROLE_MASK | JGF_FAST | JGF_WIN_MASK | JGF_NO_GENESIS | JGF_HEAD_WIDE)) == JG_ROLE_LEADER && n_app == 0;
     if (__builtin_expect(runx, 0)) {
       if (!(f & JGF_RUN)) base0 = dp->run_hi[g];
       hot = true;
@@ -612,7 +614,7 @@
         return lt.l[r] == 0xffffffffu ? dp->match_wide[(size_t)r * h.G + g] : lt.head1 - lt.l[r];
       });
     if (lt.w1 != mword0) h.mlag[g] = lt.w1;
-    if (lt.head1 != base0) h.head[g] = lt.head1;
+    if (lt.head1 != base0) h.head_lo[g] = (uint32_t)lt.head1;
     if (lt.nf != f) h.flags[g] = lt.nf;
     if (FSM) {
       uint32_t w = (n_app ? JG_FSM_APPENDED_BIT : 0u) | lt.adv | (adv_pre << JG_FSM_PRE_SHIFT);
@@ -641,7 +643,7 @@
   }
   if (DEFER || cls != JG_DENSE_RUN) return;
   *d.cold_seen = 1;
-  jg_dense_cold_lds<R, UNIFORM>(d, acks, seq, s, f, n_app, g, a, mword0, head0, dec, sm);
+  jg_dense_cold_lds<R, UNIFORM>(d, acks, seq, s, f, n_app, g, a, mword0, (f & JGF_HEAD_WIDE) ? jg_head_get(d, g) : head0, dec, sm);
 }
 
 template <int R, bool UNIFORM, bool NODE, bool DEFER, bool FSM = false, bool ANY = false>
@@ -766,8 +768,10 @@
   for (uint32_t g = blockIdx.x * JG_BLOCK + threadIdx.x; g < G; g += gridDim.x * JG_BLOCK) {
     const uint32_t f = d.flags[g];
     const uint32_t s = UNIFORM ? us : (f & JGF_SELF_MASK) >> JGF_SELF_SHIFT;
-    uint64_t a[R], mword0, head0;
-    jg_dense_load<R, false>(jg_dense_hot_of(d), acks, g, a, mword0, head0);
+    uint64_t a[R], mword0;
+    uint32_t head_lo0;
+    jg_dense_load<R, false>(jg_dense_hot_of(d), acks, g, a, mword0, head_lo0);
+    const uint64_t head0 = head_lo0;
     asm volatile("" ::"v"(f));
     __builtin_amdgcn_sched_barrier(0);
     const bool leader = (f & JGF_ROLE_MASK) == JG_ROLE_LEADER;
@@ -780,7 +784,7 @@
     uint64_t head = head0;
     uint32_t nf = f, gdec = 0;
     uint32_t l[R + 1];
-    bool fits = B <= 21;
+    bool fits = B <= 21 && !(f & JGF_HEAD_WIDE);
 #pragma unroll
     for (int r = 0; r <= R; r++) {
       l[r] = (uint32_t)(mword0 >> (r * B)) & ESC;
@@ -820,6 +824,7 @@
     }
     uint64_t w = mword0;
     if (leader && fits) {
+      fits = (head >> 32) == 0;
       w = 0;
 #pragma unroll
       for (int r = 0; r <= R; r++) {
@@ -831,7 +836,7 @@
     if (!fits) continue;
     dec += gdec;
     if (w != mword0) d.mlag[g] = w;
-    if (head != head0) d.head[g] = head;
+    if (head != head0) jg_head_lo_plane(d.head)[g] = (uint32_t)head;
     if (nf != f) d.flags[g] = nf;
   }
   return dec;
diff --git a/josefine_amd/csrc/jg_device.h b/josefine_amd/csrc/jg_device.h
--- a/josefine_amd/csrc/jg_device.h
+++ b/josefine_amd/csrc/jg_device.h
@@ -22,6 +22,7 @@
 #define JGF_FAULT_MASK (0xffu << JGF_FAULT_SHIFT)
 #define JGF_SELF_SHIFT 24
 #define JGF_SELF_MASK (0x7u << JGF_SELF_SHIFT)
+#define JGF_HEAD_WIDE (1u << 27)
 #define JGF_WIN_SHIFT 28
 #define JGF_WIN_MASK (0xfu << JGF_WIN_SHIFT)
 
@@ -194,6 +195,19 @@
 __device__ __forceinline__ uint64_t jg_lane_base(const JgLane& L) {
   return (L.flags & (JGF_WIN_MASK | JGF_NO_GENESIS)) == 0 ? L.run_hi : L.head;
 }
+__host__ __device__ __forceinline__ uint32_t* jg_head_lo_plane(uint64_t* head) { return (uint32_t*)head; }
+__host__ __device__ __forceinline__ uint32_t* jg_head_hi_plane(uint64_t* head, uint32_t G) { return (uint32_t*)head + G; }
+__device__ __forceinline__ uint64_t jg_head_get(const JgDev& d, uint32_t g) {
+  const uint32_t lo = jg_head_lo_plane(d.head)[g], hi = jg_head_hi_plane(d.head, d.G)[g];
+  return (uint64_t)hi << 32 | lo;
+}
+__device__ __forceinline__ void jg_head_set(const JgDev& d, uint32_t g, uint64_t v) {
+  jg_head_lo_plane(d.head)[g] = (uint32_t)v;
+  jg_head_hi_plane(d.head, d.G)[g] = (uint32_t)(v >> 32);
+}
+__host__ __device__ __forceinline__ uint32_t jg_head_flag(uint32_t flags, uint64_t head) {
+  return (head >> 32) ? (flags | JGF_HEAD_WIDE) : (flags & ~JGF_HEAD_WIDE);
+}
 __device__ inline uint64_t jg_match_get(const JgDev& d, const JgLane& L, uint32_t r) {
   const uint64_t f = jg_lag_field(L.mword, r, d.R);
   return jg_lag_wide(f, d.R) ? d.match_wide[(size_t)r * d.G + L.g] : L.mbase - f;
@@ -219,7 +233,7 @@
   L.g = g;
   L.flags = d.flags[g];
   L.term = d.term[g];
-  L.head = d.head[g];
+  L.head = jg_head_get(d, g);
   L.id_gen = (L.flags & JGF_FAST) ? L.head + 1 : d.id_gen[g];
   L.run_hi = (L.flags & JGF_RUN) ? L.head : d.run_hi[g];
   L.heartbeat_time = d.heartbeat_time[g];
@@ -250,6 +264,7 @@
   const bool fast = run && (L.id_gen == L.head + 1);
   L.flags = run ? (L.flags | JGF_RUN) : (L.flags & ~JGF_RUN);
   L.flags = fast ? (L.flags | JGF_FAST) : (L.flags & ~JGF_FAST);
+  L.flags = jg_head_flag(L.flags, L.head);
   if (!fast && jg_role(L) == JG_ROLE_LEADER && !jg_fault(L)) *d.irregular_seen = 1;
   if (jg_role(L) == JG_ROLE_LEADER) {
     const uint64_t base = jg_lane_base(L);
@@ -262,7 +277,7 @@
   }
   d.flags[g] = L.flags;
   d.term[g] = L.term;
-  d.head[g] = L.head;
+  jg_head_set(d, g, L.head);
   d.id_gen[g] = L.id_gen;
   d.run_hi[g] = L.run_hi;
   d.heartbeat_time[g] = L.heartbeat_time;
@@ -283,6 +298,7 @@
   const bool fast = run && (L.id_gen == L.head + 1);
   L.flags = run ? (L.flags | JGF_RUN) : (L.flags & ~JGF_RUN);
   L.flags = fast ? (L.flags | JGF_FAST) : (L.flags & ~JGF_FAST);
+  L.flags = jg_head_flag(L.flags, L.head);
   if (!fast && jg_role(L) == JG_ROLE_LEADER && !jg_fault(L)) *d.irregular_seen = 1;
   if (jg_role(L) == JG_ROLE_LEADER) {
     const uint64_t base = jg_lane_base(L);
@@ -296,7 +312,7 @@
   }
   if (L.flags != O.flags) d.flags[g] = L.flags;
   if (L.term != O.term) d.term[g] = L.term;
-  if (L.head != O.head) d.head[g] = L.head;
+  if (L.head != O.head) jg_head_set(d, g, L.head);
   if (!fast && (L.id_gen != O.id_gen || (O.flags & JGF_FAST))) d.id_gen[g] = L.id_gen;
   if (!run && (L.run_hi != O.run_hi || (O.flags & JGF_RUN))) d.run_hi[g] = L.run_hi;
   if (L.heartbeat_time != O.heartbeat_time) d.heartbeat_time[g] = L.heartbeat_time;
diff --git a/josefine_amd/csrc/jg_follower.h b/josefine_amd/csrc/jg_follower.h
--- a/josefine_amd/csrc/jg_follower.h
+++ b/josefine_amd/csrc/jg_follower.h
@@ -59,7 +59,8 @@
     const uint64_t in_from = in_ae >> 8;
     const uint32_t in_n = (uint32_t)in_ae & 0xffu;
     const uint32_t lead = ANY ? jg_member_id(d, own) : (a.leader ? a.leader[g] : a.leader_id);
-    uint64_t term = d.term[g], head = d.head[g], commit = d.commit[g];
+    uint64_t term = d.term[g], commit = d.commit[g];
+    uint32_t head = jg_head_lo_plane(d.head)[g];
     const JgCold cold0 = jg_cold_load(d.cold, g);
     uint32_t voted_for = cold0.voted_for, leader_id = cold0.leader_id;
     const uint32_t queued = cold0.queued;
@@ -75,7 +76,8 @@
     const bool quiet = !has_hb && !has_ae &&
                        ((role == JG_ROLE_FOLLOWER && (!fired || (f & JGF_VOTED))) || (role == JG_ROLE_CANDIDATE && !fired));
     const bool nothing = (!has_hb && !has_ae && !a.tick) || quiet;
-    const bool fast = role == JG_ROLE_FOLLOWER && (f & JGF_RUN) && queued == 0;
+    const bool narrow = !(f & JGF_HEAD_WIDE) && !(has_ae && in_from >= (1ull << 32) - 255u);
+    const bool fast = role == JG_ROLE_FOLLOWER && (f & JGF_RUN) && queued == 0 && narrow;
     const bool defer = !dead && !idle_leader && !nothing && !fast;
     jg_defer_mark_in(d.fdefer_bits, d, g, defer);
     if (dead || idle_leader || nothing || defer) {
@@ -86,7 +88,8 @@
     uint32_t o_has = JG_HB_NONE;
 
     uint32_t nf = f;
-    const uint64_t term0 = term, head0 = head, commit0 = commit;
+    const uint64_t term0 = term, commit0 = commit;
+    const uint32_t head0 = head;
     const uint32_t vf0 = voted_for, lid0 = leader_id;
     bool timer_dirty = false;
     uint32_t fault = 0;
@@ -125,10 +128,10 @@
         if (in_from > head) {
           fault = JG_FAULT_EXTEND_MISSING_PARENT;
         } else {
-          const uint64_t new_head = in_from + in_n;
-          const uint64_t run_hi = new_head > head ? new_head : head;
+          const uint32_t new_head = (uint32_t)in_from + in_n;
+          const uint32_t run_hi = new_head > head ? new_head : head;
           if (nf & JGF_FAST) {
-            d.id_gen[g] = head + 1;
+            d.id_gen[g] = (uint64_t)head + 1;
             nf &= ~JGF_FAST;
           }
           head = new_head;
@@ -136,8 +139,7 @@
             d.run_hi[g] = run_hi;
             nf &= ~JGF_RUN;
           }
-          if (head >= JG_MAILBOX_NONE) fault = JG_FAULT_ENGINE_MAILBOX_RANGE;
-          else o_ack = head;
+          o_ack = head;
         }
       }
     }
@@ -151,7 +153,7 @@
     }
     a.o_answer[g] = JG_ANSWER(o_ack, o_has);
     if (term != term0) d.term[g] = term;
-    if (head != head0) d.head[g] = head;
+    if (head != head0) jg_head_lo_plane(d.head)[g] = head;
     if (commit != commit0) d.commit[g] = commit;
     jg_follower_fsm_note(a, g, commit0, commit);
     {
diff --git a/josefine_amd/csrc/jg_isr.h b/josefine_amd/csrc/jg_isr.h
--- a/josefine_amd/csrc/jg_isr.h
+++ b/josefine_amd/csrc/jg_isr.h
@@ -52,7 +52,7 @@
     }
   }
   if (rare) {
-    const uint64_t head = d.head[g], base = run ? d.run_hi[g] : head;
+    const uint64_t head = jg_head_get(d, g), base = run ? d.run_hi[g] : head;
 #pragma unroll
     for (uint32_t r = 0; r < JG_MAX_REPLICAS; r++) {
       if ((rare >> r) & 1u) {
@@ -135,7 +135,7 @@
   uint64_t head[JG_ISR_ROWS];
 #pragma unroll
   for (uint32_t k = 0; k < JG_ISR_ROWS; k++)
-    head[k] = (((m[k] >> lane) & 1ull) && v[k]) ? d.head[a.g0 + t0 + k * JG_BLOCK] : 0ull;
+    head[k] = (((m[k] >> lane) & 1ull) && v[k]) ? jg_head_get(d, a.g0 + t0 + k * JG_BLOCK) : 0ull;
   const uint32_t R = d.R;
   uint64_t* out64 = (uint64_t*)a.out;
   jg_ranked_rows<JG_ISR_ROWS>(m, base, a.cap, [&](uint32_t k, uint64_t pos) {
@@ -217,7 +217,7 @@
         }
         unc = fc;
         if (rare) {
-          const uint64_t head = d.head[g], base = run ? d.run_hi[g] : head;
+          const uint64_t head = jg_head_get(d, g), base = run ? d.run_hi[g] : head;
 #pragma unroll
           for (uint32_t r = 0; r < JG_MAX_REPLICAS; r++)
             if (r < R && r != self) lag[r] = jg_isr_lag_exact(d, g, lag[r], r, base, head);
diff --git a/josefine_amd/csrc/jg_kernels.h b/josefine_amd/csrc/jg_kernels.h
--- a/josefine_amd/csrc/jg_kernels.h
+++ b/josefine_amd/csrc/jg_kernels.h
@@ -385,16 +385,16 @@
 
 template <int R>
 __global__ __launch_bounds__(JG_BLOCK) void k_stream_calib(const uint64_t* __restrict__ rot,
-                                                            const uint64_t* __restrict__ a8, uint64_t* b8,
+                                                            const uint64_t* __restrict__ a8, uint32_t* b4,
                                                             const uint32_t* __restrict__ c4, uint32_t G) {
   for (uint32_t g = blockIdx.x * JG_BLOCK + threadIdx.x; g < G; g += gridDim.x * JG_BLOCK) {
     uint64_t v[R];
 #pragma unroll
     for (int r = 0; r < R; r++) v[r] = __builtin_nontemporal_load(&rot[(size_t)r * G + g]);
-    uint64_t s = a8[g] ^ b8[g] ^ c4[g];
+    uint64_t s = a8[g] ^ b4[g] ^ c4[g];
 #pragma unroll
     for (int r = 0; r < R; r++) s += v[r];
-    b8[g] = s;
+    b4[g] = (uint32_t)s;
   }
 }
 
diff --git a/josefine_amd/csrc/jg_lookup.h b/josefine_amd/csrc/jg_lookup.h
--- a/josefine_amd/csrc/jg_lookup.h
+++ b/josefine_amd/csrc/jg_lookup.h
@@ -27,7 +27,7 @@
     return;
   }
   const uint32_t f = d.flags[g];
-  const uint64_t term = d.term[g], head = d.head[g], commit = d.commit[g], w = d.mlag[g], run_hi = d.run_hi[g], id_gen = d.id_gen[g],
+  const uint64_t term = d.term[g], head = jg_head_get(d, g), commit = d.commit[g], w = d.mlag[g], run_hi = d.run_hi[g], id_gen = d.id_gen[g],
                  hbt = d.heartbeat_time[g];
   const uint4 ct = d.cold.t[g], cv = d.cold.v[g];
   const uint32_t role = f & JGF_ROLE_MASK, fault = (f & JGF_FAULT_MASK) >> JGF_FAULT_SHIFT, self = (f & JGF_SELF_MASK) >> JGF_SELF_SHIFT;
diff --git a/josefine_amd/csrc/jg_move.h b/josefine_amd/csrc/jg_move.h
--- a/josefine_amd/csrc/jg_move.h
+++ b/josefine_amd/csrc/jg_move.h
@@ -38,12 +38,21 @@
   const size_t G = d.G;
   uint64_t* col = nullptr;
   uint32_t k = 0;
-  if (row < 7u) {
-    col = row == 0 ? d.term : row == 1 ? d.commit : row == 2 ? d.head : row == 3 ? d.id_gen : row == 4 ? d.run_hi : row == 5 ? d.mlag : d.heartbeat_time;
+  if (row == 2u) {
+    uint32_t* q = w + 2 * (JG_MOVE_W_TERM + 2u);
+    if (EXPORT) {
+      const uint64_t v = jg_head_get(d, g);
+      q[0] = (uint32_t)v, q[1] = (uint32_t)(v >> 32);
+    } else {
+      jg_head_set(d, g, (uint64_t)q[0] | (uint64_t)q[1] << 32);
+    }
+    return;
+  } else if (row < 7u) {
+    col = row == 0 ? d.term : row == 1 ? d.commit : row == 3 ? d.id_gen : row == 4 ? d.run_hi : row == 5 ? d.mlag : d.heartbeat_time;
     col += g, k = JG_MOVE_W_TERM + row;
   } else if (row == 7u) {
-    if (EXPORT) w[2 * JG_MOVE_W_FLAGS] = d.flags[g], w[2 * JG_MOVE_W_FLAGS + 1] = 0u;
-    else d.flags[g] = w[2 * JG_MOVE_W_FLAGS];
+    if (EXPORT) w[2 * JG_MOVE_W_FLAGS] = d.flags[g] & ~JGF_HEAD_WIDE, w[2 * JG_MOVE_W_FLAGS + 1] = 0u;
+    else d.flags[g] = jg_head_flag(w[2 * JG_MOVE_W_FLAGS], (uint64_t)w[2 * (JG_MOVE_W_TERM + 2u)] | (uint64_t)w[2 * (JG_MOVE_W_TERM + 2u) + 1] << 32);
     return;
   } else if (row < 10u) {
     uint4* c = (row == 8u ? d.cold.t : d.cold.v) + g;
diff --git a/josefine_amd/csrc/jg_node.h b/josefine_amd/csrc/jg_node.h
--- a/josefine_amd/csrc/jg_node.h
+++ b/josefine_amd/csrc/jg_node.h
@@ -629,7 +629,7 @@
     const uint32_t w = c.fsm_delta[g];
     if (w) {
       const uint32_t f = d.flags[g];
-      const uint64_t head = d.head[g];
+      const uint64_t head = jg_head_get(d, g);
       const uint64_t commit1 = jg_node_commit_of(d, g, f, head);
       const bool fol = (w & JGN_FSM_FOLLOWER) != 0;
       uint64_t commit0, mid;
diff --git a/josefine_amd/csrc/jg_poll.h b/josefine_amd/csrc/jg_poll.h
--- a/josefine_amd/csrc/jg_poll.h
+++ b/josefine_amd/csrc/jg_poll.h
@@ -44,7 +44,7 @@
     if (I) ish[k] = in ? (T ? a.ic.shadow : a.ir.shadow)[g] : 0u;
     if (T) mk[k] = in ? (uint32_t)a.ic.mask[g] & ((1u << d.R) - 1u) : 0u;
     if (C) {
-      head[k] = in ? d.head[g] : 0ull;
+      head[k] = in ? jg_head_get(d, g) : 0ull;
       col[k] = in ? d.commit[g] : 0ull;
       csh[k] = in ? a.cm.shadow[g] : make_uint4(0, 0, 0, 0);
     }
diff --git a/josefine_amd/csrc/jg_read.h b/josefine_amd/csrc/jg_read.h
--- a/josefine_amd/csrc/jg_read.h
+++ b/josefine_amd/csrc/jg_read.h
@@ -46,7 +46,7 @@
   const uint32_t flags = d.flags[g];
   const uint32_t fault = (flags & JGF_FAULT_MASK) >> JGF_FAULT_SHIFT;
   const uint32_t wn = fault >= 128u ? 0u : (flags & JGF_WIN_MASK) >> JGF_WIN_SHIFT;
-  const uint64_t run_hi = (flags & JGF_RUN) ? d.head[g] : d.run_hi[g];
+  const uint64_t run_hi = (flags & JGF_RUN) ? jg_head_get(d, g) : d.run_hi[g];
   s.lo[0] = 0, s.hi[0] = run_hi, s.nx[0] = 0;
   s.ok[0] = fault < 128u && !(flags & JGF_NO_GENESIS);
 #pragma unroll
@@ -80,7 +80,7 @@
   if ((flags & JGF_ROLE_MASK) != JG_ROLE_LEADER) return d.commit[g];
   const uint64_t fc = jg_lag_field(d.mlag[g], d.R, d.R);
   if (jg_lag_wide(fc, d.R)) return d.commit[g];
-  return (jg_lag_base_is_run_hi(flags) ? d.run_hi[g] : d.head[g]) - fc;
+  return (jg_lag_base_is_run_hi(flags) ? d.run_hi[g] : jg_head_get(d, g)) - fc;
 }
 
 __device__ __forceinline__ uint64_t jg_block_exclusive_scan64(uint64_t v, uint64_t* total) {
diff --git a/josefine_amd/csrc/jg_watch.h b/josefine_amd/csrc/jg_watch.h
--- a/josefine_amd/csrc/jg_watch.h
+++ b/josefine_amd/csrc/jg_watch.h
@@ -172,7 +172,7 @@
       }
       c[JG_CENSUS_LED_BY + JG_MAX_REPLICAS] += __popcll(__ballot(known && !member));
       if (hosted && v.term > max_term) max_term = v.term;
-      if (healthy && role == JG_ROLE_LEADER) uncommitted += d.head[g] - jg_read_commit(d, g, f[k]);
+      if (healthy && role == JG_ROLE_LEADER) uncommitted += jg_head_get(d, g) - jg_read_commit(d, g, f[k]);
     }
   }
   uint64_t vals[JG_CENSUS_WORDS];
```

Result: no change. 488.7 billion (-0.4%).
